# advait/c4a0

Hardware: AMD Instinct MI355X
Metric: self-play games/sec (and MCTS sims/sec) at n_mcts=100 (higher is better)
Workload: dtype bf16

## Files before the change

c4a0_amd/_lib.py:

```python
from __future__ import annotations

import ctypes as C
import os

_HERE = os.path.dirname(os.path.abspath(__file__))
LIB_PATH = os.path.join(_HERE, os.environ.get("C4A0_HIP_LIB", "libc4a0_hip.so"))

OK, ERR_BAD_ARG, ERR_HIP, ERR_NAN_IN_TREE, ERR_DEGENERATE_POLICY, ERR_ARENA_OVERFLOW, ERR_NOT_BOUND, ERR_NO_DEVICE, ERR_ILLEGAL_MOVE, ERR_CANCELLED = range(10)
STATUS_NAMES = {
    0: "C4_OK", 1: "C4_ERR_BAD_ARG", 2: "C4_ERR_HIP", 3: "C4_ERR_NAN_IN_TREE", 4: "C4_ERR_DEGENERATE_POLICY",
    5: "C4_ERR_ARENA_OVERFLOW", 6: "C4_ERR_NOT_BOUND", 7: "C4_ERR_NO_DEVICE", 8: "C4_ERR_ILLEGAL_MOVE", 9: "C4_ERR_CANCELLED",
}
FLAG_NO_MOVES = 1
FLAG_ONE_SIM_PER_STEP = 2
FLAG_RECLAIM = 4
FLAG_NO_RECLAIM = 8
FLAG_SEARCH = 16
FLAG_HOLD = 32
HOLD_PARKED = 64
HOLD_MOVE_NONE, HOLD_MOVE_SAMPLE = -1, -2
HOLD_OK, HOLD_REFUSED_TERMINAL, HOLD_REFUSED_COLUMN, HOLD_REFUSED_UNSEARCHED, HOLD_REFUSED_SAMPLE, HOLD_NO_GAME = range(6)
HOLD_POLL_UNKNOWN = 0xFFFFFFFF
MAX_SAMPLES_PER_GAME = 43
ABI_VERSION = 13
STRUCT_LAYOUT_SINCE = 7


class C4Error(RuntimeError):
    def __init__(self, status: int, detail: str = ""):
        self.status = status
        super().__init__(f"{STATUS_NAMES.get(status, status)}: {detail}" if detail else STATUS_NAMES.get(status, str(status)))


class GameMetadataC(C.Structure):
    _fields_ = [("game_id", C.c_uint64), ("player0_id", C.c_uint64), ("player1_id", C.c_uint64)]


class SampleRec(C.Structure):
    _fields_ = [("game_id", C.c_uint64), ("mask", C.c_uint64), ("value", C.c_uint64), ("policy", C.c_float * 7),
                ("q_penalty", C.c_float), ("q_no_penalty", C.c_float), ("meta", C.c_uint32)]


class Config(C.Structure):
    _fields_ = [("n_slots", C.c_uint32), ("blocks_per_slot", C.c_uint32), ("n_mcts_iterations", C.c_uint32),
                ("c_exploration", C.c_float), ("c_ply_penalty", C.c_float), ("planes_dtype", C.c_uint32),
                ("flags", C.c_uint32), ("device", C.c_int32), ("reclaim_period", C.c_uint32)]


class Counters(C.Structure):
    _fields_ = [(n, C.c_uint64) for n in ("sims", "select_levels", "backup_nodes", "expansions", "moves", "games_done",
                                          "ref_skipped_sims", "samples", "games_started", "step_kernel_ns", "step_launches",
                                          "eval_cache_probes", "eval_cache_hits", "reclaim_passes", "reclaim_blocks")] + \
               [("error", C.c_uint32), ("error_slot", C.c_uint32)]

    def as_dict(self):
        return {n: int(getattr(self, n)) for n, _ in self._fields_}


class NetworkBf16(C.Structure):
    _fields_ = [("channels", C.c_uint32), ("n_blocks", C.c_uint32), ("tower_w0", C.c_void_p), ("tower_w", C.c_void_p), ("tower_bias", C.c_void_p),
                ("w1", C.c_void_p), ("b1", C.c_void_p), ("n_policy_hidden", C.c_uint32), ("n_value_hidden", C.c_uint32),
                ("policy_w", C.c_void_p * 8), ("policy_b", C.c_void_p * 8), ("value_w", C.c_void_p * 8), ("value_b", C.c_void_p * 8),
                ("policy_out_w", C.c_void_p), ("value_out_w", C.c_void_p), ("policy_out_b", C.c_void_p), ("value_out_b", C.c_void_p)]


class PlayOptions(C.Structure):
    _fields_ = [("device", C.c_int32), ("resident_games", C.c_uint32), ("concurrent_sessions", C.c_uint32), ("steps_per_graph", C.c_uint32),
                ("tail_steps_per_graph", C.c_uint32), ("blocks_per_slot", C.c_uint32), ("flags", C.c_uint32), ("reclaim_period", C.c_uint32),
                ("dirichlet_alpha", C.c_float), ("dirichlet_epsilon", C.c_float), ("eval_cache_entries", C.c_uint64)]


class PlayPhases(C.Structure):
    _fields_ = [("setup_s", C.c_double), ("capture_s", C.c_double), ("steady_s", C.c_double), ("tail_s", C.c_double), ("drain_s", C.c_double),
                ("rounds", C.c_uint64), ("rounds_until_all_started", C.c_uint64), ("graph_captures", C.c_uint32), ("resident_games", C.c_uint32),
                ("sessions", C.c_uint32), ("rows_at_end", C.c_uint32)]

    def as_dict(self):
        return {n: getattr(self, n) for n, _ in self._fields_}


_P = C.POINTER
_vp = C.c_void_p
SIGNATURES = {
    "c4_last_error_string": (C.c_char_p, []),
    "c4_abi_version": (C.c_int, []),
    "c4_source_hash": (C.c_char_p, []),
    "c4_device_count": (C.c_int, [_P(C.c_int)]),
    "c4_session_create": (C.c_int, [_P(Config), _P(_vp)]),
    "c4_session_destroy": (C.c_int, [_vp]),
    "c4_session_set_games": (C.c_int, [_vp, _P(GameMetadataC), C.c_uint64, _P(C.c_uint64), _P(C.c_uint64)]),
    "c4_session_bind_io": (C.c_int, [_vp, _vp, _vp, _vp, _vp]),
    "c4_session_set_dirichlet": (C.c_int, [_vp, C.c_float, C.c_float]),
    "c4_session_bind_leaf_models": (C.c_int, [_vp, _vp]),
    "c4_session_set_eval_cache": (C.c_int, [_vp, C.c_uint64, C.c_uint32]),
    "c4_session_progress": (C.c_int, [_vp, _P(C.c_uint64), _P(C.c_uint64), _P(C.c_uint32)]),
    "c4_session_compact": (C.c_int, [_vp, C.c_uint32, _P(C.c_uint32), _P(C.c_uint32)]),
    "c4_session_start": (C.c_int, [_vp]),
    "c4_session_step": (C.c_int, [_vp]),
    "c4_session_set_step_shape": (C.c_int, [_vp, C.c_uint32]),
    "c4_session_step_head_out": (C.c_int, [_vp, _vp, _vp, _vp, _vp, _vp, _vp, C.c_uint32, C.c_uint32, C.c_uint32]),
    "c4_session_set_timing": (C.c_int, [_vp, C.c_int]),
    "c4_session_counters": (C.c_int, [_vp, _P(Counters)]),
    "c4_session_poll": (C.c_int, [_vp, _P(C.c_uint64), _P(C.c_uint32)]),
    "c4_session_arena": (C.c_int, [_vp, _P(C.c_uint64), _P(C.c_uint32), _P(C.c_uint32)]),
    "c4_session_sample_counts": (C.c_int, [_vp, _P(C.c_uint32), C.c_uint64]),
    "c4_session_drain_samples": (C.c_int, [_vp, _P(SampleRec), C.c_uint64, _P(C.c_uint64)]),
    "c4_session_pack_samples": (C.c_int, [_vp, _vp, C.c_uint64, _P(C.c_uint64)]),
    "c4_session_debug_phase_stamps": (C.c_int, [_vp, _P(C.c_uint64), C.c_uint64, _P(C.c_uint64)]),
    "c4_session_sample_store": (C.c_int, [_vp, _P(_vp), _P(_vp), _P(C.c_uint64)]),
    "c4_session_root_stats": (C.c_int, [_vp, C.c_uint32, _P(C.c_float), _P(C.c_float), _P(C.c_float),
                                        _P(C.c_uint64), _P(C.c_uint64), _P(C.c_uint64)]),
    "c4_trim_cached_memory": (C.c_int, []),
    "c4_records_to_cbor": (C.c_int, [_vp, _vp, C.c_uint64, _vp, C.c_uint64, _vp, C.c_uint64, _P(C.c_uint64)]),
    "c4_shuffle_games": (C.c_int, [C.c_uint64, C.c_uint64, _vp]),
    "c4_play_games_cancel": (None, []),
    "c4_play_games_bf16": (C.c_int, [_vp, C.c_uint64, C.c_uint32, C.c_float, C.c_float, _P(NetworkBf16), _P(PlayOptions), _vp, _vp, C.c_uint64,
                                     _P(C.c_uint64), _P(Counters), _P(PlayPhases)]),
    "c4_search_positions_bf16": (C.c_int, [_vp, _vp, C.c_uint64, C.c_uint32, C.c_float, C.c_float, _P(NetworkBf16), _P(PlayOptions), _vp, C.c_uint64,
                                           _P(Counters), _P(PlayPhases)]),
    "c4_cbor_to_records": (C.c_int, [_vp, C.c_uint64, _vp, _vp, C.c_uint64, _vp, C.c_uint64, _P(C.c_uint64), _P(C.c_uint64)]),
    "c4_session_leaf_keys": (C.c_int, [_vp, _vp]),
    "c4_session_unique_leaves": (C.c_int, [_vp, _vp, _vp, _vp, _vp]),
    "c4_session_scatter_outputs": (C.c_int, [_vp, _vp, _vp, C.c_uint32]),
    "c4_session_step_gather": (C.c_int, [_vp, _vp, _vp, C.c_uint32]),
    "c4_session_set_iterations": (C.c_int, [_vp, C.c_uint32]),
    "c4_session_hold_resume": (C.c_int, [_vp, _vp, _vp, _vp]),
    "c4_session_snapshot": (C.c_int, [_vp, _vp, _vp, _vp, C.c_uint64]),
    "c4_session_hold_poll": (C.c_int, [_vp, _P(C.c_uint32), _P(C.c_uint32), _P(C.c_uint32)]),
    "c4_session_leaves": (C.c_int, [_vp, _P(C.c_uint64), _P(C.c_uint64), _P(C.c_uint32), _P(C.c_uint32)]),
    "c4_pos_ops": (C.c_int, [_vp, _vp, _vp, C.c_uint64, C.c_float, _vp, _vp, _vp, _vp, _vp, _vp]),
    "c4_encode_planes": (C.c_int, [_vp, _vp, C.c_uint64, C.c_uint32, _vp, _vp]),
    "c4_expf_logf": (C.c_int, [_vp, C.c_uint64, C.c_int, _vp, _vp]),
    "c4_softmax7": (C.c_int, [_vp, _vp, C.c_uint64, _vp, _vp, _vp]),
    "c4_apply_temperature": (C.c_int, [_vp, _vp, C.c_uint64, _vp, _vp]),
    "c4_conv_tower_bf16": (C.c_int, [_vp, _vp, _vp, _vp, C.c_uint32, C.c_uint32, C.c_uint32, _vp, C.c_uint32, _vp]),
    "c4_linear_bf16": (C.c_int, [_vp, _vp, _vp, _vp, C.c_uint32, C.c_uint32, C.c_uint32, C.c_uint32, C.c_uint32, C.c_uint32, C.c_uint32, _vp]),
    "c4_linear_bf16_tile_map": (C.c_int, [C.c_uint32, C.c_uint32, C.c_uint32, C.c_uint32, _P(C.c_uint32), C.c_uint32, _P(C.c_uint32)]),
    "c4_planes_from_f32": (C.c_int, [_vp, _vp, C.c_uint32, _vp, C.c_uint32, _vp]),
    "c4_head_out_bf16": (C.c_int, [_vp, _vp, _vp, _vp, _vp, _vp, C.c_uint32, C.c_uint32, C.c_uint32, C.c_uint32, _vp, _vp, _vp]),
    "c4_dirichlet": (C.c_int, [_vp, _vp, _vp, C.c_float, C.c_uint64, _vp, _vp]),
    "c4_sample_move": (C.c_int, [_vp, _vp, _vp, _vp, C.c_uint64, _vp, _vp, _vp]),
    "c4_conv_tower_f32": (C.c_int, [_vp, _vp, _vp, _vp, C.c_uint32, C.c_uint32, C.c_uint32, _vp, _vp, _vp]),
    "c4_linear_f32": (C.c_int, [_vp, _vp, _vp, _vp, C.c_uint32, C.c_uint32, C.c_uint32, C.c_uint32, C.c_uint32, C.c_uint32, _vp]),
    "c4_head_out_f32": (C.c_int, [_vp, _vp, _vp, _vp, _vp, _vp, C.c_uint32, C.c_uint32, C.c_uint32, C.c_uint32, C.c_uint32, _vp, _vp, _vp, _vp]),
}

_lib = None


def lib() -> C.CDLL:
    global _lib
    if _lib is None:
        if not os.path.exists(LIB_PATH):
            raise ImportError(
                f"{LIB_PATH} is missing: the HIP extension is the product and there is no fallback. "
                "Build it with `python c4a0_amd/csrc/build.py` (hipcc --offload-arch=gfx950).")
        import torch

        L = C.CDLL(LIB_PATH)
        diagnostic = "C4A0_HIP_LIB" in os.environ
        for name, (res, args) in SIGNATURES.items():
            fn = getattr(L, name, None)
            if fn is None:
                if diagnostic:
                    continue
                raise ImportError(f"{LIB_PATH} does not export {name}")
            fn.restype = res
            fn.argtypes = args
        if L.c4_abi_version() != ABI_VERSION and not diagnostic:
            raise ImportError(f"{LIB_PATH} implements C ABI version {L.c4_abi_version()}, this binding is written for {ABI_VERSION}")
        if diagnostic and L.c4_abi_version() < STRUCT_LAYOUT_SINCE:
            raise ImportError(f"{LIB_PATH} implements C ABI version {L.c4_abi_version()}: c4_config / c4_counters changed layout in version "
                              f"{STRUCT_LAYOUT_SINCE}; build the A/B library from a revision at or after it")
        if "C4A0_HIP_LIB" not in os.environ:
            from .csrc import build as _build

            have, want = L.c4_source_hash().decode(), _build.source_hash()
            if have != want:
                raise ImportError(f"{LIB_PATH} was built from different sources (hash {have}, tree {want}): "
                                  "rebuild it with `python c4a0_amd/csrc/build.py`")
        _lib = L
    return _lib

# ... 6 lines not shown
```

c4a0_amd/csrc/build.py:

```python
import hashlib
import os
import subprocess
import sys

HERE = os.path.dirname(os.path.abspath(__file__))
PKG = os.path.dirname(HERE)
OUT = os.path.join(PKG, "libc4a0_hip.so")
SRCS = [os.path.join(HERE, "c4_session.hip"), os.path.join(HERE, "c4_conv_tower.hip"), os.path.join(HERE, "c4_head_gemm.hip"), os.path.join(HERE, "c4_results_host.hip"), os.path.join(HERE, "c4_selfplay_host.hip"), os.path.join(HERE, "c4_f32_net.hip")]
DEPS = SRCS + [os.path.join(HERE, "c4_device.hpp"), os.path.join(HERE, "c4_host.hpp"), os.path.join(HERE, "c4_head_out.hpp"), os.path.join(HERE, "c4_timeline.hpp"),
               os.path.join(os.path.dirname(PKG), "include", "c4a0_hip.h")]
FLAGS = ["--offload-arch=gfx950", "-O3", "-std=c++17", "-fPIC", "-shared", "-ffp-contract=off",
         "-fno-fast-math", "-Wall", "-Wno-unused-function",
         "-mllvm", "-amdgpu-kernarg-preload-count=16"]
MARKER = b"c4a0-src-hash:"


def source_hash(extra_flags=()) -> str:
    h = hashlib.sha256(" ".join(FLAGS + list(extra_flags)).encode())
    for d in DEPS:
        h.update(os.path.basename(d).encode() + b"\0")
        with open(d, "rb") as f:
            h.update(f.read())
    return h.hexdigest()[:32]


def embedded_hash(path: str):
    try:
        with open(path, "rb") as f:
            blob = f.read()
    except OSError:
        return None
    i = blob.find(MARKER)
    if i < 0:
        return None
    return blob[i + len(MARKER): i + len(MARKER) + 32].decode("ascii", "replace")


def is_stale(path: str = OUT, extra_flags=()) -> bool:
    return embedded_hash(path) != source_hash(extra_flags)


def build(force: bool = False, verbose: bool = False, diag: bool = False) -> str:
    hipcc = os.environ.get("HIPCC", "/opt/rocm/bin/hipcc")
    out = OUT.replace(".so", "_diag.so") if diag else OUT
    extra = ["-DC4_PHASE_STAMPS", "-DC4_DIAG_VARIANTS"] if diag else []
    if force or is_stale(out, extra):
        tmp = out + ".tmp%d" % os.getpid()
        cmd = [hipcc] + FLAGS + extra + ['-DC4_SOURCE_HASH="%s"' % source_hash(extra)] + SRCS + ["-o", tmp]
        if verbose:
            print(" ".join(cmd))
        r = subprocess.run(cmd, capture_output=True, text=True)
        if r.returncode != 0:
            if os.path.exists(tmp):
                os.remove(tmp)
            raise RuntimeError("hipcc failed:\n" + r.stdout + r.stderr)
        os.replace(tmp, out)
        if verbose and r.stderr:
            print(r.stderr)
    return out


if __name__ == "__main__":
    print(build(force="--force" in sys.argv, verbose=True, diag="--diag" in sys.argv))
```

c4a0_amd/csrc/c4_conv_tower.hip:

```cpp
#include <hip/hip_runtime.h>
#include <stdint.h>
#include <stdio.h>
#include <stdlib.h>

#include <string>
#include <type_traits>

#include "../../include/c4a0_hip.h"
#include "c4_head_out.hpp"
#include "c4_host.hpp"
#include "c4_timeline.hpp"

#ifndef C4_TOWER_PAIR_SAME_SIMD
#define C4_TOWER_PAIR_SAME_SIMD 0
#endif
#ifndef C4_TOWER_ALT_PRIO
#define C4_TOWER_ALT_PRIO 0
#endif

namespace {

typedef __bf16 bf16x8 __attribute__((ext_vector_type(8)));
typedef __bf16 bf16x4 __attribute__((ext_vector_type(4)));
typedef float f32x4 __attribute__((ext_vector_type(4)));

constexpr int kBS = 56;
constexpr int kTilesPerBoard = 3;

__device__ __forceinline__ int cell_slot(int r, int c) { return (r + 1) * 8 + (c + 1) + 1; }

template <int C, int NB>
struct Geo {
  static constexpr int KG = C / 8;
  static constexpr int MT = C / 16;
  static constexpr int KC = C / 32;
  static constexpr int kPlane = (NB * kBS + 10 + 15) / 16 * 16;
  static constexpr int kBufSlots = KG * kPlane;
  static constexpr bool kStageW = (C == 32);
  static constexpr int kWFrags = 9 * MT * KC;
  static constexpr int kLdsBytes = 2 * kBufSlots * 16 + (kStageW ? 2 * kWFrags * 1024 : 0);
  static constexpr int kTiles = NB * kTilesPerBoard;
  static_assert((kPlane * 16) % 256 == 0, "channel-group planes must keep the bank phase");
  static_assert(kLdsBytes <= 160 * 1024, "LDS budget");
};

#ifdef C4_PHASE_STAMPS
__device__ unsigned long long c4_tower_clk[80];
#define C4_TSTAMP(i) do { if (threadIdx.x == 0) tw_ts[i] = __builtin_amdgcn_s_memrealtime(); } while (0)
#else
#define C4_TSTAMP(i) do { } while (0)
#endif

struct TowerParams {
  const uint16_t* planes;
  const bf16x8* w0;
  const bf16x8* w;
  const float* bias;
  uint16_t* out;
  uint32_t n_boards;
  uint32_t n_blocks;
};

template <int C, int NB, bool kConv0, bool kSecond, bool kLast, int G_TILES, int MTW, bool kPrefetch, typename WF, typename Hook>
__device__ __forceinline__ void tower_layer(const uint4* __restrict__ src, uint4* __restrict__ dst, WF& wf,
                                            const float* __restrict__ bias, int tile_lo, int m0, int lane, Hook&& after_last_tile,
                                            uint16_t* __restrict__ out = nullptr, uint32_t board0 = 0, uint32_t n_boards = 0) {
  using G = Geo<C, NB>;
  constexpr int kSteps = kConv0 ? 3 : 9 * G::KC;
  constexpr int NF = kPrefetch ? 2 : 1;
  const int li = lane & 15, lg = lane >> 4;

  f32x4 bias4[MTW];
#pragma unroll
  for (int m = 0; m < MTW; m++) {
    const float* bp = bias + 16 * (m0 + m) + 4 * lg;
    bias4[m] = f32x4{bp[0], bp[1], bp[2], bp[3]};
  }

  uint4 fr[NF][kSteps];
  f32x4 acc[2][MTW];
  uint2 old[2][MTW];
  int e_slot[2], e_cell[2];
  int e_board[2];

  auto tile_cell = [&](int g, int& cell) __attribute__((always_inline)) {
    const int tl = tile_lo + g;
    const int bidx = tl / kTilesPerBoard;
    const int slot = 9 + 16 * (tl - bidx * kTilesPerBoard) + li;
    cell = slot;
    return bidx * kBS + slot;
  };
  auto load_frags = [&](int g, int f) __attribute__((always_inline)) {
    int cell;
    const int base = tile_cell(g, cell);
#pragma unroll
    for (int k = 0; k < kSteps; k++) {
      int d, plane;
      if (kConv0) {
        int tap = 4 * k + lg;
        tap = tap < 9 ? tap : 4;
        d = 8 * (tap / 3 - 1) + (tap % 3 - 1);
        plane = 0;
      } else {
        const int t = k / G::KC, kc = k % G::KC;
        d = 8 * (t / 3 - 1) + (t % 3 - 1);
        plane = 4 * kc + lg;
      }
      fr[f][k] = src[plane * G::kPlane + base + d];
    }
  };
  auto out_ptr = [&](int slot_in_plane, int m) __attribute__((always_inline)) {
    return reinterpret_cast<uint2*>(&dst[(2 * (m0 + m) + (lg >> 1)) * G::kPlane + slot_in_plane]) + (lg & 1);
  };
  auto start_tile = [&](int g, int a) __attribute__((always_inline)) {
    e_slot[a] = tile_cell(g, e_cell[a]);
    e_board[a] = (tile_lo + g) / kTilesPerBoard;
#pragma unroll
    for (int m = 0; m < MTW; m++) {
      acc[a][m] = bias4[m];
      if (kSecond && kPrefetch) old[a][m] = *out_ptr(e_slot[a], m);
    }
  };
  auto mfmas = [&](int f, int a) __attribute__((always_inline)) {
#pragma unroll
    for (int k = 0; k < kSteps; k++) {
#pragma unroll
      for (int m = 0; m < MTW; m++)
        acc[a][m] = __builtin_amdgcn_mfma_f32_16x16x32_bf16(wf[k][m], __builtin_bit_cast(bf16x8, fr[f][k]), acc[a][m], 0, 0, 0);
    }
  };
  auto epilogue = [&](int a) __attribute__((always_inline)) {
    const bool valid = ((e_cell[a] - 1) & 7) != 0;
#pragma unroll
    for (int m = 0; m < MTW; m++) {
      f32x4 v = acc[a][m];
      if (kSecond) {
        const uint2 o = kPrefetch ? old[a][m] : *out_ptr(e_slot[a], m);
        const float o0 = __uint_as_float(o.x << 16), o1 = __uint_as_float(o.x & 0xffff0000u);
        const float o2 = __uint_as_float(o.y << 16), o3 = __uint_as_float(o.y & 0xffff0000u);
        v[0] = o0 + fmaxf(v[0], 0.f); v[1] = o1 + fmaxf(v[1], 0.f);
        v[2] = o2 + fmaxf(v[2], 0.f); v[3] = o3 + fmaxf(v[3], 0.f);
      }
      const bf16x4 o = __builtin_convertvector(v, bf16x4);
      if (kLast) {
        const int rc = e_cell[a] - 1, cell = 7 * ((rc >> 3) - 1) + (rc & 7) - 1;
        const uint32_t gb = board0 + (uint32_t)e_board[a];
        if (valid && gb < n_boards)
          *reinterpret_cast<uint2*>(out + ((size_t)gb * 42 + cell) * C + 16 * (m0 + m) + 4 * lg) = __builtin_bit_cast(uint2, o);
      } else if (valid) {
        *out_ptr(e_slot[a], m) = __builtin_bit_cast(uint2, o);
      }
    }
  };

  load_frags(0, 0);
  if (kPrefetch) {
#pragma unroll
    for (int g = 0; g < G_TILES; g++) {
      const int a = g & 1, f = g & 1;
      start_tile(g, a);
      if (g + 1 < G_TILES) load_frags(g + 1, f ^ 1);
      mfmas(f, a);
      if (g >= 1) epilogue(a ^ 1);
    }
    epilogue((G_TILES - 1) & 1);
  } else {
#pragma unroll
    for (int g = 0; g < G_TILES; g++) {
      start_tile(g, 0);
      mfmas(0, 0);
      epilogue(0);
      if (g + 1 < G_TILES) load_frags(g + 1, 0);
    }
  }
  after_last_tile();
}

struct NoStamp { __device__ __forceinline__ void operator()(int) const {} };
struct NoFeed { static constexpr bool kRing = false; };
template <int C>
struct RingFeed {
  static constexpr bool kRing = true;
  static constexpr int kStageSlots = (C / 16) * (C / 32) * 64;
  const uint4* ring;
  __amdgpu_buffer_rsrc_t rsrc;
  int t, n_stages, wave, lane;
  __device__ __forceinline__ void issue(int st) {
    __builtin_amdgcn_raw_ptr_buffer_load_lds(rsrc, (__attribute__((address_space(3))) void*)(ring + (st & 3) * kStageSlots + wave * 64), 16,
                                             (int)((uint32_t)(lane * 16) | (st >= n_stages ? 0x80000000u : 0u)), st * (kStageSlots * 16) + wave * 1024, 0, 0);
  }
  __device__ __forceinline__ void stage_top() {
    t += 1;
    asm volatile("s_waitcnt vmcnt(2) lgkmcnt(0)" ::: "memory");
    __builtin_amdgcn_s_barrier();
    issue(t + 4);
  }
  template <typename WQ, int MTW>
  __device__ __forceinline__ void read(WQ& wq, int s, int kc, int m0) const {
    const uint4* st = ring + ((t + 1) & 3) * kStageSlots + lane;
#pragma unroll
    for (int m = 0; m < MTW; m++) wq[s % 2][m] = __builtin_bit_cast(bf16x8, st[((m0 + m) * (C / 32) + kc) * 64]);
  }
};
__device__ __forceinline__ float tower_relu1(float v) {
  float r;
  asm("v_max_f32 %0, 0, %1" : "=v"(r) : "v"(v));
  return r;
}
template <int C, int NB, int G_TILES, int MTW, int kDepth, typename WQ, typename Stamp = NoStamp, int kMode = -1, typename Feed = NoFeed>
__device__ __forceinline__ void tower_layer_stream(const bool kSecond, const bool kLast, const uint4* __restrict__ src, uint4* __restrict__ dst, WQ& wq,
                                                   const bf16x8* __restrict__ w_layer, bool has_next, const float* __restrict__ bias,
                                                   int tile_lo, int m0, int lane, uint16_t* __restrict__ out = nullptr,
                                                   uint32_t board0 = 0, uint32_t n_boards = 0, Stamp&& stamp = NoStamp{}, Feed&& feed = NoFeed{}) {
  using G = Geo<C, NB>;
  using FeedT = typename std::remove_reference<Feed>::type;
  constexpr int kSteps = 9 * G::KC;
  static_assert(kSteps % kDepth == 0, "the weight ring keeps its phase from layer to layer");
  static_assert(!FeedT::kRing || (kDepth == 2 && G::KC == 2), "the LDS ring is read one stage (= one tap = two k-steps) ahead");
  const int li = lane & 15, lg = lane >> 4;

  auto request = [&](int s) __attribute__((always_inline)) {
    if constexpr (FeedT::kRing) { feed.template read<WQ, MTW>(wq, s, s % G::KC, m0); return; }
    const int sl = s % kSteps;
    const bf16x8* wl = w_layer + (s >= kSteps ? G::kWFrags * 64 : 0);
#pragma unroll
    for (int m = 0; m < MTW; m++) wq[s % kDepth][m] = wl[(((sl / G::KC) * G::MT + m0 + m) * G::KC + (sl % G::KC)) * 64 + lane];
  };

  int base[G_TILES], cell[G_TILES];
  f32x4 acc[G_TILES][MTW];
#pragma unroll
  for (int g = 0; g < G_TILES; g++) {
    const int tl = tile_lo + g;
    const int bidx = tl / kTilesPerBoard;
    cell[g] = 9 + 16 * (tl - bidx * kTilesPerBoard) + li;
    base[g] = bidx * kBS + cell[g];
#pragma unroll
    for (int m = 0; m < MTW; m++) {
      const float* bp = bias + 16 * (m0 + m) + 4 * lg;
      acc[g][m] = f32x4{bp[0], bp[1], bp[2], bp[3]};
    }
  }
  uint4 fr[2][G_TILES][G::KC];
  auto read_row = [&](int r, int f) __attribute__((always_inline)) {
    const int d = 8 * (r - 1);
#pragma unroll
    for (int g = 0; g < G_TILES; g++)
#pragma unroll
      for (int kc = 0; kc < G::KC; kc++) fr[f][g][kc] = src[(4 * kc + lg) * G::kPlane + base[g] + d];
  };
  auto shifted = [&](const uint4& v, int dc) __attribute__((always_inline)) {
    if (dc == 1) return v;
    uint4 o;
    if (dc == 2) {
      o.x = (uint32_t)__builtin_amdgcn_update_dpp(0, (int)v.x, 0x101, 0xF, 0xF, true); o.y = (uint32_t)__builtin_amdgcn_update_dpp(0, (int)v.y, 0x101, 0xF, 0xF, true);
      o.z = (uint32_t)__builtin_amdgcn_update_dpp(0, (int)v.z, 0x101, 0xF, 0xF, true); o.w = (uint32_t)__builtin_amdgcn_update_dpp(0, (int)v.w, 0x101, 0xF, 0xF, true);
    } else {
      o.x = (uint32_t)__builtin_amdgcn_update_dpp(0, (int)v.x, 0x111, 0xF, 0xF, true); o.y = (uint32_t)__builtin_amdgcn_update_dpp(0, (int)v.y, 0x111, 0xF, 0xF, true);
      o.z = (uint32_t)__builtin_amdgcn_update_dpp(0, (int)v.z, 0x111, 0xF, 0xF, true); o.w = (uint32_t)__builtin_amdgcn_update_dpp(0, (int)v.w, 0x111, 0xF, 0xF, true);
// ... 11 lines not shown
      if constexpr (FeedT::kRing) {
        if (3 * r + dc > 0) { feed.stage_top(); __builtin_amdgcn_sched_barrier(0); }
      }
#pragma unroll
      for (int kc = 0; kc < G::KC; kc++) {
        const int s = (3 * r + dc) * G::KC + kc;
#pragma unroll
        for (int g = 0; g < G_TILES; g++) {
          const uint4 bfrag = shifted(fr[r & 1][g][kc], dc);
#pragma unroll
          for (int m = 0; m < MTW; m++)
            acc[g][m] = __builtin_amdgcn_mfma_f32_16x16x32_bf16(wq[s % kDepth][m], __builtin_bit_cast(bf16x8, bfrag), acc[g][m], 0, 0, 0);
        }
        if (FeedT::kRing || s + kDepth < kSteps || has_next) request(s + kDepth);
        __builtin_amdgcn_sched_barrier(0);
      }
    }
  }
  stamp(1);
  if constexpr (kMode >= 0) {
    constexpr bool kSec = kMode >= 1, kLst = kMode == 2;
    auto optr = [&](int g, int m) __attribute__((always_inline)) {
      return reinterpret_cast<uint2*>(&dst[(2 * (m0 + m) + (lg >> 1)) * G::kPlane + base[g]]) + (lg & 1);
    };
    uint2 res[G_TILES][MTW];
    if (kSec) {
#pragma unroll
      for (int g = 0; g < G_TILES; g++)
#pragma unroll
        for (int m = 0; m < MTW; m++) res[g][m] = *optr(g, m);
    }
    const bool valid = (li & 7) != 0;
    const uint32_t vmask = valid ? 0xFFFFFFFFu : 0u;
#pragma unroll
    for (int g = 0; g < G_TILES; g++) {
#pragma unroll
      for (int m = 0; m < MTW; m++) {
        f32x4 v = acc[g][m];
        if (kSec) {
          const uint2 o = res[g][m];
          v[0] = __uint_as_float(o.x << 16) + tower_relu1(v[0]); v[1] = __uint_as_float(o.x & 0xffff0000u) + tower_relu1(v[1]);
          v[2] = __uint_as_float(o.y << 16) + tower_relu1(v[2]); v[3] = __uint_as_float(o.y & 0xffff0000u) + tower_relu1(v[3]);
        }
        uint2 ob = __builtin_bit_cast(uint2, __builtin_convertvector(v, bf16x4));
        if (kLst) {
          const int rc = cell[g] - 1, bcell = 7 * ((rc >> 3) - 1) + (rc & 7) - 1;
          const uint32_t gb = board0 + (uint32_t)((tile_lo + g) / kTilesPerBoard);
          if (valid && gb < n_boards) *reinterpret_cast<uint2*>(out + ((size_t)gb * 42 + bcell) * C + 16 * (m0 + m) + 4 * lg) = ob;
        } else {
          ob.x &= vmask; ob.y &= vmask;
          *optr(g, m) = ob;
        }
      }
    }
    stamp(2);
    return;
  }
#pragma unroll
  for (int g = 0; g < G_TILES; g++) {
    const bool valid = ((cell[g] - 1) & 7) != 0;
#pragma unroll
    for (int m = 0; m < MTW; m++) {
      uint2* op = reinterpret_cast<uint2*>(&dst[(2 * (m0 + m) + (lg >> 1)) * G::kPlane + base[g]]) + (lg & 1);
      f32x4 v = acc[g][m];
      if (kSecond) {
        const uint2 o = *op;
        v[0] = __uint_as_float(o.x << 16) + fmaxf(v[0], 0.f); v[1] = __uint_as_float(o.x & 0xffff0000u) + fmaxf(v[1], 0.f);
        v[2] = __uint_as_float(o.y << 16) + fmaxf(v[2], 0.f); v[3] = __uint_as_float(o.y & 0xffff0000u) + fmaxf(v[3], 0.f);
      }
      const bf16x4 o = __builtin_convertvector(v, bf16x4);
      if (kLast) {
        const int rc = cell[g] - 1, bcell = 7 * ((rc >> 3) - 1) + (rc & 7) - 1;
        const uint32_t gb = board0 + (uint32_t)((tile_lo + g) / kTilesPerBoard);
        if (valid && gb < n_boards)
          *reinterpret_cast<uint2*>(out + ((size_t)gb * 42 + bcell) * C + 16 * (m0 + m) + 4 * lg) = __builtin_bit_cast(uint2, o);
      } else if (valid) {
        *op = __builtin_bit_cast(uint2, o);
      }
    }
  }
  stamp(2);
}

template <int KW, int NWAVES>
__device__ __forceinline__ void dma_weights(const void* w, uint32_t bytes, uint4* lds_dst, int first_frag, int wave, int lane) {
  const auto rsrc = __builtin_amdgcn_make_buffer_rsrc(const_cast<void*>(w), 0, (int)bytes, 0x00020000);
  const int wave_u = __builtin_amdgcn_readfirstlane(wave);
  for (int c = wave_u; c < KW; c += NWAVES)
    __builtin_amdgcn_raw_ptr_buffer_load_lds(rsrc, (__attribute__((address_space(3))) void*)(lds_dst + c * 64), 16, lane * 16, (first_frag + c) * 1024, 0, 0);
}

template <int C, int NB, int NT, int MS, bool ST = false, int KD = 3, bool RG = false>
__global__ __launch_bounds__(NT) void c4_conv_tower_kernel(const uint16_t* __restrict__ a_planes, const bf16x8* __restrict__ a_w0, const bf16x8* __restrict__ a_w,
                                                             const float* __restrict__ a_bias, uint16_t* __restrict__ a_out, uint32_t a_n_boards, uint32_t a_n_blocks) {
  const TowerParams p{a_planes, a_w0, a_w, a_bias, a_out, a_n_boards, a_n_blocks};
  C4_TL_BEGIN();
#ifdef C4_PHASE_STAMPS
  unsigned long long tw_ts[64];
  const unsigned long long wave_c0 = __builtin_amdgcn_s_memtime();
  const unsigned long long wave_r0 = __builtin_amdgcn_s_memrealtime();
  auto tw_flush = [&](int last) {
    if (threadIdx.x == 0) {
      atomicAdd(&c4_tower_clk[70], __builtin_amdgcn_s_memtime() - wave_c0);
      atomicAdd(&c4_tower_clk[71], __builtin_amdgcn_s_memrealtime() - wave_r0);
      atomicAdd(&c4_tower_clk[0], 1ull);
      for (int i = 0; i < last; i++) atomicAdd(&c4_tower_clk[1 + i], tw_ts[i + 1] - tw_ts[i]);
      atomicMin(&c4_tower_clk[78], tw_ts[0]);
      atomicMax(&c4_tower_clk[79], tw_ts[last]);
    }
  };
#endif
  C4_TSTAMP(0);
#ifdef C4_PHASE_STAMPS
  const unsigned long long wave_t0 = __builtin_amdgcn_s_memrealtime();
#endif
  using G = Geo<C, NB>;
  constexpr int MTW = G::MT / MS;
  static_assert(G::MT % MS == 0 && (!G::kStageW || MS == 1), "co-tile split");

  extern __shared__ __attribute__((aligned(256))) uint8_t lds_raw[];
  uint4* X = reinterpret_cast<uint4*>(lds_raw);
  uint4* T = X + G::kBufSlots;

  const int tid = threadIdx.x;
  const int lane = tid & 63;
  const int wave = tid >> 6;
#if C4_TOWER_PAIR_SAME_SIMD
  constexpr int kGroups = NT / 64 / MS;
  const int grp_index = wave % kGroups, grp_member = wave / kGroups;
#else
  const int grp_index = wave / MS, grp_member = wave % MS;
#endif
  const int m0 = grp_member * MTW;
  const uint32_t board0 = blockIdx.x * NB;

  constexpr int kWSteps = 9 * G::KC;
  bf16x8 wf[kWSteps][MTW];
#pragma unroll
  for (int k = 0; k < 3; k++)
#pragma unroll
    for (int m = 0; m < MTW; m++) wf[k][m] = p.w0[(k * G::MT + m0 + m) * 64 + lane];
  const int n_layers = 2 * (int)p.n_blocks;
  if constexpr (ST && RG) {
    RingFeed<C> f0{reinterpret_cast<const uint4*>(lds_raw) + 2 * G::kBufSlots,
                   __builtin_amdgcn_make_buffer_rsrc(const_cast<bf16x8*>(p.w), 0, (int)(2u * p.n_blocks * G::kWFrags * 1024u), 0x00020000), -1, 9 * n_layers,
                   __builtin_amdgcn_readfirstlane(wave), lane};
#pragma unroll
    for (int st = 0; st < 4; st++) f0.issue(st);
  }
  auto load_layer_weights = [&](int layer) __attribute__((always_inline)) {
    const bf16x8* wl = p.w + (size_t)(layer - 1) * G::kWFrags * 64;
#pragma unroll
    for (int k = 0; k < kWSteps; k++)
#pragma unroll
      for (int m = 0; m < MTW; m++) wf[k][m] = wl[(((k / G::KC) * G::MT + m0 + m) * G::KC + (k % G::KC)) * 64 + lane];
  };
  uint4* Wst = T + G::kBufSlots;
  auto stage_layer_weights = [&](int layer) __attribute__((always_inline)) {
    if (layer <= n_layers)
      dma_weights<G::kWFrags, NT / 64>(p.w, 2u * p.n_blocks * G::kWFrags * 1024u, Wst + (layer & 1) * G::kWFrags * 64, (layer - 1) * G::kWFrags, wave, lane);
  };
  auto fetch_staged_weights = [&](int layer) __attribute__((always_inline)) {
    const uint4* ws = Wst + (layer & 1) * G::kWFrags * 64;
#pragma unroll
    for (int k = 0; k < kWSteps; k++)
#pragma unroll
      for (int m = 0; m < MTW; m++)
        wf[k][m] = __builtin_bit_cast(bf16x8, ws[(((k / G::KC) * G::MT + m0 + m) * G::KC + (k % G::KC)) * 64 + lane]);
  };
  if (G::kStageW && !ST) stage_layer_weights(1);

  constexpr int kIn = (NB * 42 + NT - 1) / NT;
  uint32_t in_v[kIn];
#pragma unroll
  for (int j = 0; j < kIn; j++) {
    const int i = tid + j * NT;
    const int b = i / 42, cell = i - b * 42;
    const uint32_t g = board0 + b;
    in_v[j] = 0;
    if (i < NB * 42 && g < p.n_boards) in_v[j] = (uint32_t)p.planes[(size_t)g * 84 + cell] | ((uint32_t)p.planes[(size_t)g * 84 + 42 + cell] << 16);
  }
  for (int i = tid; i < 2 * G::kBufSlots; i += NT) X[i] = make_uint4(0, 0, 0, 0);
  int* pair_ctr = reinterpret_cast<int*>(lds_raw + G::kLdsBytes);
  if (ST && !RG && tid < 16) pair_ctr[tid] = 0;
  __syncthreads();
#pragma unroll
  for (int j = 0; j < kIn; j++) {
    const int i = tid + j * NT;
    const int b = i / 42, cell = i - b * 42;
    if (i < NB * 42) T[b * kBS + cell_slot(cell / 7, cell % 7)] = make_uint4(in_v[j], 0, 0, 0);
  }
  __syncthreads();
  C4_TSTAMP(1);

  constexpr int kWaves = NT / 64 / MS;
  static_assert(G::kTiles % kWaves == 0, "every wavefront owns the same number of cell tiles");
  constexpr int kTilesPerWave = G::kTiles / kWaves;
  constexpr bool kPrefetch = (C == 32);
  constexpr bool kFuseOut = (C == 32);
  const int tile_lo = grp_index * kTilesPerWave;

  if constexpr (ST && RG) {
    static_assert(NT == 512 && MS == 2 && C == 64, "one 1 KB DMA piece per wavefront and stage");
    const uint4* ring = T + G::kBufSlots;
    float* bias_lds = reinterpret_cast<float*>(lds_raw + 2 * G::kBufSlots * 16 + 4 * RingFeed<C>::kStageSlots * 16);
    RingFeed<C> feed{ring, __builtin_amdgcn_make_buffer_rsrc(const_cast<bf16x8*>(p.w), 0, (int)(2u * p.n_blocks * G::kWFrags * 1024u), 0x00020000),
                     -1, 9 * n_layers, __builtin_amdgcn_readfirstlane(wave), lane};
    for (int i = tid; i < n_layers * C; i += NT) bias_lds[i] = p.bias[C + i];
    bf16x8 wq[2][MTW];
    tower_layer<C, NB, true, false, false, kTilesPerWave, MTW, false>(T, X, wf, p.bias, tile_lo, m0, lane, [&]() __attribute__((always_inline)) {});
    asm volatile("s_waitcnt vmcnt(0) lgkmcnt(0)" ::: "memory");
    __builtin_amdgcn_s_barrier();
    feed.template read<decltype(wq), MTW>(wq, 0, 0, m0);
    feed.template read<decltype(wq), MTW>(wq, 1, 1, m0);
    for (int layer = 1; layer <= n_layers; layer++) {
      const bool second = (layer & 1) == 0;
      const float* bl = bias_lds + (size_t)(layer - 1) * C;
      if (layer == n_layers)
        tower_layer_stream<C, NB, kTilesPerWave, MTW, 2, decltype(wq), NoStamp, 2, RingFeed<C>&>(true, true, T, X, wq, nullptr, false, bl, tile_lo, m0, lane, p.out, board0, p.n_boards, NoStamp{}, feed);
      else if (second)
        tower_layer_stream<C, NB, kTilesPerWave, MTW, 2, decltype(wq), NoStamp, 1, RingFeed<C>&>(true, false, T, X, wq, nullptr, true, bl, tile_lo, m0, lane, p.out, board0, p.n_boards, NoStamp{}, feed);
      else
        tower_layer_stream<C, NB, kTilesPerWave, MTW, 2, decltype(wq), NoStamp, 0, RingFeed<C>&>(false, false, X, T, wq, nullptr, true, bl, tile_lo, m0, lane, p.out, board0, p.n_boards, NoStamp{}, feed);
    }
    asm volatile("s_waitcnt vmcnt(0)" ::: "memory");
    if (n_layers > 0) return;
  } else if constexpr (ST) {
    constexpr int kDepth = KD;
    bf16x8 wq[kDepth][MTW];
    if (n_layers >= 1) {
#pragma unroll
      for (int sdx = 0; sdx < kDepth; sdx++)
#pragma unroll
        for (int m = 0; m < MTW; m++) wq[sdx][m] = p.w[(((sdx / G::KC) * G::MT + m0 + m) * G::KC + (sdx % G::KC)) * 64 + lane];
    }
    tower_layer<C, NB, true, false, false, kTilesPerWave, MTW, false>(T, X, wf, p.bias, tile_lo, m0, lane, [&]() __attribute__((always_inline)) {});
    constexpr bool kBarrier = !(MS == 1 && kTilesPerWave % kTilesPerBoard == 0);
    if (kBarrier) __syncthreads();
    C4_TSTAMP(2);
    for (int layer = 1; layer <= n_layers; layer++) {
      const bf16x8* wl = p.w + (size_t)(layer - 1) * G::kWFrags * 64;
      const bool has_next = layer < n_layers;
      const float* bl = p.bias + (size_t)layer * C;
      const bool second = (layer & 1) == 0;
#if C4_TOWER_ALT_PRIO
      if (((layer ^ (__builtin_amdgcn_readfirstlane(wave) >> 2)) & 1) != 0) __builtin_amdgcn_s_setprio(1); else __builtin_amdgcn_s_setprio(0);
#endif
#ifdef C4_PHASE_STAMPS
      auto st_stamp = [&](int q) __attribute__((always_inline)) {
        asm volatile("s_waitcnt vmcnt(0) lgkmcnt(0)" ::: "memory");
        if (layer <= 19) C4_TSTAMP(2 + 3 * (layer - 1) + q);
      };
#elif defined(C4_TOWER64_FENCE)
      auto st_stamp = [&](int q) __attribute__((always_inline)) {
        if (C4_TOWER64_FENCE == 1) asm volatile("" ::: "memory");
        if (C4_TOWER64_FENCE == 2) asm volatile("s_waitcnt lgkmcnt(0)" ::: "memory");
        if (C4_TOWER64_FENCE == 3) asm volatile("s_waitcnt vmcnt(0) lgkmcnt(0)" ::: "memory");
      };
#else
      NoStamp st_stamp;
#endif
      if constexpr (MS == 1) {
        if (layer == n_layers)
          tower_layer_stream<C, NB, kTilesPerWave, MTW, kDepth, decltype(wq), decltype(st_stamp)&, 2>(true, true, T, X, wq, wl, false, bl, tile_lo, m0, lane, p.out, board0, p.n_boards, st_stamp);
        else if (second)
          tower_layer_stream<C, NB, kTilesPerWave, MTW, kDepth, decltype(wq), decltype(st_stamp)&, 1>(true, false, T, X, wq, wl, true, bl, tile_lo, m0, lane, p.out, board0, p.n_boards, st_stamp);
        else
          tower_layer_stream<C, NB, kTilesPerWave, MTW, kDepth, decltype(wq), decltype(st_stamp)&, 0>(false, false, X, T, wq, wl, true, bl, tile_lo, m0, lane, p.out, board0, p.n_boards, st_stamp);
      } else
      tower_layer_stream<C, NB, kTilesPerWave, MTW, kDepth>(second, layer == n_layers, second ? T : X, second ? X : T, wq, wl, has_next, bl, tile_lo, m0, lane,
                                                            p.out, board0, p.n_boards, st_stamp);
#ifdef C4_PHASE_STAMPS
      if (layer == n_layers) {
        st_stamp(3);
        if (layer <= 19) tw_flush(2 + 3 * layer);
        if (lane == 0) atomicAdd(&c4_tower_clk[62 + wave], __builtin_amdgcn_s_memrealtime() - wave_t0);
      }
#endif
      if (layer == n_layers) return;
      if (kBarrier) {
        __builtin_amdgcn_fence(__ATOMIC_RELEASE, "workgroup");
        int* ctr = pair_ctr + grp_index;
        if (lane == 0) __hip_atomic_fetch_add(ctr, 1, __ATOMIC_RELAXED, __HIP_MEMORY_SCOPE_WORKGROUP);
        while (__hip_atomic_load(ctr, __ATOMIC_RELAXED, __HIP_MEMORY_SCOPE_WORKGROUP) < MS * layer) __builtin_amdgcn_s_sleep(1);
        __builtin_amdgcn_fence(__ATOMIC_ACQUIRE, "workgroup");
      }
#if defined(C4_PHASE_STAMPS) || defined(C4_TOWER64_FENCE)
      st_stamp(3);
#endif
    }
  } else {
  tower_layer<C, NB, true, false, false, kTilesPerWave, MTW, kPrefetch>(T, X, wf, p.bias, tile_lo, m0, lane, [&]() __attribute__((always_inline)) {
    if (!G::kStageW && n_layers >= 1) load_layer_weights(1);
  });
  if (G::kStageW) asm volatile("s_waitcnt vmcnt(0)" ::: "memory");
  __syncthreads();
  C4_TSTAMP(2);
  for (int layer = 1; layer <= n_layers; layer++) {
    const bool is_second = (layer & 1) == 0;
    if (G::kStageW) {
      stage_layer_weights(layer + 1);
      fetch_staged_weights(layer);
    }
    auto next_weights = [&]() __attribute__((always_inline)) {
      if (!G::kStageW && layer < n_layers) load_layer_weights(layer + 1);
    };
    if (kFuseOut && layer == n_layers) {
      tower_layer<C, NB, false, true, true, kTilesPerWave, MTW, kPrefetch>(T, X, wf, p.bias + (size_t)layer * C, tile_lo, m0, lane, next_weights,
                                                                          p.out, board0, p.n_boards);
#ifdef C4_PHASE_STAMPS
      asm volatile("s_waitcnt vmcnt(0)" ::: "memory");
      if (layer < 20) { C4_TSTAMP(2 + layer); tw_flush(2 + layer); }
#endif
      C4_TL_END(1, p.out);
      return;
    }
    if (is_second) tower_layer<C, NB, false, true, false, kTilesPerWave, MTW, kPrefetch>(T, X, wf, p.bias + (size_t)layer * C, tile_lo, m0, lane, next_weights);
    else tower_layer<C, NB, false, false, false, kTilesPerWave, MTW, kPrefetch>(X, T, wf, p.bias + (size_t)layer * C, tile_lo, m0, lane, next_weights);
    if (G::kStageW) asm volatile("s_waitcnt vmcnt(0)" ::: "memory");
    __syncthreads();
#ifdef C4_PHASE_STAMPS
    if (layer < 20) C4_TSTAMP(2 + layer);
#endif
  }
  }

  if (ST) __syncthreads();
  for (int i = tid; i < NB * 42 * G::KG; i += NT) {
    const int kg = i % G::KG;
    const int bc = i / G::KG;
    const int b = bc / 42, cell = bc - b * 42;
    const uint32_t g = board0 + b;
    if (g < p.n_boards) {
      const uint4 v = X[kg * G::kPlane + b * kBS + cell_slot(cell / 7, cell % 7)];
      reinterpret_cast<uint4*>(p.out)[((size_t)g * 42 + cell) * G::KG + kg] = v;
    }
  }
  C4_TL_END(1, p.out);
}

template <int C, int NB, int NT, int MS, bool ST = false, int KD = 3, bool RG = false>
int launch_tower(const TowerParams& p, uint32_t n_boards, hipStream_t stream, int device) {
  const int kLds = Geo<C, NB>::kLdsBytes + (ST ? 64 : 0) + (RG ? 4 * RingFeed<C>::kStageSlots * 16 + 2 * (int)p.n_blocks * C * 4 : 0);
  auto k = c4_conv_tower_kernel<C, NB, NT, MS, ST, KD, RG>;
  hipError_t e = c4host::opt_in_lds((const void*)k, RG ? 160 * 1024 : kLds, device);
  if (e != hipSuccess) return c4host::fail(C4_ERR_HIP, std::string("c4_conv_tower_bf16: LDS opt-in (") + std::to_string(kLds) + " bytes) on device " + std::to_string(device) + ": " + hipGetErrorString(e));
  k<<<dim3((n_boards + NB - 1) / NB), dim3(NT), kLds, stream>>>(p.planes, p.w0, p.w, p.bias, p.out, p.n_boards, p.n_blocks);
  e = hipGetLastError();
  if (e != hipSuccess) return c4host::fail(C4_ERR_HIP, std::string("c4_conv_tower_bf16 launch: ") + hipGetErrorString(e));
  return C4_OK;
}

}

#ifdef C4_PHASE_STAMPS
extern "C" int c4_debug_tower_phases(double* phase_us, int n, double* span_us, unsigned long long* n_workgroups, int reset) {
  unsigned long long h[80];
  if (hipDeviceSynchronize() != hipSuccess || hipMemcpyFromSymbol(h, HIP_SYMBOL(c4_tower_clk), sizeof h) != hipSuccess) return C4_ERR_HIP;
  for (int i = 0; i < n && i < 76; i++) phase_us[i] = h[0] ? (double)h[1 + i] / (double)h[0] * 0.01 : 0.0;
  if (span_us) *span_us = h[79] > h[78] ? (double)(h[79] - h[78]) * 0.01 : 0.0;
  if (n_workgroups) *n_workgroups = h[0];
  if (reset) { unsigned long long z[80] = {0}; z[78] = ~0ull; if (hipMemcpyToSymbol(HIP_SYMBOL(c4_tower_clk), z, sizeof z) != hipSuccess) return C4_ERR_HIP; }
  return C4_OK;
}
#endif

C4_TL_SETTER(c4_debug_timeline_tower)

extern "C" {

int c4_conv_tower_bf16(const void* planes_dev, const void* w0_dev, const void* w_dev, const float* bias_dev,
                       uint32_t n_boards, uint32_t channels, uint32_t n_blocks, void* out_dev, uint32_t config, void* stream) {
  if (!planes_dev || !w0_dev || !bias_dev || !out_dev || (n_blocks && !w_dev)) return c4host::fail(C4_ERR_BAD_ARG, "c4_conv_tower_bf16: null argument");
  if (channels != 32 && channels != 64) return c4host::fail(C4_ERR_BAD_ARG, "c4_conv_tower_bf16: channels must be 32 or 64");
  if (n_boards == 0) return C4_OK;
  const int device = c4host::stream_device((hipStream_t)stream);
  c4host::DeviceGuard guard(device);
  if (guard.error() != hipSuccess) return c4host::fail(C4_ERR_HIP, std::string("c4_conv_tower_bf16: hipSetDevice: ") + hipGetErrorString(guard.error()));
  TowerParams p{(const uint16_t*)planes_dev, (const bf16x8*)w0_dev, (const bf16x8*)w_dev, bias_dev, (uint16_t*)out_dev, n_boards, n_blocks};
  if (config > 6 || (channels == 32 && config > 5)) return c4host::fail(C4_ERR_BAD_ARG, "c4_conv_tower_bf16: config must be 0 (automatic) .. 5 (32 channels) / .. 6 (64 channels)");
  if (channels == 64 && config == 4 && Geo<64, 8>::kLdsBytes + 64 + 4 * RingFeed<64>::kStageSlots * 16 + 2 * (int)n_blocks * 64 * 4 > 160 * 1024)
    return c4host::fail(C4_ERR_BAD_ARG, "c4_conv_tower_bf16: config 4 (weights through an LDS ring) keeps the layers' biases in LDS behind the ring: at most 23 residual blocks");
  if (channels == 32 && config == 1) return launch_tower<32, 16, 512, 1>(p, n_boards, (hipStream_t)stream, device);
  if (channels == 32 && config == 2) return launch_tower<32, 8, 512, 1>(p, n_boards, (hipStream_t)stream, device);
  if (channels == 32 && config == 3) return launch_tower<32, 16, 768, 1>(p, n_boards, (hipStream_t)stream, device);
  if (channels == 32 && config == 4) return launch_tower<32, 4, 768, 1>(p, n_boards, (hipStream_t)stream, device);
  if (channels == 32 && config == 5) return launch_tower<32, 2, 384, 1>(p, n_boards, (hipStream_t)stream, device);
  if (channels == 32 && n_boards <= 512) return launch_tower<32, 2, 384, 1>(p, n_boards, (hipStream_t)stream, device);
  if (channels == 32 && n_boards <= 1024) return launch_tower<32, 4, 768, 1>(p, n_boards, (hipStream_t)stream, device);
  if (channels == 32 && n_boards <= 8 * 160)
    return launch_tower<32, 8, 512, 1>(p, n_boards, (hipStream_t)stream, device);
#ifdef C4_DIAG_VARIANTS
  static const int st32 = [] { const char* e = getenv("C4_TOWER32_STREAM"); return e ? atoi(e) : 0; }();
  if (channels == 32 && st32) return launch_tower<32, 16, 512, 1, true>(p, n_boards, (hipStream_t)stream, device);
  static const int held = [] { const char* e = getenv("C4_TOWER64_HELD"); return e ? atoi(e) : 0; }();
  if (channels == 64 && held) return launch_tower<64, 8, 512, 2>(p, n_boards, (hipStream_t)stream, device);
#endif
  if (channels == 32)
    return launch_tower<32, 16, 512, 1>(p, n_boards, (hipStream_t)stream, device);
  if (channels == 64 && (config == 5 || (config == 0 && n_boards > 512 && n_boards <= 1024))) return launch_tower<64, 4, 512, 2, true>(p, n_boards, (hipStream_t)stream, device);
  if (channels == 64 && (config == 6 || (config == 0 && n_boards <= 512))) return launch_tower<64, 2, 256, 2, true>(p, n_boards, (hipStream_t)stream, device);
  if (channels == 64 && config == 2) return launch_tower<64, 8, 256, 1, true, 6>(p, n_boards, (hipStream_t)stream, device);
  if (channels == 64 && config == 3) return launch_tower<64, 8, 256, 1, true, 3>(p, n_boards, (hipStream_t)stream, device);
  if (channels == 64 && config == 4 && Geo<64, 8>::kLdsBytes + 64 + 4 * RingFeed<64>::kStageSlots * 16 + 2 * (int)n_blocks * 64 * 4 <= 160 * 1024)
    return launch_tower<64, 8, 512, 2, true, 2, true>(p, n_boards, (hipStream_t)stream, device);
  return launch_tower<64, 8, 512, 2, true>(p, n_boards, (hipStream_t)stream, device);
// ... 152 lines not shown
```

c4a0_amd/csrc/c4_head_out.hpp:

```cpp
#pragma once
#include <hip/hip_runtime.h>
#include <stdint.h>

namespace c4ho {

typedef __bf16 bf16x8 __attribute__((ext_vector_type(8)));
typedef float f32x4 __attribute__((ext_vector_type(4)));

constexpr int kHeadWaves = 6, kHeadSteps = 7;

struct Shared {
  f32x4 part[kHeadWaves][2][64];
  float tile[2][16][17];
  float res[16][12];
};

template <int kRows>
__device__ __forceinline__ void head_out_block(Shared& sh, const uint4* __restrict__ hp, const uint4* __restrict__ hv, const uint4* __restrict__ wp,
                                               const uint4* __restrict__ wv, const float* __restrict__ bp, const float* __restrict__ bv, uint32_t n_boards,
                                               uint32_t f8, uint32_t sp8, uint32_t sv8, float* __restrict__ logprobs, float* __restrict__ q, uint32_t block) {
  const uint32_t lane = threadIdx.x & 63, wave = threadIdx.x >> 6;
  const uint32_t row = lane & 15, kq = lane >> 4;
  const uint32_t g0 = block * kRows;
  const uint32_t gr = g0 + (row & (kRows - 1));
  const uint32_t g = gr < n_boards ? gr : n_boards - 1;
  const uint4* xp = hp + (size_t)g * sp8 + kq;
  const uint4* xv = hv + (size_t)g * sv8 + kq;
  const uint4* wpl = wp + (size_t)(row < 7 ? row : 0) * f8 + kq;
  const uint4* wvl = wv + (size_t)(row < 2 ? row : 0) * f8 + kq;
  f32x4 accp = {0.f, 0.f, 0.f, 0.f}, accv = {0.f, 0.f, 0.f, 0.f};
  const uint32_t n_iter = f8 / (4 * kHeadSteps * kHeadWaves);
  for (uint32_t it = 0; it < n_iter; it++) {
    const uint32_t s0 = (it * kHeadWaves + wave) * kHeadSteps;
    uint4 a_p[kHeadSteps], a_v[kHeadSteps], b_p[kHeadSteps], b_v[kHeadSteps];
#pragma unroll
    for (int s = 0; s < kHeadSteps; s++) {
      a_p[s] = xp[4 * (s0 + s)];
      a_v[s] = xv[4 * (s0 + s)];
      b_p[s] = wpl[4 * (s0 + s)];
      b_v[s] = wvl[4 * (s0 + s)];
    }
    __builtin_amdgcn_sched_barrier(0);
    const uint32_t mp = row < 7 ? 0xFFFFFFFFu : 0u, mv = row < 2 ? 0xFFFFFFFFu : 0u;
#pragma unroll
    for (int s = 0; s < kHeadSteps; s++) {
      b_p[s].x &= mp; b_p[s].y &= mp; b_p[s].z &= mp; b_p[s].w &= mp;
      b_v[s].x &= mv; b_v[s].y &= mv; b_v[s].z &= mv; b_v[s].w &= mv;
    }
#pragma unroll
    for (int s = 0; s < kHeadSteps; s++) {
      accp = __builtin_amdgcn_mfma_f32_16x16x32_bf16(__builtin_bit_cast(bf16x8, a_p[s]), __builtin_bit_cast(bf16x8, b_p[s]), accp, 0, 0, 0);
      accv = __builtin_amdgcn_mfma_f32_16x16x32_bf16(__builtin_bit_cast(bf16x8, a_v[s]), __builtin_bit_cast(bf16x8, b_v[s]), accv, 0, 0, 0);
    }
  }
  sh.part[wave][0][lane] = accp;
  sh.part[wave][1][lane] = accv;
  __syncthreads();
  if (wave < 2) {
    f32x4 sum = sh.part[0][wave][lane];
#pragma unroll
    for (int w = 1; w < kHeadWaves; w++) sum += sh.part[w][wave][lane];
    const float bias = wave == 0 ? (row < 7 ? bp[row] : 0.f) : (row < 2 ? bv[row] : 0.f);
#pragma unroll
    for (int r = 0; r < 4; r++) sh.tile[wave][4 * kq + r][row] = sum[r] + bias;
  }
  __syncthreads();
  if (threadIdx.x < kRows) {
    const uint32_t b = threadIdx.x, gb = g0 + b;
    float v[9];
#pragma unroll
    for (int o = 0; o < 7; o++) v[o] = sh.tile[0][b][o];
    v[7] = sh.tile[1][b][0];
    v[8] = sh.tile[1][b][1];
    float mx = v[0];
#pragma unroll
    for (int o = 1; o < 7; o++) mx = fmaxf(mx, v[o]);
    float sm = 0.f;
#pragma unroll
    for (int o = 0; o < 7; o++) sm += expf(v[o] - mx);
    const float lse = mx + logf(sm);
    const float q0 = tanhf(v[7]), q1 = tanhf(v[8]);
#pragma unroll
    for (int o = 0; o < 7; o++) sh.res[b][o] = v[o] - lse;
    sh.res[b][7] = q0;
    sh.res[b][8] = q1;
    if (gb < n_boards) {
#pragma unroll
      for (int o = 0; o < 7; o++) logprobs[(size_t)gb * 7 + o] = v[o] - lse;
      q[(size_t)gb * 2 + 0] = q0;
      q[(size_t)gb * 2 + 1] = q1;
    }
  }
}

}
```

c4a0_amd/csrc/c4_session.hip:

```cpp
#include <hip/hip_runtime.h>
#include <hip/hip_bf16.h>
#include <stddef.h>
#include <stdint.h>
#include <stdio.h>
#include <stdlib.h>
#include <string.h>
#include <mutex>
#include <string>
#include <vector>

#include "../../include/c4a0_hip.h"
#include "c4_device.hpp"
#include "c4_head_out.hpp"
#include "c4_host.hpp"
#include "c4_timeline.hpp"

#pragma clang fp contract(off)

namespace {

struct __attribute__((aligned(16))) Entry {
  uint32_t n;
  float q_pen;
  float q_nopen;
  float prior;
};
struct __attribute__((aligned(16))) Tail {
  uint16_t child[7];
  uint16_t legal;
};
struct __attribute__((aligned(128))) Block {
  Entry e[7];
  Tail t;
};
constexpr uint32_t kMaxBlocksPerSlot = 65535;

constexpr uint32_t kMaxPath = 43;
constexpr uint32_t kHotPath = 16;
struct __attribute__((aligned(256))) Slot {
  uint64_t root_mask, root_value;
  uint64_t leaf_mask, leaf_value;
  uint64_t game_id;
  uint32_t ordinal;
  uint32_t root_n;
  uint32_t state;
  uint32_t arena;
  uint32_t root_ref;
  uint32_t rng_word;
  uint32_t path[kHotPath];
  uint32_t path_deep[kMaxPath - kHotPath];
  uint32_t pad_[32 - (kMaxPath - kHotPath)];
};
static_assert(sizeof(Slot) == 256 && offsetof(Slot, path) == 64 && offsetof(Slot, path_deep) == 128, "slot state: one hot line + the deep path");
C4_DEV constexpr uint32_t slot_state(uint32_t status, uint32_t depth, uint32_t n_moves, uint32_t term, uint32_t rng_for) {
  return status | (depth << 8) | (n_moves << 16) | (term << 24) | (rng_for << 26);
}
C4_DEV uint32_t slot_status(uint32_t state) { return state & 0xFFu; }
static_assert(sizeof(Block) == 128 && sizeof(Entry) == 16 && sizeof(Tail) == 16 && sizeof(c4_sample_rec) == 64, "layout");

enum : uint32_t { kIdle = 0, kActive = 1, kParked = C4_HOLD_PARKED };
constexpr uint32_t kWavesPerTimingHelper = 1024;

#ifdef C4_PHASE_STAMPS
#define C4_STAMP(i, force)                                                                          \
  do {                                                                                              \
    asm volatile("s_waitcnt vmcnt(0) lgkmcnt(0)" ::: "memory");                                       \
    if (lane == 0) p.phase[(size_t)wave_index * 16 + (i)] = __builtin_amdgcn_s_memrealtime() + ((force) & 0);  \
  } while (0)
#define C4_STAMP_ANY(i)                                                                             \
  do {                                                                                              \
    asm volatile("s_waitcnt vmcnt(0) lgkmcnt(0)" ::: "memory");                                       \
    if (lane == (uint32_t)(__ffsll((long long)__ballot(1)) - 1)) p.phase[(size_t)wave_index * 16 + (i)] = __builtin_amdgcn_s_memrealtime();  \
  } while (0)
#else
#define C4_STAMP(i, force) do { } while (0)
#define C4_STAMP_ANY(i) do { } while (0)
#endif
enum : int { CTR_SIMS = 0, CTR_S, CTR_K, CTR_E, CTR_MOVES, CTR_DONE, CTR_SKIPPED, CTR_SAMPLES, CTR_PROBES, CTR_HITS, CTR_N = 16 };

struct Globals {
  unsigned long long queue_head;
  unsigned long long games_done;
  uint32_t error;
  uint32_t error_slot;
  uint32_t hold_active;
  uint32_t hold_need;
};

struct Params {
  Slot* slots;
  Block* blocks;
  unsigned long long* wave_ctr;
  unsigned long long* stamps;
  unsigned long long* clock_acc;
  uint32_t n_waves;
  uint32_t seq;
  unsigned long long* phase;
  uint64_t* leaf_models;
// ... 692 lines not shown
  const Slot* st = p.slots + gs;
  const Block* blocks = p.blocks + (size_t)gs * p.blocks_per_slot;
  const uint32_t state = st->state, root_block = st->arena >> 16, root_ref = st->root_ref;
  const bool game = slot_status(state) != kIdle;
  const uint4 re = load_block_lane(blocks, game ? root_block : 0u, sub);
  const float cnt = (game && sub < 7 && root_block != 0) ? (float)re.x : 0.0f;
  float w[7];
  float csum = 0.0f;
  for (int i = 0; i < 7; i++) { w[i] = shfl_f32(cnt, gbase + i); csum = csum + w[i]; }
  if (g >= p.n_slots) return;
  c4_sample_rec* rec = dst + g;
  if (!game) {
    reinterpret_cast<uint2*>(rec)[sub] = make_uint2(0u, 0u);
    if (sub == 7) { visits[g] = 0; status[g] = kIdle; }
    return;
  }
  if (sub < 7) rec->policy[sub] = (csum == 0.0f) ? (1.0f / 7.0f) : (w[sub] / csum);
  if (sub == 7) {
    const Entry* re0 = &blocks[root_ref >> 3].e[root_ref & 7];
    const float nf = (float)re0->n + 1.0f;
    rec->game_id = st->game_id; rec->mask = st->root_mask; rec->value = st->root_value;
    rec->q_penalty = re0->q_pen / nf; rec->q_no_penalty = re0->q_nopen / nf;
    rec->meta = ((state >> 16) & 0xFFu) | (3u << 16);
    visits[g] = re0->n;
    status[g] = slot_status(state);
  }
}

template <typename PlaneT, bool NOISE, bool CACHE>
__global__ __launch_bounds__(64, (NOISE || CACHE) ? 1 : C4_STEP_WAVES) void c4_step_gather_kernel(
    Slot* __restrict__ a_slots, const float* __restrict__ a_answers, const uint32_t* __restrict__ a_inverse, uint32_t a_n_unique, uint32_t a_n_waves,
    uint32_t a_n_slots, Params p) {
  const uint32_t lane = threadIdx.x & 63;
  const uint32_t sub = lane & 7;
  const uint32_t wave_index = blockIdx.x;
  const uint32_t g = wave_index * 8 + (lane >> 3);
  const unsigned long long t_start = __builtin_amdgcn_s_memrealtime();
  C4_STAMP(0, 0);
  if (blockIdx.x >= a_n_waves) { timing_helper(p, lane); return; }
  const uint32_t gs = g < a_n_slots ? g : 0;
  Slot* st = a_slots + gs;
  const uint4 hot = reinterpret_cast<const uint4*>(st)[sub];
  const uint32_t row = a_inverse[gs];
  float nn_logit = 0.f, nn_q = 0.f;
  if (row < a_n_unique) {
    nn_logit = a_answers[(size_t)row * 9 + (sub < 7 ? sub : 6)];
    nn_q = a_answers[(size_t)row * 9 + 7 + (sub & 1)];
  }
  step_body<PlaneT, NOISE, CACHE>(p, wave_index, lane, a_n_slots, st, hot, nn_logit, nn_q, t_start, g);
}

#ifdef C4_OUT_STEP_WAVES_PER_EU
#define C4_OUT_STEP_ATTR __attribute__((amdgpu_waves_per_eu(C4_OUT_STEP_WAVES_PER_EU, C4_OUT_STEP_WAVES_PER_EU)))
#else
#define C4_OUT_STEP_ATTR
#endif
template <typename PlaneT, uint32_t kGpw, bool SEARCH = false, bool HOLD = false>
__global__ __launch_bounds__(64 * c4ho::kHeadWaves, 1) C4_OUT_STEP_ATTR void c4_out_step_kernel(
    const uint4* __restrict__ hp, const uint4* __restrict__ hv, const uint4* __restrict__ wp, const uint4* __restrict__ wv,
    const float* __restrict__ bp, const float* __restrict__ bv, Slot* __restrict__ a_slots, uint32_t a_n_slots, uint32_t f8, uint32_t sp8, uint32_t sv8,
    Params p) {
  __shared__ c4ho::Shared sh;
  C4_TL_BEGIN();
  constexpr uint32_t kStepWaves = 16 / kGpw;
  static_assert(kGpw == 8 || kGpw == 4, "16 games per workgroup on two or four stepping wavefronts");
  const uint32_t lane = threadIdx.x & 63, wave = threadIdx.x >> 6, sub = lane & 7, grp = lane >> 3;
  const uint32_t b = wave * kGpw + grp;
  const bool mine = wave < kStepWaves && grp < kGpw;
  const uint32_t g = mine ? blockIdx.x * 16 + b : a_n_slots;
  const uint32_t wave_index = blockIdx.x * 2 + wave / (kStepWaves / 2);
  const uint32_t gs = g < a_n_slots ? g : 0;
  Slot* st = a_slots + gs;
  uint4 hot = make_uint4(0, 0, 0, 0);
  if (wave < kStepWaves) hot = reinterpret_cast<const uint4*>(st)[sub];
  c4ho::head_out_block<16>(sh, hp, hv, wp, wv, bp, bv, a_n_slots, f8, sp8, sv8, const_cast<float*>(p.logprobs), const_cast<float*>(p.q), blockIdx.x);
  __syncthreads();
  if (wave >= kStepWaves || wave_index >= p.n_waves) return;
  const float nn_logit = sh.res[b & 15][sub < 7 ? sub : 6];
  const float nn_q = sh.res[b & 15][7 + (sub & 1)];
  step_body<PlaneT, false, false, SEARCH, HOLD>(p, wave_index, lane, a_n_slots, st, hot, nn_logit, nn_q, 0ull, g);
  C4_TL_END(3, a_slots);
}

__global__ void k_pos_ops(const uint64_t* mask, const uint64_t* value, const int32_t* col, uint64_t n, float c_ply,
                          uint64_t* om, uint64_t* ov, uint32_t* olegal, uint32_t* oterm, float* oq) {
  const uint64_t i = (uint64_t)blockIdx.x * blockDim.x + threadIdx.x;
  if (i >= n) return;
  uint64_t m = mask[i], v = value[i];
  const uint32_t legal = c4::legal_mask(m);
  const uint32_t t = c4::terminal_state(m, v);
  float a = 0.0f, b = 0.0f;
  if (t) c4::terminal_value(t, m, c_ply, a, b);
  olegal[i] = legal;
  oterm[i] = t;
  oq[2 * i] = a;
  oq[2 * i + 1] = b;
  const int32_t c = col[i];
  if (c >= 0 && c < 7 && ((legal >> c) & 1u)) {
    c4::make_move(m, v, (uint32_t)c);
    om[i] = m; ov[i] = v;
  } else {
    om[i] = 0; ov[i] = 0;
  }
}

template <typename PlaneT>
__global__ void k_encode(const uint64_t* mask, const uint64_t* value, uint64_t n, void* planes) {
  const uint64_t i = (uint64_t)blockIdx.x * blockDim.x + threadIdx.x;
  if (i >= n * C4_PLANES_LEN) return;
  const uint64_t g = i / C4_PLANES_LEN;
  const uint32_t e = (uint32_t)(i % C4_PLANES_LEN);
  store_plane<PlaneT>(planes, i, c4::plane_bit(mask[g], value[g], e));
}

__global__ void k_ln_table(float* tab, uint32_t n) {
  const uint32_t i = blockIdx.x * blockDim.x + threadIdx.x;
  if (i < n) tab[i] = c4::c4_logf((float)i);
}

__global__ void k_expf_logf(const float* x, uint64_t n, int which, float* y) {
  const uint64_t i = (uint64_t)blockIdx.x * blockDim.x + threadIdx.x;
  if (i >= n) return;
  y[i] = which ? c4::c4_logf(x[i]) : c4::c4_expf(x[i]);
}

__global__ void k_softmax7(const float* logits, const uint32_t* legal, uint64_t n, float* out, uint32_t* err) {
  const uint64_t i = (uint64_t)blockIdx.x * blockDim.x + threadIdx.x;
  if (i >= n) return;
  float l[7], o[7];
  for (int c = 0; c < 7; c++) {
    l[c] = logits[7 * i + c];
    if (legal && !((legal[i] >> c) & 1u)) l[c] = __uint_as_float(0xff800000u);
  }
  const bool ok = c4::softmax7(l, o);
  err[i] = ok ? 0u : (uint32_t)C4_ERR_DEGENERATE_POLICY;
  for (int c = 0; c < 7; c++) out[7 * i + c] = ok ? o[c] : 0.0f;
}

__global__ void k_temperature(const float* policy, const float* t, uint64_t n, float* out) {
  const uint64_t i = (uint64_t)blockIdx.x * blockDim.x + threadIdx.x;
  if (i >= n) return;
  float p[7], o[7];
  for (int c = 0; c < 7; c++) p[c] = policy[7 * i + c];
  c4::apply_temperature(p, t[i], o);
  for (int c = 0; c < 7; c++) out[7 * i + c] = o[c];
}

__global__ void k_sample_move(const uint64_t* game_id, const uint32_t* n_moves, const float* policy, const float* t,
                              uint64_t n, int32_t* out_col, uint32_t* out_u32) {
  const uint64_t i = (uint64_t)blockIdx.x * blockDim.x + threadIdx.x;
  if (i >= n) return;
  float p[7], o[7];
  for (int c = 0; c < 7; c++) p[c] = policy[7 * i + c];
  c4::apply_temperature(p, t[i], o);
  const uint32_t u = c4::rng_first_u32(game_id[i] * (uint64_t)(42 + n_moves[i]));
  out_col[i] = c4::weighted_index(o, u);
  if (out_u32) out_u32[i] = u;
}

__global__ void k_dirichlet(const uint64_t* game_id, const uint32_t* n_moves, const uint32_t* legal, float alpha, uint64_t n, float* eta) {
  const uint64_t i = (uint64_t)blockIdx.x * blockDim.x + threadIdx.x;
  if (i >= n) return;
  float e[7];
  c4::dirichlet_noise(game_id[i], n_moves[i], legal[i], alpha, e);
  for (int c = 0; c < 7; c++) eta[7 * i + c] = e[c];
}
// ... 416 lines not shown

static int maybe_reclaim(c4_session* s) {
  if (!s->p.half_blocks) return C4_OK;
  hipStreamCaptureStatus cs = hipStreamCaptureStatusNone;
  unsigned long long id = 0;
  if (hipStreamGetCaptureInfo(s->stream, &cs, &id) != hipSuccess) { (void)hipGetLastError(); cs = hipStreamCaptureStatusNone; id = 0; }
  if (cs != hipStreamCaptureStatusActive) id = 0;
  if (id != s->reclaim_capture_id) { s->reclaim_capture_id = id; s->reclaim_count = 0; }
  if (s->reclaim_count++ % s->reclaim_period != 0) return C4_OK;
  hipLaunchKernelGGL(k_arena_reclaim, dim3((s->p.n_slots + kReclaimSlotsPerGroup - 1) / kReclaimSlotsPerGroup), dim3(kReclaimThreads), 0, s->stream, s->p,
                     reclaim_min_free(s->reclaim_period, s->p.max_sims));
  HIP_TRY(hipGetLastError());
  return C4_OK;
}

static hipError_t reset_clock_acc(unsigned long long* acc_dev) {
  const unsigned long long init[5] = {0ull, 0ull, ~0ull, 0ull, 0ull};
  return hipMemcpy(acc_dev, init, sizeof init, hipMemcpyHostToDevice);
}

static int session_create_on_device(const c4_config* cfg, c4_session* s) {
  uint64_t bps = cfg->blocks_per_slot;
  const bool reclaim = reclaim_mode(cfg);
  if (reclaim) {
    s->reclaim_period = cfg->reclaim_period ? cfg->reclaim_period : kReclaimPeriod;
    if (bps == 0) {
      uint64_t half = reclaim_half_min(cfg->n_mcts_iterations, s->reclaim_period, 2) + 3ull * cfg->n_mcts_iterations / 2;
      bps = 2 * (half > kMaxBlocksPerSlot / 2 ? kMaxBlocksPerSlot / 2 : half);
    }
    s->p.half_blocks = (uint32_t)(bps / 2);
    bps = 2ull * s->p.half_blocks;
  } else {
    if (bps == 0 && (cfg->flags & C4_FLAG_SEARCH)) bps = (uint64_t)cfg->n_mcts_iterations + 8;
    if (bps == 0) bps = 43ull * (cfg->n_mcts_iterations ? cfg->n_mcts_iterations : 1) + 8;
    if (bps < 2) bps = 2;
  }
  s->cfg.blocks_per_slot = (uint32_t)bps;
  const size_t n = cfg->n_slots;
  const uint32_t games_per_wave = 64u / s->lanes_per_game;
  s->n_waves = (uint32_t)((n + games_per_wave - 1) / games_per_wave);
  s->n_waves_cap = (uint32_t)((n + 7) / 8);
  Params& p = s->p;
  p.n_slots = cfg->n_slots;
  p.blocks_per_slot = (uint32_t)bps;
  p.n_iter = cfg->n_mcts_iterations;
  p.c_exploration = cfg->c_exploration;
  p.c_ply_penalty = cfg->c_ply_penalty;
  p.flags = cfg->flags;
  p.max_sims = (cfg->flags & (C4_FLAG_NO_MOVES | C4_FLAG_ONE_SIM_PER_STEP)) ? 1u : 2u;
  uint32_t n_ln = cfg->n_mcts_iterations + 64u;
  n_ln = n_ln < 1024u ? 1024u : (n_ln > 65536u ? 65536u : n_ln);
  hipError_t e;
  const size_t phase_rows = (size_t)s->n_waves_cap + (s->n_waves_cap + kWavesPerTimingHelper - 1) / kWavesPerTimingHelper + 1;
  if ((e = hipMalloc(&p.slots, n * sizeof(Slot))) != hipSuccess ||
      (e = arena_acquire(cfg->device, s->arena_bytes = n * bps * sizeof(Block), (void**)&p.blocks)) != hipSuccess ||
      (e = hipMalloc(&p.wave_ctr, (size_t)s->n_waves_cap * CTR_N * sizeof(unsigned long long))) != hipSuccess ||
      (e = hipMalloc(&p.glob, sizeof(Globals))) != hipSuccess ||
      (e = hipMalloc(&p.stamps, (size_t)s->n_waves_cap * 4 * sizeof(unsigned long long))) != hipSuccess ||
      (e = hipMalloc(&p.clock_acc, 5 * sizeof(unsigned long long))) != hipSuccess ||
      (e = hipMalloc(&p.phase, phase_rows * 16 * sizeof(unsigned long long))) != hipSuccess ||
      (e = hipMalloc(&s->ln_tab_dev, (size_t)n_ln * sizeof(float))) != hipSuccess ||
      (e = hipMalloc(&p.reclaim_ctr, 2 * sizeof(unsigned long long))) != hipSuccess ||
      (e = hipHostMalloc(&s->probe_host, sizeof(Globals))) != hipSuccess ||
      (e = hipEventCreateWithFlags(&s->probe_event, hipEventDisableTiming)) != hipSuccess)
    return fail(C4_ERR_HIP, std::string("allocating session (") + std::to_string((n * bps * sizeof(Block)) >> 20) +
                                " MiB of tree arena): " + hipGetErrorString(e));
  p.n_waves = s->n_waves;
  p.ln_tab = s->ln_tab_dev;
  p.n_ln = n_ln;
  hipLaunchKernelGGL(k_ln_table, dim3((n_ln + 255) / 256), dim3(256), 0, nullptr, s->ln_tab_dev, n_ln);
  HIP_TRY(hipGetLastError());
  HIP_TRY(hipDeviceSynchronize());
  HIP_TRY(hipMemset(p.stamps, 0, (size_t)s->n_waves_cap * 4 * sizeof(unsigned long long)));
  HIP_TRY(reset_clock_acc(p.clock_acc));
  HIP_TRY(hipMemset(p.phase, 0, phase_rows * 16 * sizeof(unsigned long long)));
  HIP_TRY(hipMemset(p.slots, 0, n * sizeof(Slot)));
  HIP_TRY(hipMemset(p.glob, 0, sizeof(Globals)));
  HIP_TRY(hipMemset(p.reclaim_ctr, 0, 2 * sizeof(unsigned long long)));
  HIP_TRY(hipMemset(p.wave_ctr, 0, (size_t)s->n_waves_cap * CTR_N * sizeof(unsigned long long)));
  memset(s->probe_host, 0, sizeof(Globals));
  return C4_OK;
}

int c4_session_create(const c4_config* cfg, c4_session** out) {
  if (!cfg || !out) return fail(C4_ERR_BAD_ARG, "null argument");
  *out = nullptr;
  if (cfg->n_slots == 0) return fail(C4_ERR_BAD_ARG, "n_slots must be > 0");
  if (cfg->planes_dtype > 1) return fail(C4_ERR_BAD_ARG, "planes_dtype must be 0 (f32) or 1 (bf16)");
  if (cfg->blocks_per_slot > kMaxBlocksPerSlot) return fail(C4_ERR_BAD_ARG, "blocks_per_slot is limited to 65535 (16-bit child links)");
  if (cfg->flags & C4_FLAG_SEARCH) {
    if (cfg->flags & C4_FLAG_NO_MOVES) return fail(C4_ERR_BAD_ARG, "C4_FLAG_SEARCH and C4_FLAG_NO_MOVES exclude each other: a search ends at n_mcts_iterations visits and hands its slot on");
    if (cfg->flags & C4_FLAG_RECLAIM) return fail(C4_ERR_BAD_ARG, "C4_FLAG_SEARCH: a search never moves, so its arena (n_mcts_iterations + 8 blocks) has nothing to reclaim (C4_FLAG_RECLAIM)");
    if (cfg->n_mcts_iterations == 0) return fail(C4_ERR_BAD_ARG, "C4_FLAG_SEARCH needs n_mcts_iterations >= 1");
  }
  if (cfg->flags & C4_FLAG_HOLD) {
    if (cfg->flags & C4_FLAG_SEARCH) return fail(C4_ERR_BAD_ARG, "C4_FLAG_HOLD and C4_FLAG_SEARCH exclude each other: a search hands its slot on after one record, a held game keeps it");
    if (cfg->flags & C4_FLAG_NO_MOVES) return fail(C4_ERR_BAD_ARG, "C4_FLAG_HOLD and C4_FLAG_NO_MOVES exclude each other: a held game parks at its target and moves when c4_session_hold_resume says so");
    if (cfg->flags & C4_FLAG_RECLAIM) return fail(C4_ERR_BAD_ARG, "C4_FLAG_HOLD: a held game's arena is never reclaimed (C4_FLAG_RECLAIM): the subtree under a move is kept in place");
    if (cfg->n_mcts_iterations == 0) return fail(C4_ERR_BAD_ARG, "C4_FLAG_HOLD needs n_mcts_iterations >= 1 (the largest target c4_session_set_iterations may ask for)");
  }
  if (reclaim_mode(cfg)) {
    const uint32_t period = cfg->reclaim_period ? cfg->reclaim_period : kReclaimPeriod;
    const uint64_t need = reclaim_half_min(cfg->n_mcts_iterations, period, 2);
    const uint64_t half = cfg->blocks_per_slot ? cfg->blocks_per_slot / 2 : kMaxBlocksPerSlot / 2;
    if (cfg->flags & C4_FLAG_NO_MOVES) return fail(C4_ERR_BAD_ARG, "C4_FLAG_RECLAIM: a search that never moves never frees anything (C4_FLAG_NO_MOVES)");
    if (cfg->flags & C4_FLAG_NO_RECLAIM) return fail(C4_ERR_BAD_ARG, "C4_FLAG_RECLAIM and C4_FLAG_NO_RECLAIM exclude each other");
    if (period > 4096) return fail(C4_ERR_BAD_ARG, "reclaim_period is limited to 4096 step launches");
    if (half < need)
      return fail(C4_ERR_BAD_ARG, "reclaimed arena too small: each half must hold the live subtree (n_mcts_iterations + simulations per launch + 8 blocks) and the blocks of 4 x "
                                  "reclaim_period step launches (" + std::to_string(need) + " blocks per half, i.e. blocks_per_slot >= " + std::to_string(2 * need) +
                                  "; a half is at most 32 767 blocks: n_mcts_iterations <= " + std::to_string(kMaxBlocksPerSlot / 2 - (need - cfg->n_mcts_iterations)) + ")");
  } else if ((cfg->flags & C4_FLAG_SEARCH) && cfg->blocks_per_slot == 0 && (uint64_t)cfg->n_mcts_iterations + 8 > kMaxBlocksPerSlot)
    return fail(C4_ERR_BAD_ARG, "C4_FLAG_SEARCH: n_mcts_iterations + 8 blocks per slot exceed 65535 (16-bit child links)");
  else if (!(cfg->flags & C4_FLAG_SEARCH) && cfg->blocks_per_slot == 0 && 43ull * cfg->n_mcts_iterations + 8 > kMaxBlocksPerSlot)
    return fail(C4_ERR_BAD_ARG, "n_mcts_iterations > 1523 is not supported with a never-reclaimed arena (C4_FLAG_NO_MOVES / C4_FLAG_NO_RECLAIM): a game's tree arena is limited to "
                                "65535 blocks (16-bit child links; up to 43 n + 8 blocks per game). "
                                "Pass blocks_per_slot explicitly to accept C4_ERR_ARENA_OVERFLOW on long searches");
  int ndev = 0;
  if (hipGetDeviceCount(&ndev) != hipSuccess || ndev == 0) return fail(C4_ERR_NO_DEVICE, "no HIP device visible");
  if (cfg->device < 0 || cfg->device >= ndev) return fail(C4_ERR_BAD_ARG, "device ordinal out of range");
  C4_ON_DEVICE(cfg->device);
  c4_session* s = new c4_session();
  s->cfg = *cfg;
  const int rc = session_create_on_device(cfg, s);
  if (rc != C4_OK) {
    const std::string msg = g_last_error;
    c4_session_destroy(s);
    return fail(rc, msg);
  }
  *out = s;
  return C4_OK;
}

int c4_session_destroy(c4_session* s) {
  if (!s) return C4_OK;
  c4host::DeviceGuard guard(s->cfg.device);
  if (s->stream) (void)hipStreamSynchronize(s->stream); else (void)hipDeviceSynchronize();
  (void)hipFree(s->p.slots); arena_release(s->cfg.device, s->p.blocks, s->arena_bytes); (void)hipFree(s->p.wave_ctr); (void)hipFree(s->p.glob); (void)hipFree(s->p.stamps); (void)hipFree(s->p.clock_acc); (void)hipFree(s->p.phase); (void)hipFree(s->p.reclaim_ctr);
  (void)hipFree(s->p.samples); (void)hipFree(s->p.sample_counts); (void)hipFree(s->p.cache);
  (void)hipFree(s->plan_dev); (void)hipFree(s->pairs_dev); (void)hipFree(s->offsets_dev); (void)hipFree(s->ln_tab_dev);
  if (s->total_host) (void)hipHostFree(s->total_host);
  (void)hipFree(s->uniq_tab); (void)hipFree(s->uniq_cell); (void)hipFree(s->uniq_row); (void)hipFree(s->uniq_count);
  (void)hipFree(s->reqs_dev); (void)hipFree(s->start_mask_dev); (void)hipFree(s->start_value_dev);
  (void)hipFree(s->hold_cols_dev); (void)hipFree(s->hold_temps_dev); (void)hipFree(s->hold_results_dev); (void)hipFree(s->snap_dev);
  if (s->snap_host) (void)hipHostFree(s->snap_host);
  if (s->probe_host) (void)hipHostFree(s->probe_host);
  if (s->probe_event) (void)hipEventDestroy(s->probe_event);
  delete s;
  return C4_OK;
}

int c4_trim_cached_memory(void) {
  ArenaCache c;
  {
    std::lock_guard<std::mutex> lock(g_arena_mutex);
    c = g_arena_cache;
    g_arena_cache = ArenaCache{};
  }
  if (c.ptr) {
    c4host::DeviceGuard guard(c.device);
    HIP_TRY(hipFree(c.ptr));
  }
  return C4_OK;
}

int c4_session_set_games(c4_session* s, const c4_game_metadata* reqs, uint64_t n_games,
                         const uint64_t* start_masks, const uint64_t* start_values) {
  if (!s || (!reqs && n_games)) return fail(C4_ERR_BAD_ARG, "null argument");
  if ((start_masks == nullptr) != (start_values == nullptr)) return fail(C4_ERR_BAD_ARG, "start_masks and start_values go together");
  if (n_games >= (1ull << 32) - 1) return fail(C4_ERR_BAD_ARG, "too many games for one session");
  if (hold_mode(s) && n_games > s->cfg.n_slots)
    return fail(C4_ERR_BAD_ARG, "c4_session_set_games: a hold session (C4_FLAG_HOLD) keeps request i on slot i for good: " + std::to_string(n_games) +
                                    " games do not fit " + std::to_string(s->cfg.n_slots) + " slots");
  C4_ON_DEVICE(s->cfg.device);
  HIP_TRY(hipStreamSynchronize(s->stream));
  (void)hipFree(s->reqs_dev); (void)hipFree(s->start_mask_dev); (void)hipFree(s->start_value_dev);
  (void)hipFree(s->p.samples); (void)hipFree(s->p.sample_counts); (void)hipFree(s->offsets_dev);
  s->reqs_dev = nullptr; s->start_mask_dev = s->start_value_dev = nullptr;
  s->p.samples = nullptr; s->p.sample_counts = nullptr; s->offsets_dev = nullptr;
  const size_t ng = n_games ? n_games : 1;
  HIP_TRY(hipMalloc(&s->offsets_dev, (ng + 1) * sizeof(unsigned long long)));
  if (!s->total_host) HIP_TRY(hipHostMalloc(&s->total_host, sizeof(unsigned long long)));
  HIP_TRY(hipMalloc(&s->reqs_dev, ng * sizeof(c4_game_metadata)));
  HIP_TRY(hipMalloc(&s->p.samples, ng * C4_MAX_SAMPLES_PER_GAME * sizeof(c4_sample_rec)));
  HIP_TRY(hipMalloc(&s->p.sample_counts, ng * sizeof(uint32_t)));
  HIP_TRY(hipMemset(s->p.sample_counts, 0, ng * sizeof(uint32_t)));
  if (n_games) HIP_TRY(hipMemcpy(s->reqs_dev, reqs, n_games * sizeof(c4_game_metadata), hipMemcpyHostToDevice));
  if (start_masks && n_games) {
    HIP_TRY(hipMalloc(&s->start_mask_dev, n_games * 8));
    HIP_TRY(hipMalloc(&s->start_value_dev, n_games * 8));
    HIP_TRY(hipMemcpy(s->start_mask_dev, start_masks, n_games * 8, hipMemcpyHostToDevice));
    HIP_TRY(hipMemcpy(s->start_value_dev, start_values, n_games * 8, hipMemcpyHostToDevice));
  }
  s->p.n_slots = s->cfg.n_slots;
  s->n_waves = s->p.n_waves = (s->cfg.n_slots + 64u / s->lanes_per_game - 1) / (64u / s->lanes_per_game);
  Globals g0{};
  g0.queue_head = n_games < s->cfg.n_slots ? n_games : s->cfg.n_slots;
  HIP_TRY(hipMemcpy(s->p.glob, &g0, sizeof g0, hipMemcpyHostToDevice));
  HIP_TRY(hipMemset(s->p.wave_ctr, 0, (size_t)s->n_waves_cap * CTR_N * sizeof(unsigned long long)));
  s->p.reqs = s->reqs_dev;
  s->p.start_mask = s->start_mask_dev;
  s->p.start_value = s->start_value_dev;
  s->p.n_games = n_games;
  s->n_games = n_games;
  s->have_games = true;
  HIP_TRY(hipMemset(s->p.stamps, 0, (size_t)s->n_waves_cap * 4 * sizeof(unsigned long long)));
  HIP_TRY(reset_clock_acc(s->p.clock_acc));
  if (s->p.cache) HIP_TRY(hipMemset(s->p.cache, 0, ((size_t)s->p.cache_mask + 1) * 64));
  s->seq = 0;
  s->reclaim_count = 0; s->reclaim_capture_id = 0;
  HIP_TRY(hipMemset(s->p.reclaim_ctr, 0, 2 * sizeof(unsigned long long)));
// ... 121 lines not shown
  constexpr unsigned lds_pad = 0;
#endif
  const uint32_t helpers = s->p.seq ? (s->n_waves + kWavesPerTimingHelper - 1) / kWavesPerTimingHelper : 0u;
  auto launch = [&](auto kernel) {
    hipLaunchKernelGGL(kernel, dim3(s->n_waves + helpers), dim3(64), lds_pad, s->stream, s->p.slots, s->p.logprobs, s->p.q, s->p.n_waves, s->p.n_slots, s->p);
  };
  auto launch_gather = [&](auto kernel) {
    hipLaunchKernelGGL(kernel, dim3(s->n_waves + helpers), dim3(64), lds_pad, s->stream, s->p.slots, answers, inverse, n_unique, s->p.n_waves, s->p.n_slots, s->p);
  };
  const bool f32 = s->cfg.planes_dtype == 0;
#define C4_LAUNCH_STEP(KERNEL, LAUNCH)                                                                               \
  do {                                                                                                               \
    if (f32) {                                                                                                       \
      if (noise) { if (cache) LAUNCH(KERNEL<float, true, true>); else LAUNCH(KERNEL<float, true, false>); }          \
      else       { if (cache) LAUNCH(KERNEL<float, false, true>); else LAUNCH(KERNEL<float, false, false>); }        \
    } else {                                                                                                         \
      if (noise) { if (cache) LAUNCH(KERNEL<uint16_t, true, true>); else LAUNCH(KERNEL<uint16_t, true, false>); }    \
      else       { if (cache) LAUNCH(KERNEL<uint16_t, false, true>); else LAUNCH(KERNEL<uint16_t, false, false>); }  \
    }                                                                                                                \
  } while (0)
  if (search_mode(s)) {
    if (f32) launch(c4_step_kernel<float, false, false, true>); else launch(c4_step_kernel<uint16_t, false, false, true>);
  } else if (hold_mode(s)) {
    if (f32) launch(c4_step_kernel<float, false, false, false, true>); else launch(c4_step_kernel<uint16_t, false, false, false, true>);
  } else if (inverse) C4_LAUNCH_STEP(c4_step_gather_kernel, launch_gather); else C4_LAUNCH_STEP(c4_step_kernel, launch);
#undef C4_LAUNCH_STEP
  HIP_TRY(hipGetLastError());
  return maybe_reclaim(s);
}

int c4_session_step(c4_session* s) { return launch_step(s, nullptr, nullptr, 0); }

int c4_session_step_gather(c4_session* s, const uint32_t* inverse_dev, const float* answers, uint32_t n_unique) {
  if (!s || !inverse_dev || (!answers && n_unique)) return fail(C4_ERR_BAD_ARG, "null argument");
  if (search_mode(s)) return fail(C4_ERR_BAD_ARG, "c4_session_step_gather: a search session (C4_FLAG_SEARCH) takes a device evaluator, not the callback mode's batches");
  if (hold_mode(s)) return fail(C4_ERR_BAD_ARG, "c4_session_step_gather: a hold session (C4_FLAG_HOLD) takes a device evaluator, not the callback mode's batches");
  if (!s->bound) return fail(C4_ERR_NOT_BOUND, "c4_session_step_gather: bind_io first");
  void *inv = nullptr, *ans = nullptr;
  {
    C4_ON_DEVICE(s->cfg.device);
    if (int rc = device_view(inverse_dev, s->cfg.device, "c4_session_step_gather: inverse_dev", &inv)) return rc;
    if (answers) if (int rc = device_view(answers, s->cfg.device, "c4_session_step_gather: answers", &ans)) return rc;
  }
  return launch_step(s, (const uint32_t*)inv, (const float*)ans, n_unique);
}

int c4_session_step_head_out(c4_session* s, const void* hidden_policy_dev, const void* hidden_value_dev, const void* w_policy_dev,
                             const void* w_value_dev, const float* b_policy_dev, const float* b_value_dev, uint32_t features,
                             uint32_t policy_row_stride, uint32_t value_row_stride) {
  if (!s) return fail(C4_ERR_BAD_ARG, "null session");
  if (!s->bound || !s->have_games) return fail(C4_ERR_NOT_BOUND, "bind_io and set_games must precede step");
  if (!hidden_policy_dev || !hidden_value_dev || !w_policy_dev || !w_value_dev || !b_policy_dev || !b_value_dev)
    return fail(C4_ERR_BAD_ARG, "c4_session_step_head_out: null argument");
  if (features % 8 != 0 || policy_row_stride % 8 != 0 || value_row_stride % 8 != 0 || (features / 8) % (4 * c4ho::kHeadSteps * c4ho::kHeadWaves) != 0)
    return fail(C4_ERR_BAD_ARG, "c4_session_step_head_out: features must be a multiple of 1 344 (42 x 32 channels) and the row strides of 8 elements");
  if (s->p.dir_eps > 0.0f || s->p.cache != nullptr || s->timing)
    return fail(C4_ERR_BAD_ARG, "c4_session_step_head_out: the fused launch exists for the default configuration only (no Dirichlet noise, no evaluation "
                                "cache, per-launch timing off): call c4_head_out_bf16 and c4_session_step");
  C4_ON_DEVICE(s->cfg.device);
  s->p.seq = 0;
  const uint32_t groups = (s->p.n_slots + 15) / 16;
  auto launch = [&](auto kernel) {
    hipLaunchKernelGGL(kernel, dim3(groups), dim3(64 * c4ho::kHeadWaves), 0, s->stream, (const uint4*)hidden_policy_dev, (const uint4*)hidden_value_dev,
                       (const uint4*)w_policy_dev, (const uint4*)w_value_dev, b_policy_dev, b_value_dev, s->p.slots, s->p.n_slots, features / 8,
                       policy_row_stride / 8, value_row_stride / 8, s->p);
  };
  if (search_mode(s)) {
    if (s->cfg.planes_dtype == 0)
      return fail(C4_ERR_BAD_ARG, "c4_session_step_head_out: a search session's fused launch is built for bf16 planes (planes_dtype 1): call c4_head_out_bf16 and c4_session_step");
    if (s->out_step_gpw == 4) launch(c4_out_step_kernel<uint16_t, 4, true>); else launch(c4_out_step_kernel<uint16_t, 8, true>);
  } else if (hold_mode(s)) {
    if (s->cfg.planes_dtype == 0)
      return fail(C4_ERR_BAD_ARG, "c4_session_step_head_out: a hold session's fused launch is built for bf16 planes (planes_dtype 1): call c4_head_out_bf16 and c4_session_step");
    if (s->out_step_gpw == 4) launch(c4_out_step_kernel<uint16_t, 4, false, true>); else launch(c4_out_step_kernel<uint16_t, 8, false, true>);
  } else if (s->out_step_gpw == 4) {
    if (s->cfg.planes_dtype == 0) launch(c4_out_step_kernel<float, 4>); else launch(c4_out_step_kernel<uint16_t, 4>);
  } else {
    if (s->cfg.planes_dtype == 0) launch(c4_out_step_kernel<float, 8>); else launch(c4_out_step_kernel<uint16_t, 8>);
  }
  HIP_TRY(hipGetLastError());
  return maybe_reclaim(s);
}

int c4_session_set_step_shape(c4_session* s, uint32_t games_per_wavefront) {
  if (!s) return fail(C4_ERR_BAD_ARG, "null session");
  if (games_per_wavefront != 4 && games_per_wavefront != 8) return fail(C4_ERR_BAD_ARG, "c4_session_set_step_shape: games_per_wavefront must be 4 or 8");
  s->out_step_gpw = games_per_wavefront;
  return C4_OK;
}

int c4_session_set_timing(c4_session* s, int enable) {
  if (!s) return fail(C4_ERR_BAD_ARG, "null session");
  C4_ON_DEVICE(s->cfg.device);
  HIP_TRY(hipStreamSynchronize(s->stream));
  HIP_TRY(hipMemset(s->p.stamps, 0, (size_t)s->n_waves_cap * 4 * sizeof(unsigned long long)));
  if (enable && !s->timing) s->seq = 0;
  s->timing = enable != 0;
  return C4_OK;
}

int c4_session_counters(c4_session* s, c4_counters* out) {
  if (!s || !out) return fail(C4_ERR_BAD_ARG, "null argument");
  C4_ON_DEVICE(s->cfg.device);
  HIP_TRY(hipStreamSynchronize(s->stream));
  std::vector<unsigned long long> h((size_t)s->n_waves_cap * CTR_N);
  HIP_TRY(hipMemcpy(h.data(), s->p.wave_ctr, h.size() * sizeof(unsigned long long), hipMemcpyDeviceToHost));
  Globals g{};
  HIP_TRY(hipMemcpy(&g, s->p.glob, sizeof g, hipMemcpyDeviceToHost));
  unsigned long long sum[CTR_N] = {0};
  for (size_t w = 0; w < s->n_waves_cap; w++)
    for (int k = 0; k < CTR_N; k++) sum[k] += h[w * CTR_N + k];
  memset(out, 0, sizeof *out);
  out->sims = sum[CTR_SIMS]; out->select_levels = sum[CTR_S]; out->backup_nodes = sum[CTR_K];
  out->expansions = sum[CTR_E]; out->moves = sum[CTR_MOVES]; out->games_done = sum[CTR_DONE];
  out->ref_skipped_sims = sum[CTR_SKIPPED]; out->samples = sum[CTR_SAMPLES];
  out->eval_cache_probes = sum[CTR_PROBES]; out->eval_cache_hits = sum[CTR_HITS];
  out->games_started = g.queue_head < s->n_games ? g.queue_head : s->n_games;
  out->error = g.error; out->error_slot = g.error_slot;
  unsigned long long rc2[2] = {0, 0};
  HIP_TRY(hipMemcpy(rc2, s->p.reclaim_ctr, sizeof rc2, hipMemcpyDeviceToHost));
  out->reclaim_passes = rc2[0]; out->reclaim_blocks = rc2[1];
  unsigned long long acc[2] = {0, 0};
  HIP_TRY(hipMemcpy(acc, s->p.clock_acc, sizeof acc, hipMemcpyDeviceToHost));
  if (s->seq > 0) {
    std::vector<unsigned long long> st((size_t)s->n_waves * 2);
    HIP_TRY(hipMemcpy(st.data(), s->p.stamps + (size_t)(s->seq & 1) * s->n_waves * 2, st.size() * sizeof(unsigned long long), hipMemcpyDeviceToHost));
    unsigned long long lo = ~0ull, hi = 0ull;
    for (size_t w = 0; w < s->n_waves; w++) { if (st[2 * w] < lo) lo = st[2 * w]; if (st[2 * w + 1] > hi) hi = st[2 * w + 1]; }
    if (hi > lo) { acc[0] += hi - lo; acc[1] += 1; }
  }
  out->step_kernel_ns = acc[0] * 10ull;
  out->step_launches = acc[1];
  return C4_OK;
}

int c4_session_poll(c4_session* s, uint64_t* games_done, uint32_t* error) {
  if (!s) return fail(C4_ERR_BAD_ARG, "null session");
  C4_ON_DEVICE(s->cfg.device);
  if (s->probe_pending && hipEventQuery(s->probe_event) == hipSuccess) {
    s->probe_done = s->probe_host->games_done;
    s->probe_started = s->probe_host->queue_head < s->n_games ? s->probe_host->queue_head : s->n_games;
    s->probe_error = s->probe_host->error;
    if (s->probe_epoch == s->hold_epoch) {
      s->hold_probe_valid = true;
      s->hold_probe_active = s->probe_host->hold_active;
      s->hold_probe_need = s->probe_host->hold_need;
    }
    s->probe_pending = false;
  }
  if (!s->probe_pending) {
    HIP_TRY(hipMemcpyAsync(s->probe_host, s->p.glob, sizeof(Globals), hipMemcpyDeviceToHost, s->stream));
    HIP_TRY(hipEventRecord(s->probe_event, s->stream));
    s->probe_pending = true;
    s->probe_epoch = s->hold_epoch;
  }
  if (games_done) *games_done = s->probe_done;
  if (error) *error = s->probe_error;
  return C4_OK;
}

int c4_session_progress(c4_session* s, uint64_t* games_done, uint64_t* games_started, uint32_t* error) {
  const int rc = c4_session_poll(s, games_done, error);
  if (rc == C4_OK && games_started) *games_started = s->probe_started;
  return rc;
}

// ... 387 lines not shown
```

c4a0_amd/nn.py:

```python
from __future__ import annotations

import ctypes
import threading
import warnings
from dataclasses import dataclass
from typing import Optional, Tuple

import numpy as np
import torch
import torch.nn as nn
import torch.nn.functional as F

from ._lib import check, lib

N_COLS, N_ROWS = 7, 6


@dataclass
class ModelConfig:
    n_residual_blocks: int = 1
    conv_filter_size: int = 32
    n_policy_layers: int = 4
    n_value_layers: int = 2

# ... 222 lines not shown

    def np_planes(self, st: dict, bucket: int):
        return st["in"][:bucket]

    def tower(self, planes, config=0):
        x = planes.float().contiguous()
        g = x.shape[0]
        out = torch.empty((g, 42 * self.cp), dtype=torch.float32, device=self.device)
        work = torch.empty_like(out) if self.n_blocks else None
        check(self.L.c4_conv_tower_f32(x.data_ptr(), self.tw0.data_ptr(), self.tw.data_ptr(), self.tbias.data_ptr(), g, self.cp, self.n_blocks,
                                       out.data_ptr(), work.data_ptr() if work is not None else None, _stream(self.device)))
        return out

    def linear_relu(self, x, w, b, out=None, config=0):
        assert x.stride(1) == 1 and w.is_contiguous()
        m, (n, k) = x.shape[0], w.shape
        y = out if out is not None else torch.empty((m, n), dtype=torch.float32, device=self.device)
        check(self.L.c4_linear_f32(x.data_ptr(), w.data_ptr(), b.data_ptr(), y.data_ptr(), m, n, k, x.stride(0), y.stride(0), 1, _stream(self.device)))
        return y

    def head_out(self, p, v, out_logprobs=None, out_q=None, out_preact=None):
        g = p.shape[0]
        lp = out_logprobs if out_logprobs is not None else torch.empty((g, 7), dtype=torch.float32, device=self.device)
        q = out_q if out_q is not None else torch.empty((g, 2), dtype=torch.float32, device=self.device)
        assert p.stride(1) == 1 and v.stride(1) == 1
        check(self.L.c4_head_out_f32(p.data_ptr(), v.data_ptr(), self.pol_w[-1].data_ptr(), self.val_w[-1].data_ptr(),
                                     self.pol_b32.data_ptr(), self.val_b32.data_ptr(), g, self.pol_w[-1].shape[1], self.val_w[-1].shape[1], p.stride(0),
                                     v.stride(0), lp.data_ptr(), q.data_ptr(), out_preact.data_ptr() if out_preact is not None else None, _stream(self.device)))
        return lp, q


class EvaluatorFallbackWarning(UserWarning):
    """An InferenceNet on a HIP device that runs neither hand-written chain: not bf16 with 32 or 64 channels (the bf16 chain),
    and not f32 with hip_tower=True (the f32 chain, 1 to 64 channels), so PyTorch's kernels evaluate it."""


class InferenceNet:

    latency_mode = False
    graph_safe = True
    stage_hook = None
    _CHAIN_OPERANDS = frozenset(("tw0", "tw", "tbias", "conv_w", "conv_b", "pol_w", "pol_b", "val_w", "val_b", "pol_b32", "val_b32",
                                 "_bias32", "cp", "hp"))

    def __init__(self, model: ConnectFourNet, device: torch.device, dtype: torch.dtype = torch.bfloat16,
                 hip_tower: Optional[bool] = None, gemm: Optional[str] = None, gemm_config=None, tower_config: int = 0,
                 strict: bool = False):
        self.device, self.dtype = torch.device(device), dtype
        model = model.eval()
        self.channels = model.config.conv_filter_size
        self.n_blocks = len(model.conv) - 1
        f32 = dtype == torch.float32 and bool(hip_tower)
        if f32:
            if self.device.type != "cuda" or not 1 <= self.channels <= 64:
                raise ValueError("the f32 HIP evaluator needs a HIP device and 1 to 64 channels")
            if gemm not in (None, "hip") or gemm_config is not None or tower_config:
                raise ValueError("gemm / gemm_config / tower_config are bf16 switches: the f32 HIP evaluator has none")
        can_tower = self.device.type == "cuda" and ((dtype == torch.bfloat16 and self.channels in (32, 64)) or f32)
        if hip_tower and not can_tower:
            raise ValueError("hip_tower needs a HIP device, bf16 and 32 or 64 channels")
        self.hip_tower = can_tower if hip_tower is None else bool(hip_tower)
        if not self.hip_tower and hip_tower is None and self.device.type == "cuda":
            why = (f"{self.channels} channels (the HIP tower and GEMM are written for 32 and 64)" if dtype == torch.bfloat16
                   else f"dtype {dtype} (the default HIP kernels compute in bf16; f32 networks: hip_tower=True)")
            msg = (f"InferenceNet: {why}: this evaluator runs on PyTorch's convolutions and the library GEMM, not on the "
                   "hand-written HIP kernels -- slower, and a position's low bits depend on the batch it is evaluated in")
            if strict:
                raise ValueError(msg + " (strict=True)")
            warnings.warn(msg, EvaluatorFallbackWarning, stacklevel=2)
        folded = fold_network(model)
        gemm = gemm or ("hip" if self.hip_tower else "hipblaslt")
        if gemm not in ("hip", "hipblaslt"):
            raise ValueError("gemm must be 'hip' or 'hipblaslt'")
        if gemm == "hip" and not (self.hip_tower and (f32 or (42 * self.channels) % 192 == 0)):
            raise ValueError("gemm='hip' needs the HIP tower (bf16, 32 or 64 channels on a HIP device)")
        self.gemm = gemm
        if strict and gemm != "hip":
            raise ValueError("InferenceNet(strict=True): gemm='hipblaslt' leaves the hand-written GEMM (its low bits depend on the batch)")
        self.batch_invariant = self.hip_tower and gemm == "hip"
        cfg = str(gemm_config if gemm_config is not None else "0").split(",")
        self.gemm_config = (int(cfg[0]), int(cfg[-1]))
        self.tower_config = int(tower_config)
        self._np_lock = threading.Lock()
        ch = self.chain = (_F32Chain(folded, self.device) if f32 else _Bf16Chain(folded, self.device, hip_gemm=gemm == "hip") if self.hip_tower
                           else _TorchChain(folded, self.device, dtype))
        self.merged_w1 = self.merged_b1 = None
        if len(ch.pol_w) > 1 and len(ch.val_w) > 1:
            self.merged_w1 = torch.cat([ch.pol_w[0], ch.val_w[0]], dim=0).contiguous()
            self.merged_b1 = torch.cat([ch.pol_b[0], ch.val_b[0]], dim=0).contiguous()
            ch.hidden_bias_added(self.merged_b1)

    def __getattr__(self, name):
        if name in InferenceNet._CHAIN_OPERANDS and "chain" in self.__dict__:
            return getattr(self.chain, name)
        raise AttributeError(f"{type(self).__name__!r} object has no attribute {name!r}")

    @property
    def path(self) -> str:
        return "hip" if (self.hip_tower and self.gemm == "hip") else "torch"

    @torch.no_grad()
    def tower(self, planes: torch.Tensor, latency: Optional[bool] = None) -> torch.Tensor:
        latency = self.latency_mode if latency is None else latency
        config = self.tower_config or (2 if (latency and self.channels == 32 and 1024 < planes.shape[0] <= 2048) else 0)
        return self.chain.tower(planes, config)

    @torch.no_grad()
    def forward_hidden(self, planes: torch.Tensor, latency: Optional[bool] = None) -> Tuple[torch.Tensor, torch.Tensor]:
        hook, ch = self.stage_hook, self.chain
        if hook is not None:
            hook(0)
        x = self.tower(planes, latency)
        if hook is not None:
            hook(2)
        if self.merged_w1 is not None:
            h = self._linear_relu(x, self.merged_w1, self.merged_b1, latency=latency)
            f = self.merged_w1.shape[0] // 2
            p, v, rest = h[:, :f], h[:, f:], slice(1, -1)
        else:
            p, v, rest = x, x, slice(0, -1)
        if hook is not None:
            hook(1)
        for i, (w, b) in enumerate(zip(ch.pol_w[rest], ch.pol_b[rest])):
            p = self._linear_relu(p, w, b, latency=latency)
            if hook is not None:
                hook(3 + i)
        for w, b in zip(ch.val_w[rest], ch.val_b[rest]):
            v = self._linear_relu(v, w, b, latency=latency)
        return p, v

    @property
    def fused_step_ok(self) -> bool:
        own = type(self).forward is InferenceNet.forward and type(self).__call__ is InferenceNet.__call__
        return own and bool(self.hip_tower) and self.dtype == torch.bfloat16 and (42 * self.channels) % 1344 == 0

    def head_out_operands(self):
        ch = self.chain
        return ch.pol_w[-1], ch.val_w[-1], ch.pol_b32, ch.val_b32

    @torch.no_grad()
    def forward(self, planes: torch.Tensor, out_logprobs: Optional[torch.Tensor] = None,
                out_q: Optional[torch.Tensor] = None, latency: Optional[bool] = None) -> Tuple[torch.Tensor, torch.Tensor]:
        p, v = self.forward_hidden(planes, latency)
        return self.chain.head_out(p, v, out_logprobs, out_q)

    def _head_out_f32(self, p, v, out_logprobs=None, out_q=None, out_preact=None):
        return self.chain.head_out(p, v, out_logprobs, out_q, out_preact)

    _NP_BUCKET = 128

    @torch.no_grad()
    def forward_numpy(self, x):
        x = np.ascontiguousarray(x, dtype=np.float32)
        b = int(x.shape[0])
        if b == 0:
            return np.zeros((0, 7), np.float32), np.zeros((0,), np.float32), np.zeros((0,), np.float32)
        if self.chain.np_planes is None:
            lp, q = self.forward(torch.from_numpy(x).to(self.device))
            lp, q = lp.float().cpu().numpy(), q.float().cpu().numpy()
            return np.ascontiguousarray(lp), np.ascontiguousarray(q[:, 0]), np.ascontiguousarray(q[:, 1])
        if x.shape[1:] != (2, 6, 7):
            raise ValueError(f"forward_numpy: positions must be [B, 2, 6, 7], got {x.shape}")
        bucket = -(-b // self._NP_BUCKET) * self._NP_BUCKET
        with self._np_lock:
            return self._forward_numpy_locked(x, b, bucket)

    def _forward_numpy_locked(self, x, b: int, bucket: int):
        ch = self.chain
        st = getattr(self, "_np", None)
        if st is None or st["cap"] < bucket:
            cap = max(2048, 1 << (bucket - 1).bit_length())
            st = self._np = {"cap": cap, "graphs": {}, "stream": torch.cuda.Stream(device=self.device),
                             "in": torch.zeros((cap, 2, 6, 7), dtype=torch.float32, device=self.device),
                             "slot": torch.zeros(2, dtype=torch.int64).pin_memory(),
                             "h_lp": torch.zeros((cap, 7), dtype=torch.float32).pin_memory(),
                             "h_q": torch.zeros((cap, 2), dtype=torch.float32).pin_memory(),
                             "planes": torch.zeros((cap, 2, 6, 7), dtype=torch.bfloat16, device=self.device) if ch.np_converts else None}
            st["slot_np"] = st["slot"].numpy()
        stream = st["stream"]
        with torch.cuda.stream(stream):
            g = st["graphs"].get(bucket)
            if g is None:
                from .session import CAPTURE_ERROR_MODE

                def body():
                    self.forward(ch.np_planes(st, bucket), out_logprobs=st["h_lp"][:bucket], out_q=st["h_q"][:bucket], latency=True)

                st["slot_np"][0], st["slot_np"][1] = st["in"].data_ptr(), 0
                for _ in range(2):
                    body()
                stream.synchronize()
                g = torch.cuda.CUDAGraph()
                with torch.cuda.graph(g, stream=stream, capture_error_mode=CAPTURE_ERROR_MODE):
                    body()
                st["graphs"][bucket] = g
            if ch.np_converts and x.flags.writeable and x.ctypes.data % 16 == 0 and torch.from_numpy(x).is_pinned():
                st["slot_np"][0] = x.ctypes.data
            else:
                st["in"][:b].copy_(torch.from_numpy(x if x.flags.writeable else x.copy()), non_blocking=True)
                st["slot_np"][0] = st["in"].data_ptr()
            st["slot_np"][1] = b
            g.replay()
        stream.synchronize()
        lp, q = st["h_lp"].numpy()[:b], st["h_q"].numpy()[:b]
        return lp.copy(), np.ascontiguousarray(q[:, 0]), np.ascontiguousarray(q[:, 1])

    def _alone_config(self, m: int, n: int, k: int, latency: Optional[bool] = None) -> int:
        if not (self.latency_mode if latency is None else latency):
            return 0
        wide = n > k
        if k >= 2048:
            return 0 if (m <= 1024 or wide) else 11
        if m <= 1024:
            if not self.use_loader_waves:
                return 0
            if wide:
                return 41 if m <= 384 else (42 if m <= 576 else (44 if m <= 864 else 43))
# ... 49 lines not shown
```

c4a0_amd/session.py:

```python
from __future__ import annotations

import ctypes as C
import time
from typing import Callable, List, Optional, Sequence, Tuple

import numpy as np
import torch

from . import _lib
from ._lib import C4Error, Config, Counters, GameMetadataC, SampleRec, check

DeviceEvaluator = Callable[[torch.Tensor], Tuple[torch.Tensor, torch.Tensor]]
"""evaluator(planes[G,2,6,7]) -> (policy_logprobs[G,7] float32, q[G,2] float32) on the same device."""

CAPTURE_ERROR_MODE = "thread_local"


class _capture:

    def __init__(self, graph: "torch.cuda.CUDAGraph", stream: Optional[torch.cuda.Stream] = None):
        self.graph = graph
        self.stream = stream if stream is not None else torch.cuda.Stream()
        self.ctx = torch.cuda.stream(self.stream)

    def __enter__(self):
        self.ctx.__enter__()
        self.graph.capture_begin(capture_error_mode=CAPTURE_ERROR_MODE)

    def __exit__(self, *args):
        self.graph.capture_end()
        self.ctx.__exit__(*args)


def capture(graph: "torch.cuda.CUDAGraph", stream: Optional[torch.cuda.Stream] = None):
    return _capture(graph, stream) if LEAN_CAPTURE else torch.cuda.graph(graph, stream=stream, capture_error_mode=CAPTURE_ERROR_MODE)


LEAN_CAPTURE = True


class DeviceSession:
    def __init__(self, n_slots: int, n_mcts_iterations: int, c_exploration: float, c_ply_penalty: float,
                 device: Optional[torch.device] = None, planes_dtype: torch.dtype = torch.float32,
                 blocks_per_slot: int = 0, no_moves: bool = False, one_sim_per_step: bool = False,
                 reclaim: Optional[bool] = None, reclaim_period: int = 0, search: bool = False, hold: bool = False):
        if not torch.cuda.is_available():
            raise RuntimeError("c4a0_amd needs a HIP device: the tree kernels have no CPU fallback")
        self.L = _lib.lib()
        self.device = torch.device(device if device is not None else f"cuda:{torch.cuda.current_device()}")
        if self.device.type != "cuda":
            raise ValueError("device must be a cuda (HIP) device")
        dev_index = self.device.index if self.device.index is not None else torch.cuda.current_device()
        if planes_dtype not in (torch.float32, torch.bfloat16):
            raise ValueError("planes_dtype must be float32 or bfloat16")
        self.n_slots = int(n_slots)
        self.n_mcts_iterations = int(n_mcts_iterations)
        cfg = Config(self.n_slots, int(blocks_per_slot), self.n_mcts_iterations, float(c_exploration),
                     float(c_ply_penalty), 0 if planes_dtype == torch.float32 else 1,
                     (_lib.FLAG_NO_MOVES if no_moves else 0) | (_lib.FLAG_ONE_SIM_PER_STEP if one_sim_per_step else 0) |
                     (_lib.FLAG_RECLAIM if reclaim else (_lib.FLAG_NO_RECLAIM if reclaim is False else 0)) |
                     (_lib.FLAG_SEARCH if search else 0) | (_lib.FLAG_HOLD if hold else 0), dev_index, int(reclaim_period))
        self.search = bool(search)
        self.hold = bool(hold)
        h = C.c_void_p()
        check(self.L.c4_session_create(C.byref(cfg), C.byref(h)))
        self._h = h
        with torch.cuda.device(self.device):
            self.planes = torch.zeros((self.n_slots, 2, 6, 7), dtype=planes_dtype, device=self.device)
            self.logprobs = torch.zeros((self.n_slots, 7), dtype=torch.float32, device=self.device)
            self.q = torch.zeros((self.n_slots, 2), dtype=torch.float32, device=self.device)
        self.n_games = 0
        self.rows = self.n_slots
        self._bound_stream = None
        self._timing, self._extensions = True, False

    def close(self):
        if getattr(self, "_h", None):
            self.L.c4_session_destroy(self._h)
            self._h = None

    def __del__(self):
        try:
            self.close()
        except Exception:
            pass

    def set_games(self, reqs, start_positions: Optional[Sequence[Tuple[int, int]]] = None):
        if isinstance(reqs, np.ndarray):
            tab = np.ascontiguousarray(reqs, dtype=np.uint64).reshape(-1, 3)
        else:
            tab = np.array([(int(g), int(a), int(b)) for g, a, b in reqs], dtype=np.uint64).reshape(-1, 3)
        n = len(tab)
        arr = C.cast(tab.ctypes.data, C.POINTER(GameMetadataC)) if n else (GameMetadataC * 1)()
        sm = sv = None
        if start_positions is not None:
            if len(start_positions) != n:
                raise ValueError("start_positions must match reqs")
            if isinstance(start_positions, np.ndarray):
                cols = np.ascontiguousarray(start_positions, dtype=np.uint64).reshape(-1, 2)
                keep = (np.ascontiguousarray(cols[:, 0]), np.ascontiguousarray(cols[:, 1]))
                sm, sv = (C.cast(a.ctypes.data, C.POINTER(C.c_uint64)) if n else None for a in keep)
            else:
                sm = (C.c_uint64 * max(1, n))(*[int(m) for m, _ in start_positions])
                sv = (C.c_uint64 * max(1, n))(*[int(v) for _, v in start_positions])
        check(self.L.c4_session_set_games(self._h, arr, n, sm, sv))
        self.n_games = n
        self.rows = self.n_slots

    def bind(self, stream: Optional[torch.cuda.Stream] = None):
        st = stream if stream is not None else torch.cuda.current_stream(self.device)
        check(self.L.c4_session_bind_io(self._h, self.planes.data_ptr(), self.logprobs.data_ptr(), self.q.data_ptr(),
                                        C.c_void_p(st.cuda_stream)))
        self._bound_stream = st

    def set_dirichlet(self, alpha: float, epsilon: float):
        check(self.L.c4_session_set_dirichlet(self._h, float(alpha), float(epsilon)))
        self._extensions = self._extensions or float(epsilon) > 0.0

    def set_eval_cache(self, n_entries: int, max_sims_per_step: int = 0):
        check(self.L.c4_session_set_eval_cache(self._h, int(n_entries), int(max_sims_per_step)))
        self._extensions = self._extensions or int(n_entries) > 0

    def bind_leaf_models(self) -> torch.Tensor:
        models = torch.zeros(self.n_slots, dtype=torch.int64, device=self.device)
        check(self.L.c4_session_bind_leaf_models(self._h, C.c_void_p(models.data_ptr())))
        self.leaf_models = models
        return self.leaf_models

    def arena(self) -> dict:
        b, bps, half = C.c_uint64(), C.c_uint32(), C.c_uint32()
        check(self.L.c4_session_arena(self._h, C.byref(b), C.byref(bps), C.byref(half)))
        return {"bytes": b.value, "blocks_per_slot": bps.value, "reclaim_half_blocks": half.value}

    def start(self):
        check(self.L.c4_session_start(self._h))

    def step(self):
        check(self.L.c4_session_step(self._h))

    def set_timing(self, enable: bool):
        check(self.L.c4_session_set_timing(self._h, 1 if enable else 0))
        self._timing = bool(enable)

    def set_step_shape(self, games_per_wavefront: int):
        if not hasattr(self.L, "c4_session_set_step_shape"):
            return
        check(self.L.c4_session_set_step_shape(self._h, int(games_per_wavefront)))

    def round(self, evaluator: DeviceEvaluator):
        if (self.fuse_output_step and not self._timing and not self._extensions and getattr(self, "leaf_models", None) is None
                and getattr(evaluator, "fused_step_ok", False) and not ((self.search or self.hold) and self.planes.dtype != torch.bfloat16)):
            r = self.rows
            p, v = evaluator.forward_hidden(self.planes if r == self.n_slots else self.planes[:r])
            wp, wv, bp, bv = evaluator.head_out_operands()
            assert p.stride(1) == 1 and v.stride(1) == 1 and p.shape[0] == r
            check(self.L.c4_session_step_head_out(self._h, C.c_void_p(p.data_ptr()), C.c_void_p(v.data_ptr()), C.c_void_p(wp.data_ptr()),
                                                  C.c_void_p(wv.data_ptr()), C.c_void_p(bp.data_ptr()), C.c_void_p(bv.data_ptr()),
                                                  p.shape[1], p.stride(0), v.stride(0)))
            return
        if hasattr(evaluator, "round") and getattr(evaluator, "s", None) is self:
            evaluator.round()
            return
        self.evaluate(evaluator)
        self.step()

    def capture_steps(self, evaluator: DeviceEvaluator, steps_per_graph: int = 8,
                      stream: Optional[torch.cuda.Stream] = None) -> "torch.cuda.CUDAGraph":
        self.set_timing(False)
        main = stream if stream is not None else torch.cuda.current_stream(self.device)
        side = torch.cuda.Stream(device=self.device)
        side.wait_stream(main)
        with torch.cuda.stream(side):
            self.bind(side)
            for _ in range(2):
                self.evaluate(evaluator)
        main.wait_stream(side)
        torch.cuda.synchronize(self.device)
        graph = torch.cuda.CUDAGraph()
        with capture(graph, stream if stream is not None else torch.cuda.Stream(device=self.device)):
            self.bind(torch.cuda.current_stream(self.device))
            for _ in range(steps_per_graph):
                self.round(evaluator)
        self.bind(main)
        return graph

    def counters(self) -> dict:
        c = Counters()
        check(self.L.c4_session_counters(self._h, C.byref(c)))
        return c.as_dict()

    def poll(self) -> Tuple[int, int]:
        done, err = C.c_uint64(), C.c_uint32()
        check(self.L.c4_session_poll(self._h, C.byref(done), C.byref(err)))
        return done.value, err.value

    def progress(self) -> Tuple[int, int, int]:
        done, started, err = C.c_uint64(), C.c_uint64(), C.c_uint32()
        check(self.L.c4_session_progress(self._h, C.byref(done), C.byref(started), C.byref(err)))
        return done.value, started.value, err.value

    def compact(self, multiple: int = 256) -> Tuple[int, int]:
        act, rows = C.c_uint32(), C.c_uint32()
        check(self.L.c4_session_compact(self._h, int(multiple), C.byref(act), C.byref(rows)))
        self.rows = rows.value
        return act.value, rows.value

    def raise_if_device_error(self):
        c = self.counters()
        if c["error"]:
            raise C4Error(c["error"], f"raised on device by slot {c['error_slot']}")

    def sample_counts(self) -> np.ndarray:
        out = np.zeros(max(1, self.n_games), dtype=np.uint32)
        check(self.L.c4_session_sample_counts(self._h, out.ctypes.data_as(C.POINTER(C.c_uint32)), self.n_games))
        return out[: self.n_games]

    def drain_samples(self) -> np.ndarray:
        n = C.c_uint64()
        check(self.L.c4_session_drain_samples(self._h, None, 0, C.byref(n)))
        buf = np.zeros(max(1, n.value), dtype=SAMPLE_DTYPE)
        check(self.L.c4_session_drain_samples(self._h, buf.ctypes.data_as(C.POINTER(SampleRec)), n.value, C.byref(n)))
        return buf[: n.value]

    def pack_samples_device(self) -> torch.Tensor:
        n = C.c_uint64()
        check(self.L.c4_session_pack_samples(self._h, None, 0, C.byref(n)))
        out = torch.empty((max(1, n.value), 64), dtype=torch.uint8, device=self.device)
        if n.value:
            check(self.L.c4_session_pack_samples(self._h, C.c_void_p(out.data_ptr()), n.value, C.byref(n)))
        return out[: n.value]

    def set_iterations(self, n: int):
        check(self.L.c4_session_set_iterations(self._h, int(n)))

    def hold_resume(self, cols: Optional[torch.Tensor] = None, temperatures: Optional[torch.Tensor] = None,
                    results: Optional[torch.Tensor] = None):
        ptr = lambda t: C.c_void_p(t.data_ptr()) if t is not None else None
        check(self.L.c4_session_hold_resume(self._h, ptr(cols), ptr(temperatures), ptr(results)))

    def snapshot(self) -> Tuple[np.ndarray, np.ndarray, np.ndarray]:
        recs = np.zeros(self.n_slots, dtype=SAMPLE_DTYPE)
        visits, status = np.zeros(self.n_slots, dtype=np.uint32), np.zeros(self.n_slots, dtype=np.uint32)
        check(self.L.c4_session_snapshot(self._h, recs.ctypes.data, visits.ctypes.data, status.ctypes.data, self.n_slots))
        return recs, visits, status

    def hold_poll(self) -> Tuple[Optional[int], Optional[int], int]:
        act, need, err = C.c_uint32(), C.c_uint32(), C.c_uint32()
        check(self.L.c4_session_hold_poll(self._h, C.byref(act), C.byref(need), C.byref(err)))
        known = act.value != _lib.HOLD_POLL_UNKNOWN
        return (act.value if known else None), (need.value if known else None), err.value

    def root_stats(self, slot: int = 0):
        pol = (C.c_float * 7)()
        qp, qn = C.c_float(), C.c_float()
        n, m, v = C.c_uint64(), C.c_uint64(), C.c_uint64()
        check(self.L.c4_session_root_stats(self._h, slot, pol, C.byref(qp), C.byref(qn), C.byref(n), C.byref(m), C.byref(v)))
        return np.array(pol[:], dtype=np.float32), qp.value, qn.value, n.value, (m.value, v.value)

    def leaves(self, with_ordinals: bool = False):
        m = np.zeros(self.n_slots, dtype=np.uint64)
        v = np.zeros(self.n_slots, dtype=np.uint64)
        s = np.zeros(self.n_slots, dtype=np.uint32)
        o = np.zeros(self.n_slots, dtype=np.uint32)
        check(self.L.c4_session_leaves(self._h, m.ctypes.data_as(C.POINTER(C.c_uint64)), v.ctypes.data_as(C.POINTER(C.c_uint64)),
                                       s.ctypes.data_as(C.POINTER(C.c_uint32)), o.ctypes.data_as(C.POINTER(C.c_uint32))))
        return (m, v, s, o) if with_ordinals else (m, v, s)

    def evaluate(self, evaluator: DeviceEvaluator):
        r = self.rows
        planes, logprobs, q = (self.planes, self.logprobs, self.q) if r == self.n_slots else (self.planes[:r], self.logprobs[:r], self.q[:r])
        if getattr(evaluator, "graph_safe", False):
            evaluator(planes, out_logprobs=logprobs, out_q=q)
            return
        lp, q_out = evaluator(planes)
        if lp.data_ptr() != logprobs.data_ptr():
            logprobs.copy_(lp.reshape(r, 7))
        if q_out.data_ptr() != q.data_ptr():
            q.copy_(q_out.reshape(r, 2))

    fuse_output_step = True
    NARROW_CHECK_ROUNDS = 64

    def wants_narrowing(self, multiple: int = 256, asynchronous: bool = False) -> bool:
        if getattr(self, "leaf_models", None) is not None or self.rows <= multiple:
            return False
        if asynchronous:
            done, started, _err = self.progress()
        else:
            c = self.counters()
            done, started = c["games_done"], c["games_started"]
        return started >= self.n_games and (self.n_games - done) <= self.rows // 2

    def narrow_if_worthwhile(self, multiple: int = 256, asynchronous: bool = False) -> bool:
        if not self.wants_narrowing(multiple, asynchronous):
            return False
        before = self.rows
        self.compact(multiple)
        return self.rows != before

    def run(self, evaluator: DeviceEvaluator, max_steps: Optional[int] = None, poll_every: int = 16,
            on_step: Optional[Callable[[int], None]] = None, steps_per_graph: int = 0, phases: Optional[dict] = None,
            tail_steps_per_graph: int = 0) -> int:
        self.bind()
        self.start()
        steps = 0
        t_c = time.perf_counter()
        graph = self.capture_steps(evaluator, steps_per_graph) if steps_per_graph > 0 else None
        if phases is not None:
            phases.update(first_capture_s=time.perf_counter() - t_c, recapture_s=0.0, captures=1 if graph is not None else 0, t_loop0=time.perf_counter())
        max_chunks_in_flight = 2
        inflight = []
        chunks = 0
        while True:
            if graph is not None:
                graph.replay()
                steps += steps_per_graph
                chunk_end = True
            else:
                if on_step is not None:
                    self.evaluate(evaluator)
                    on_step(steps)
                    self.step()
                else:
                    self.round(evaluator)
                steps += 1
                chunk_end = steps % poll_every == 0
            if chunk_end:
                ev = torch.cuda.Event()
                ev.record(torch.cuda.current_stream(self.device))
                inflight.append(ev)
                if len(inflight) > max_chunks_in_flight:
                    inflight.pop(0).synchronize()
                done, started, err = self.progress()
                if err:
                    self.raise_if_device_error()
                if phases is not None and started >= self.n_games and "t_all_started" not in phases:
                    phases["t_all_started"], phases["steps_all_started"] = time.perf_counter(), steps
                if done >= self.n_games:
                    break
                chunks += 1
                if graph is not None and chunks % max(1, self.NARROW_CHECK_ROUNDS // steps_per_graph) == 0 and \
                        self.narrow_if_worthwhile(asynchronous=bool(getattr(evaluator, "batch_invariant", False))):
                    inflight.clear()
                    t_c = time.perf_counter()
                    steps_per_graph = int(tail_steps_per_graph or steps_per_graph)
                    graph = self.capture_steps(evaluator, steps_per_graph)
                    if phases is not None:
                        phases["recapture_s"] += time.perf_counter() - t_c
                        phases["captures"] += 1
                        phases.setdefault("narrowings", []).append((steps, [self.rows]))
            if max_steps is not None and steps >= max_steps:
                break
        if graph is not None:
            torch.cuda.synchronize(self.device)
            self.set_timing(True)
        c = self.counters()
        if c["error"]:
            raise C4Error(c["error"], f"raised on device by slot {c['error_slot']}")
        return steps


PAIRED_STEP_GAMES_PER_WAVEFRONT = 4


def capture_pair(sessions: Sequence["DeviceSession"], streams: Sequence[torch.cuda.Stream], evaluator, steps_per_graph: int = 32,
                 strict: bool = False, offset_stage: int = 1) -> "torch.cuda.CUDAGraph":
    a, b = sessions
    s0, s1 = streams
    dev = a.device
    for s in sessions:
        s.set_timing(False)
        s.set_step_shape(PAIRED_STEP_GAMES_PER_WAVEFRONT)
    for s, st in zip(sessions, streams):
        side = torch.cuda.Stream(device=dev)
        side.wait_stream(st)
        with torch.cuda.stream(side):
            s.bind(side)
            for _ in range(2):
                s.evaluate(evaluator)
        st.wait_stream(side)
    torch.cuda.synchronize(dev)
    graph = torch.cuda.CUDAGraph()
    prev_hook = getattr(evaluator, "stage_hook", None)
    try:
        with capture(graph, s0):
            a.bind(s0)
            b.bind(s1)
            s1.wait_stream(s0)
            ev_b_prev = None
            for r in range(steps_per_graph):
                ev_a, ev_b = torch.cuda.Event(), torch.cuda.Event()
                free = not strict

                def hook_a(stage, ev_a=ev_a, wait_for=ev_b_prev, free=free, r=r):
                    if free:
                        if r == 0 and stage == offset_stage:
                            ev_a.record(s0)
                        return
                    if stage == 0 and wait_for is not None:
                        s0.wait_event(wait_for)
                    elif stage == 1:
                        ev_a.record(s0)

                def hook_b(stage, ev_a=ev_a, ev_b=ev_b, free=free, r=r):
                    if free:
                        if r == 0 and stage == 0:
                            s1.wait_event(ev_a)
                        return
                    if stage == 0:
                        s1.wait_event(ev_a)
                    elif stage == 1:
                        ev_b.record(s1)

                evaluator.stage_hook = hook_a
                with torch.cuda.stream(s0):
                    a.round(evaluator)
                evaluator.stage_hook = hook_b
                with torch.cuda.stream(s1):
                    b.round(evaluator)
                ev_b_prev = ev_b
            s0.wait_stream(s1)
    finally:
        evaluator.stage_hook = prev_hook
    return graph


def run_sessions(sessions: Sequence["DeviceSession"], evaluator: DeviceEvaluator, steps_per_graph: int = 8,
                 max_chunks_in_flight: int = 2, paired: Optional[bool] = None, phases: Optional[dict] = None,
                 tail_steps_per_graph: Optional[int] = None) -> List[int]:
    dev = sessions[0].device
    streams = [torch.cuda.Stream(device=dev) for _ in sessions]
    cur = torch.cuda.current_stream(dev)
    invariant = bool(getattr(evaluator, "batch_invariant", False))
    paired = len(sessions) == 2 and hasattr(evaluator, "stage_hook") and paired is not False
    graphs = []
    for s, st in zip(sessions, streams):
        st.wait_stream(cur)
        with torch.cuda.stream(st):
            s.bind(st)
            s.start()
        st.synchronize()
        if not paired:
            graphs.append(s.capture_steps(evaluator, steps_per_graph, stream=st))
    if paired:
        return _run_pair(sessions, streams, evaluator, steps_per_graph, max_chunks_in_flight, invariant, phases, tail_steps_per_graph)
    steps = [0] * len(sessions)
    chunks = [0] * len(sessions)
    live = [s.n_games > 0 for s in sessions]
    inflight: List[List[torch.cuda.Event]] = [[] for _ in sessions]
    while any(live):
        for i, (s, st, g) in enumerate(zip(sessions, streams, graphs)):
            if not live[i]:
                continue
            with torch.cuda.stream(st):
                g.replay()
                ev = torch.cuda.Event()
                ev.record(st)
                steps[i] += steps_per_graph
                inflight[i].append(ev)
                if len(inflight[i]) > max_chunks_in_flight:
                    inflight[i].pop(0).synchronize()
                done, err = s.poll()
            if err:
                torch.cuda.synchronize(dev)
                s.raise_if_device_error()
            chunks[i] += 1
            if done >= s.n_games:
                live[i] = False
            elif chunks[i] % max(1, s.NARROW_CHECK_ROUNDS // steps_per_graph) == 0 and s.narrow_if_worthwhile(asynchronous=invariant):
                inflight[i].clear()
                graphs[i] = s.capture_steps(evaluator, steps_per_graph, stream=st)
    torch.cuda.synchronize(dev)
    for s in sessions:
        s.set_timing(True)
        s.raise_if_device_error()
    return steps


def _run_pair(sessions, streams, evaluator, steps_per_graph, max_chunks_in_flight, invariant, phases=None, tail_steps_per_graph=None) -> List[int]:
    dev = sessions[0].device
    t_c = time.perf_counter()
    graph = capture_pair(sessions, streams, evaluator, steps_per_graph)
    if phases is not None:
        phases.update(first_capture_s=time.perf_counter() - t_c, recapture_s=0.0, captures=1, t_loop0=time.perf_counter())
    per_graph = steps_per_graph
    tail_steps = int(tail_steps_per_graph or steps_per_graph)
    steps = 0
    since_check = 0
    inflight: List[torch.cuda.Event] = []
    while True:
        with torch.cuda.stream(streams[0]):
            graph.replay()
            ev = torch.cuda.Event()
            ev.record(streams[0])
        steps += per_graph
        since_check += per_graph
        inflight.append(ev)
        if len(inflight) > max_chunks_in_flight:
            inflight.pop(0).synchronize()
        done_all, started_all = True, True
        for s, st in zip(sessions, streams):
            with torch.cuda.stream(st):
# ... 41 lines not shown
```

include/c4a0_hip.h:

```cpp
#ifndef C4A0_HIP_H
#define C4A0_HIP_H

#include <stddef.h>
#include <stdint.h>

#ifdef __cplusplus
extern "C" {
#endif

#define C4_ABI_VERSION 13

#define C4_N_COLS 7
#define C4_N_ROWS 6
#define C4_BUF_N_CHANNELS 2
#define C4_PLANES_LEN 84
#define C4_MAX_SAMPLES_PER_GAME 43

typedef enum {
  C4_OK = 0,
  C4_ERR_BAD_ARG = 1,
  C4_ERR_HIP = 2,
  C4_ERR_NAN_IN_TREE = 3,
  C4_ERR_DEGENERATE_POLICY = 4,
  C4_ERR_ARENA_OVERFLOW = 5,
  C4_ERR_NOT_BOUND = 6,
  C4_ERR_NO_DEVICE = 7,
  C4_ERR_ILLEGAL_MOVE = 8,
  C4_ERR_CANCELLED = 9
} c4_status;

typedef struct {
  uint64_t game_id;
  uint64_t player0_id;
  uint64_t player1_id;
} c4_game_metadata;

typedef struct {
  uint64_t game_id;
  uint64_t mask;
  uint64_t value;
  float policy[7];
  float q_penalty;
  float q_no_penalty;
  uint32_t meta;
} c4_sample_rec;

typedef struct {
  uint32_t n_slots;
  uint32_t blocks_per_slot;
  uint32_t n_mcts_iterations;
  float c_exploration;
  float c_ply_penalty;
  uint32_t planes_dtype;
  uint32_t flags;
  int32_t device;
  uint32_t reclaim_period;
} c4_config;

#define C4_FLAG_NO_MOVES 1u
#define C4_FLAG_ONE_SIM_PER_STEP 2u

#define C4_FLAG_RECLAIM 4u

#define C4_FLAG_NO_RECLAIM 8u

#define C4_FLAG_SEARCH 16u

#define C4_FLAG_HOLD 32u
#define C4_HOLD_PARKED 64u
#define C4_HOLD_MOVE_NONE (-1)
#define C4_HOLD_MOVE_SAMPLE (-2)
#define C4_HOLD_OK 0
#define C4_HOLD_REFUSED_TERMINAL 1
#define C4_HOLD_REFUSED_COLUMN 2
#define C4_HOLD_REFUSED_UNSEARCHED 3
#define C4_HOLD_REFUSED_SAMPLE 4
#define C4_HOLD_NO_GAME 5
#define C4_HOLD_POLL_UNKNOWN 0xFFFFFFFFu

typedef struct {
  uint64_t sims;
  uint64_t select_levels;
  uint64_t backup_nodes;
  uint64_t expansions;
  uint64_t moves;
  uint64_t games_done;
  uint64_t ref_skipped_sims;
  uint64_t samples;
  uint64_t games_started;
  uint64_t step_kernel_ns;
  uint64_t step_launches;
  uint64_t eval_cache_probes;
  uint64_t eval_cache_hits;
  uint64_t reclaim_passes;
  uint64_t reclaim_blocks;
  uint32_t error;
  uint32_t error_slot;
} c4_counters;

typedef struct c4_session c4_session;

const char* c4_last_error_string(void);
int c4_abi_version(void);
const char* c4_source_hash(void);
int c4_device_count(int* out);

int c4_session_create(const c4_config* cfg, c4_session** out);
int c4_session_destroy(c4_session* s);
int c4_trim_cached_memory(void);

int c4_session_set_games(c4_session* s, const c4_game_metadata* reqs, uint64_t n_games,
                         const uint64_t* start_masks, const uint64_t* start_values);

int c4_session_bind_io(c4_session* s, void* planes_dev, const float* logprobs_dev, const float* q_dev,
                       void* stream);

int c4_session_set_dirichlet(c4_session* s, float alpha, float epsilon);

int c4_session_bind_leaf_models(c4_session* s, uint64_t* leaf_models_dev);

int c4_session_set_eval_cache(c4_session* s, uint64_t n_entries, uint32_t max_sims_per_step);

int c4_session_start(c4_session* s);

int c4_session_step(c4_session* s);


int c4_session_step_head_out(c4_session* s, const void* hidden_policy_dev, const void* hidden_value_dev, const void* w_policy_dev,
                             const void* w_value_dev, const float* b_policy_dev, const float* b_value_dev, uint32_t features,
                             uint32_t policy_row_stride, uint32_t value_row_stride);
int c4_session_set_step_shape(c4_session* s, uint32_t games_per_wavefront);

int c4_session_set_timing(c4_session* s, int enable);

int c4_session_counters(c4_session* s, c4_counters* out);
int c4_session_poll(c4_session* s, uint64_t* games_done, uint32_t* error);
int c4_session_progress(c4_session* s, uint64_t* games_done, uint64_t* games_started, uint32_t* error);

int c4_session_compact(c4_session* s, uint32_t multiple, uint32_t* n_active, uint32_t* n_slots_now);

int c4_session_arena(c4_session* s, uint64_t* bytes, uint32_t* blocks_per_slot, uint32_t* reclaim_half_blocks);
int c4_session_sample_counts(c4_session* s, uint32_t* counts_host, uint64_t n_games);
int c4_session_drain_samples(c4_session* s, c4_sample_rec* dst_host, uint64_t cap, uint64_t* n_written);
int c4_session_pack_samples(c4_session* s, c4_sample_rec* dst_dev, uint64_t cap, uint64_t* n_written);
int c4_session_debug_phase_stamps(c4_session* s, uint64_t* out_host, uint64_t cap_words, uint64_t* n_words);
int c4_session_sample_store(c4_session* s, const c4_sample_rec** recs_dev, const uint32_t** counts_dev, uint64_t* n_games);

typedef struct {
  uint32_t channels;
  uint32_t n_blocks;
  const void* tower_w0;
  const void* tower_w;
  const float* tower_bias;
  const void* w1;
  const float* b1;
  uint32_t n_policy_hidden;
  uint32_t n_value_hidden;
  const void* policy_w[8];
  const float* policy_b[8];
  const void* value_w[8];
  const float* value_b[8];
  const void* policy_out_w;
  const void* value_out_w;
  const float* policy_out_b;
  const float* value_out_b;
} c4_network_bf16;

typedef struct {
  int32_t device;
  uint32_t resident_games;
  uint32_t concurrent_sessions;
  uint32_t steps_per_graph;
  uint32_t tail_steps_per_graph;
  uint32_t blocks_per_slot;
  uint32_t flags;
  uint32_t reclaim_period;
  float dirichlet_alpha;
  float dirichlet_epsilon;
  uint64_t eval_cache_entries;
} c4_play_options;

typedef struct {
  double setup_s;
  double capture_s;
  double steady_s;
  double tail_s;
  double drain_s;
  uint64_t rounds;
  uint64_t rounds_until_all_started;
  uint32_t graph_captures;
  uint32_t resident_games;
  uint32_t sessions;
  uint32_t rows_at_end;
} c4_play_phases;

int c4_play_games_bf16(const c4_game_metadata* reqs, uint64_t n_games, uint32_t n_mcts_iterations, float c_exploration,
                       float c_ply_penalty, const c4_network_bf16* net, const c4_play_options* options, uint32_t* counts_host,
                       c4_sample_rec* records_host, uint64_t records_cap, uint64_t* n_records, c4_counters* totals,
                       c4_play_phases* phases);
int c4_search_positions_bf16(const uint64_t* masks, const uint64_t* values, uint64_t n_positions, uint32_t n_mcts_iterations,
                             float c_exploration, float c_ply_penalty, const c4_network_bf16* net, const c4_play_options* options,
                             c4_sample_rec* records, uint64_t records_cap, c4_counters* totals, c4_play_phases* phases);
void c4_play_games_cancel(void);

int c4_records_to_cbor(const c4_game_metadata* metas, const uint32_t* counts, uint64_t n_games, const c4_sample_rec* recs,
                       uint64_t n_records, uint8_t* dst, uint64_t cap, uint64_t* n_written);
int c4_cbor_to_records(const uint8_t* src, uint64_t len, c4_game_metadata* metas, uint32_t* counts, uint64_t cap_games,
                       c4_sample_rec* recs, uint64_t cap_records, uint64_t* n_games, uint64_t* n_records);

int c4_shuffle_games(uint64_t seed, uint64_t n_games, uint32_t* order);

int c4_session_root_stats(c4_session* s, uint32_t slot, float policy[7], float* q_penalty,
                          float* q_no_penalty, uint64_t* visit_count, uint64_t* root_mask, uint64_t* root_value);
// ... 65 lines not shown
```

Before: 28830.

## Fuse next round's conv tower into the head-out/MCTS step kernel

Adds a kernel that runs the output heads and MCTS step and then, in the same launch, runs the conv tower on the freshly written leaf planes for the next round. The tower output is handed to the evaluator so the next forward skips its own tower launch. The staged-weight tower path moves into a shared header and the output layers' LDS reuses the idle weight stage. This removes a kernel launch and a round-trip of the planes per round, but it adds cache-invalidation bookkeeping keyed on buffer pointers, and the fused kernel needs enough LDS for both stages.

```diff
diff --git a/c4a0_amd/_lib.py b/c4a0_amd/_lib.py
--- a/c4a0_amd/_lib.py
+++ b/c4a0_amd/_lib.py
@@ -22,7 +22,7 @@
 HOLD_OK, HOLD_REFUSED_TERMINAL, HOLD_REFUSED_COLUMN, HOLD_REFUSED_UNSEARCHED, HOLD_REFUSED_SAMPLE, HOLD_NO_GAME = range(6)
 HOLD_POLL_UNKNOWN = 0xFFFFFFFF
 MAX_SAMPLES_PER_GAME = 43
-ABI_VERSION = 13
+ABI_VERSION = 14
 STRUCT_LAYOUT_SINCE = 7
 
 
@@ -99,6 +99,7 @@
     "c4_session_step": (C.c_int, [_vp]),
     "c4_session_set_step_shape": (C.c_int, [_vp, C.c_uint32]),
     "c4_session_step_head_out": (C.c_int, [_vp, _vp, _vp, _vp, _vp, _vp, _vp, C.c_uint32, C.c_uint32, C.c_uint32]),
+    "c4_session_step_head_out_tower": (C.c_int, [_vp, _vp, _vp, _vp, _vp, _vp, _vp, C.c_uint32, C.c_uint32, C.c_uint32, _vp, _vp, _vp, C.c_uint32, C.c_uint32, _vp]),
     "c4_session_set_timing": (C.c_int, [_vp, C.c_int]),
     "c4_session_counters": (C.c_int, [_vp, _P(Counters)]),
     "c4_session_poll": (C.c_int, [_vp, _P(C.c_uint64), _P(C.c_uint32)]),
diff --git a/c4a0_amd/csrc/build.py b/c4a0_amd/csrc/build.py
--- a/c4a0_amd/csrc/build.py
+++ b/c4a0_amd/csrc/build.py
@@ -7,7 +7,7 @@
 PKG = os.path.dirname(HERE)
 OUT = os.path.join(PKG, "libc4a0_hip.so")
 SRCS = [os.path.join(HERE, "c4_session.hip"), os.path.join(HERE, "c4_conv_tower.hip"), os.path.join(HERE, "c4_head_gemm.hip"), os.path.join(HERE, "c4_results_host.hip"), os.path.join(HERE, "c4_selfplay_host.hip"), os.path.join(HERE, "c4_f32_net.hip")]
-DEPS = SRCS + [os.path.join(HERE, "c4_device.hpp"), os.path.join(HERE, "c4_host.hpp"), os.path.join(HERE, "c4_head_out.hpp"), os.path.join(HERE, "c4_timeline.hpp"),
+DEPS = SRCS + [os.path.join(HERE, "c4_device.hpp"), os.path.join(HERE, "c4_host.hpp"), os.path.join(HERE, "c4_head_out.hpp"), os.path.join(HERE, "c4_timeline.hpp"), os.path.join(HERE, "c4_tower.hpp"),
                os.path.join(os.path.dirname(PKG), "include", "c4a0_hip.h")]
 FLAGS = ["--offload-arch=gfx950", "-O3", "-std=c++17", "-fPIC", "-shared", "-ffp-contract=off",
          "-fno-fast-math", "-Wall", "-Wno-unused-function",
diff --git a/c4a0_amd/csrc/c4_conv_tower.hip b/c4a0_amd/csrc/c4_conv_tower.hip
--- a/c4a0_amd/csrc/c4_conv_tower.hip
+++ b/c4a0_amd/csrc/c4_conv_tower.hip
@@ -10,6 +10,7 @@
 #include "c4_head_out.hpp"
 #include "c4_host.hpp"
 #include "c4_timeline.hpp"
+#include "c4_tower.hpp"
 
 #ifndef C4_TOWER_PAIR_SAME_SIMD
 #define C4_TOWER_PAIR_SAME_SIMD 0
@@ -20,29 +21,7 @@
 
 namespace {
 
-typedef __bf16 bf16x8 __attribute__((ext_vector_type(8)));
-typedef __bf16 bf16x4 __attribute__((ext_vector_type(4)));
-typedef float f32x4 __attribute__((ext_vector_type(4)));
-
-constexpr int kBS = 56;
-constexpr int kTilesPerBoard = 3;
-
-__device__ __forceinline__ int cell_slot(int r, int c) { return (r + 1) * 8 + (c + 1) + 1; }
-
-template <int C, int NB>
-struct Geo {
-  static constexpr int KG = C / 8;
-  static constexpr int MT = C / 16;
-  static constexpr int KC = C / 32;
-  static constexpr int kPlane = (NB * kBS + 10 + 15) / 16 * 16;
-  static constexpr int kBufSlots = KG * kPlane;
-  static constexpr bool kStageW = (C == 32);
-  static constexpr int kWFrags = 9 * MT * KC;
-  static constexpr int kLdsBytes = 2 * kBufSlots * 16 + (kStageW ? 2 * kWFrags * 1024 : 0);
-  static constexpr int kTiles = NB * kTilesPerBoard;
-  static_assert((kPlane * 16) % 256 == 0, "channel-group planes must keep the bank phase");
-  static_assert(kLdsBytes <= 160 * 1024, "LDS budget");
-};
+using namespace c4tw;
 
 #ifdef C4_PHASE_STAMPS
 __device__ unsigned long long c4_tower_clk[80];
@@ -50,131 +29,6 @@
 #else
 #define C4_TSTAMP(i) do { } while (0)
 #endif
-
-struct TowerParams {
-  const uint16_t* planes;
-  const bf16x8* w0;
-  const bf16x8* w;
-  const float* bias;
-  uint16_t* out;
-  uint32_t n_boards;
-  uint32_t n_blocks;
-};
-
-template <int C, int NB, bool kConv0, bool kSecond, bool kLast, int G_TILES, int MTW, bool kPrefetch, typename WF, typename Hook>
-__device__ __forceinline__ void tower_layer(const uint4* __restrict__ src, uint4* __restrict__ dst, WF& wf,
-                                            const float* __restrict__ bias, int tile_lo, int m0, int lane, Hook&& after_last_tile,
-                                            uint16_t* __restrict__ out = nullptr, uint32_t board0 = 0, uint32_t n_boards = 0) {
-  using G = Geo<C, NB>;
-  constexpr int kSteps = kConv0 ? 3 : 9 * G::KC;
-  constexpr int NF = kPrefetch ? 2 : 1;
-  const int li = lane & 15, lg = lane >> 4;
-
-  f32x4 bias4[MTW];
-#pragma unroll
-  for (int m = 0; m < MTW; m++) {
-    const float* bp = bias + 16 * (m0 + m) + 4 * lg;
-    bias4[m] = f32x4{bp[0], bp[1], bp[2], bp[3]};
-  }
-
-  uint4 fr[NF][kSteps];
-  f32x4 acc[2][MTW];
-  uint2 old[2][MTW];
-  int e_slot[2], e_cell[2];
-  int e_board[2];
-
-  auto tile_cell = [&](int g, int& cell) __attribute__((always_inline)) {
-    const int tl = tile_lo + g;
-    const int bidx = tl / kTilesPerBoard;
-    const int slot = 9 + 16 * (tl - bidx * kTilesPerBoard) + li;
-    cell = slot;
-    return bidx * kBS + slot;
-  };
-  auto load_frags = [&](int g, int f) __attribute__((always_inline)) {
-    int cell;
-    const int base = tile_cell(g, cell);
-#pragma unroll
-    for (int k = 0; k < kSteps; k++) {
-      int d, plane;
-      if (kConv0) {
-        int tap = 4 * k + lg;
-        tap = tap < 9 ? tap : 4;
-        d = 8 * (tap / 3 - 1) + (tap % 3 - 1);
-        plane = 0;
-      } else {
-        const int t = k / G::KC, kc = k % G::KC;
-        d = 8 * (t / 3 - 1) + (t % 3 - 1);
-        plane = 4 * kc + lg;
-      }
-      fr[f][k] = src[plane * G::kPlane + base + d];
-    }
-  };
-  auto out_ptr = [&](int slot_in_plane, int m) __attribute__((always_inline)) {
-    return reinterpret_cast<uint2*>(&dst[(2 * (m0 + m) + (lg >> 1)) * G::kPlane + slot_in_plane]) + (lg & 1);
-  };
-  auto start_tile = [&](int g, int a) __attribute__((always_inline)) {
-    e_slot[a] = tile_cell(g, e_cell[a]);
-    e_board[a] = (tile_lo + g) / kTilesPerBoard;
-#pragma unroll
-    for (int m = 0; m < MTW; m++) {
-      acc[a][m] = bias4[m];
-      if (kSecond && kPrefetch) old[a][m] = *out_ptr(e_slot[a], m);
-    }
-  };
-  auto mfmas = [&](int f, int a) __attribute__((always_inline)) {
-#pragma unroll
-    for (int k = 0; k < kSteps; k++) {
-#pragma unroll
-      for (int m = 0; m < MTW; m++)
-        acc[a][m] = __builtin_amdgcn_mfma_f32_16x16x32_bf16(wf[k][m], __builtin_bit_cast(bf16x8, fr[f][k]), acc[a][m], 0, 0, 0);
-    }
-  };
-  auto epilogue = [&](int a) __attribute__((always_inline)) {
-    const bool valid = ((e_cell[a] - 1) & 7) != 0;
-#pragma unroll
-    for (int m = 0; m < MTW; m++) {
-      f32x4 v = acc[a][m];
-      if (kSecond) {
-        const uint2 o = kPrefetch ? old[a][m] : *out_ptr(e_slot[a], m);
-        const float o0 = __uint_as_float(o.x << 16), o1 = __uint_as_float(o.x & 0xffff0000u);
-        const float o2 = __uint_as_float(o.y << 16), o3 = __uint_as_float(o.y & 0xffff0000u);
-        v[0] = o0 + fmaxf(v[0], 0.f); v[1] = o1 + fmaxf(v[1], 0.f);
-        v[2] = o2 + fmaxf(v[2], 0.f); v[3] = o3 + fmaxf(v[3], 0.f);
-      }
-      const bf16x4 o = __builtin_convertvector(v, bf16x4);
-      if (kLast) {
-        const int rc = e_cell[a] - 1, cell = 7 * ((rc >> 3) - 1) + (rc & 7) - 1;
-        const uint32_t gb = board0 + (uint32_t)e_board[a];
-        if (valid && gb < n_boards)
-          *reinterpret_cast<uint2*>(out + ((size_t)gb * 42 + cell) * C + 16 * (m0 + m) + 4 * lg) = __builtin_bit_cast(uint2, o);
-      } else if (valid) {
-        *out_ptr(e_slot[a], m) = __builtin_bit_cast(uint2, o);
-      }
-    }
-  };
-
-  load_frags(0, 0);
-  if (kPrefetch) {
-#pragma unroll
-    for (int g = 0; g < G_TILES; g++) {
-      const int a = g & 1, f = g & 1;
-      start_tile(g, a);
-      if (g + 1 < G_TILES) load_frags(g + 1, f ^ 1);
-      mfmas(f, a);
-      if (g >= 1) epilogue(a ^ 1);
-    }
-    epilogue((G_TILES - 1) & 1);
-  } else {
-#pragma unroll
-    for (int g = 0; g < G_TILES; g++) {
-      start_tile(g, 0);
-      mfmas(0, 0);
-      epilogue(0);
-      if (g + 1 < G_TILES) load_frags(g + 1, 0);
-    }
-  }
-  after_last_tile();
-}
 
 struct NoStamp { __device__ __forceinline__ void operator()(int) const {} };
 struct NoFeed { static constexpr bool kRing = false; };
@@ -352,14 +206,6 @@
   stamp(2);
 }
 
-template <int KW, int NWAVES>
-__device__ __forceinline__ void dma_weights(const void* w, uint32_t bytes, uint4* lds_dst, int first_frag, int wave, int lane) {
-  const auto rsrc = __builtin_amdgcn_make_buffer_rsrc(const_cast<void*>(w), 0, (int)bytes, 0x00020000);
-  const int wave_u = __builtin_amdgcn_readfirstlane(wave);
-  for (int c = wave_u; c < KW; c += NWAVES)
-    __builtin_amdgcn_raw_ptr_buffer_load_lds(rsrc, (__attribute__((address_space(3))) void*)(lds_dst + c * 64), 16, lane * 16, (first_frag + c) * 1024, 0, 0);
-}
-
 template <int C, int NB, int NT, int MS, bool ST = false, int KD = 3, bool RG = false>
 __global__ __launch_bounds__(NT) void c4_conv_tower_kernel(const uint16_t* __restrict__ a_planes, const bf16x8* __restrict__ a_w0, const bf16x8* __restrict__ a_w,
                                                              const float* __restrict__ a_bias, uint16_t* __restrict__ a_out, uint32_t a_n_boards, uint32_t a_n_blocks) {
@@ -404,6 +250,33 @@
   const int m0 = grp_member * MTW;
   const uint32_t board0 = blockIdx.x * NB;
 
+  if constexpr (G::kStageW && !ST) {
+    using S = StagedTower<C, NB, NT>;
+    typename S::WF wf;
+    uint32_t in_v[S::kIn];
+    S::load_conv0_weights(wf, p, lane);
+    S::template stage_layer_weights<NT / 64>(p, lds_raw, 1, wave, lane);
+    S::load_input(p, board0, tid, in_v);
+    S::template zero_images<NT>(lds_raw, tid);
+    __syncthreads();
+    S::store_input(lds_raw, tid, in_v);
+    __syncthreads();
+    C4_TSTAMP(1);
+    auto stamp = [&](int i) __attribute__((always_inline)) {
+#ifdef C4_PHASE_STAMPS
+      if (i < 22) C4_TSTAMP(i);
+#endif
+    };
+    if (S::layers(p, lds_raw, wf, board0, tid, stamp)) {
+#ifdef C4_PHASE_STAMPS
+      asm volatile("s_waitcnt vmcnt(0)" ::: "memory");
+      const int last = 2 + 2 * (int)p.n_blocks;
+      if (last < 22) { C4_TSTAMP(last); tw_flush(last); }
+#endif
+      C4_TL_END(1, p.out);
+      return;
+    }
+  } else {
   constexpr int kWSteps = 9 * G::KC;
   bf16x8 wf[kWSteps][MTW];
 #pragma unroll
@@ -425,20 +298,6 @@
 #pragma unroll
       for (int m = 0; m < MTW; m++) wf[k][m] = wl[(((k / G::KC) * G::MT + m0 + m) * G::KC + (k % G::KC)) * 64 + lane];
   };
-  uint4* Wst = T + G::kBufSlots;
-  auto stage_layer_weights = [&](int layer) __attribute__((always_inline)) {
-    if (layer <= n_layers)
-      dma_weights<G::kWFrags, NT / 64>(p.w, 2u * p.n_blocks * G::kWFrags * 1024u, Wst + (layer & 1) * G::kWFrags * 64, (layer - 1) * G::kWFrags, wave, lane);
-  };
-  auto fetch_staged_weights = [&](int layer) __attribute__((always_inline)) {
-    const uint4* ws = Wst + (layer & 1) * G::kWFrags * 64;
-#pragma unroll
-    for (int k = 0; k < kWSteps; k++)
-#pragma unroll
-      for (int m = 0; m < MTW; m++)
-        wf[k][m] = __builtin_bit_cast(bf16x8, ws[(((k / G::KC) * G::MT + m0 + m) * G::KC + (k % G::KC)) * 64 + lane]);
-  };
-  if (G::kStageW && !ST) stage_layer_weights(1);
 
   constexpr int kIn = (NB * 42 + NT - 1) / NT;
   uint32_t in_v[kIn];
@@ -466,8 +325,6 @@
   constexpr int kWaves = NT / 64 / MS;
   static_assert(G::kTiles % kWaves == 0, "every wavefront owns the same number of cell tiles");
   constexpr int kTilesPerWave = G::kTiles / kWaves;
-  constexpr bool kPrefetch = (C == 32);
-  constexpr bool kFuseOut = (C == 32);
   const int tile_lo = grp_index * kTilesPerWave;
 
   if constexpr (ST && RG) {
@@ -560,38 +417,23 @@
 #endif
     }
   } else {
-  tower_layer<C, NB, true, false, false, kTilesPerWave, MTW, kPrefetch>(T, X, wf, p.bias, tile_lo, m0, lane, [&]() __attribute__((always_inline)) {
-    if (!G::kStageW && n_layers >= 1) load_layer_weights(1);
+  tower_layer<C, NB, true, false, false, kTilesPerWave, MTW, false>(T, X, wf, p.bias, tile_lo, m0, lane, [&]() __attribute__((always_inline)) {
+    if (n_layers >= 1) load_layer_weights(1);
   });
-  if (G::kStageW) asm volatile("s_waitcnt vmcnt(0)" ::: "memory");
   __syncthreads();
   C4_TSTAMP(2);
   for (int layer = 1; layer <= n_layers; layer++) {
     const bool is_second = (layer & 1) == 0;
-    if (G::kStageW) {
-      stage_layer_weights(layer + 1);
-      fetch_staged_weights(layer);
-    }
     auto next_weights = [&]() __attribute__((always_inline)) {
-      if (!G::kStageW && layer < n_layers) load_layer_weights(layer + 1);
+      if (layer < n_layers) load_layer_weights(layer + 1);
     };
-    if (kFuseOut && layer == n_layers) {
-      tower_layer<C, NB, false, true, true, kTilesPerWave, MTW, kPrefetch>(T, X, wf, p.bias + (size_t)layer * C, tile_lo, m0, lane, next_weights,
-                                                                          p.out, board0, p.n_boards);
-#ifdef C4_PHASE_STAMPS
-      asm volatile("s_waitcnt vmcnt(0)" ::: "memory");
-      if (layer < 20) { C4_TSTAMP(2 + layer); tw_flush(2 + layer); }
-#endif
-      C4_TL_END(1, p.out);
-      return;
-    }
-    if (is_second) tower_layer<C, NB, false, true, false, kTilesPerWave, MTW, kPrefetch>(T, X, wf, p.bias + (size_t)layer * C, tile_lo, m0, lane, next_weights);
-    else tower_layer<C, NB, false, false, false, kTilesPerWave, MTW, kPrefetch>(X, T, wf, p.bias + (size_t)layer * C, tile_lo, m0, lane, next_weights);
-    if (G::kStageW) asm volatile("s_waitcnt vmcnt(0)" ::: "memory");
+    if (is_second) tower_layer<C, NB, false, true, false, kTilesPerWave, MTW, false>(T, X, wf, p.bias + (size_t)layer * C, tile_lo, m0, lane, next_weights);
+    else tower_layer<C, NB, false, false, false, kTilesPerWave, MTW, false>(X, T, wf, p.bias + (size_t)layer * C, tile_lo, m0, lane, next_weights);
     __syncthreads();
 #ifdef C4_PHASE_STAMPS
     if (layer < 20) C4_TSTAMP(2 + layer);
 #endif
+  }
   }
   }
 
diff --git a/c4a0_amd/csrc/c4_head_out.hpp b/c4a0_amd/csrc/c4_head_out.hpp
--- a/c4a0_amd/csrc/c4_head_out.hpp
+++ b/c4a0_amd/csrc/c4_head_out.hpp
@@ -29,7 +29,7 @@
   const uint4* wpl = wp + (size_t)(row < 7 ? row : 0) * f8 + kq;
   const uint4* wvl = wv + (size_t)(row < 2 ? row : 0) * f8 + kq;
   f32x4 accp = {0.f, 0.f, 0.f, 0.f}, accv = {0.f, 0.f, 0.f, 0.f};
-  const uint32_t n_iter = f8 / (4 * kHeadSteps * kHeadWaves);
+  const uint32_t n_iter = wave < kHeadWaves ? f8 / (4 * kHeadSteps * kHeadWaves) : 0;
   for (uint32_t it = 0; it < n_iter; it++) {
     const uint32_t s0 = (it * kHeadWaves + wave) * kHeadSteps;
     uint4 a_p[kHeadSteps], a_v[kHeadSteps], b_p[kHeadSteps], b_v[kHeadSteps];
@@ -53,8 +53,10 @@
       accv = __builtin_amdgcn_mfma_f32_16x16x32_bf16(__builtin_bit_cast(bf16x8, a_v[s]), __builtin_bit_cast(bf16x8, b_v[s]), accv, 0, 0, 0);
     }
   }
-  sh.part[wave][0][lane] = accp;
-  sh.part[wave][1][lane] = accv;
+  if (wave < kHeadWaves) {
+    sh.part[wave][0][lane] = accp;
+    sh.part[wave][1][lane] = accv;
+  }
   __syncthreads();
   if (wave < 2) {
     f32x4 sum = sh.part[0][wave][lane];
diff --git a/c4a0_amd/csrc/c4_session.hip b/c4a0_amd/csrc/c4_session.hip
--- a/c4a0_amd/csrc/c4_session.hip
+++ b/c4a0_amd/csrc/c4_session.hip
@@ -14,6 +14,7 @@
 #include "c4_head_out.hpp"
 #include "c4_host.hpp"
 #include "c4_timeline.hpp"
+#include "c4_tower.hpp"
 
 #pragma clang fp contract(off)
 
@@ -872,6 +873,57 @@
   C4_TL_END(3, a_slots);
 }
 
+using FusedTower = c4tw::StagedTower<32, 16, 512>;
+constexpr int kFusedTowerLds = c4tw::Geo<32, 16>::kLdsBytes;
+static_assert(sizeof(c4ho::Shared) <= (size_t)FusedTower::kFreeUntilLayer1Bytes, "the output layers' LDS fits in the idle weight stage");
+template <uint32_t kGpw>
+__global__ __launch_bounds__(512) void c4_out_step_tower_kernel(
+    const uint4* __restrict__ hp, const uint4* __restrict__ hv, const uint4* __restrict__ wp, const uint4* __restrict__ wv,
+    const float* __restrict__ bp, const float* __restrict__ bv, Slot* __restrict__ a_slots, uint32_t a_n_slots, uint32_t f8, uint32_t sp8, uint32_t sv8,
+    const c4tw::bf16x8* tw0, const c4tw::bf16x8* tw, const float* tbias, uint16_t* tout, uint32_t n_blocks, Params p) {
+  extern __shared__ __attribute__((aligned(256))) uint8_t c4_fused_lds[];
+  c4ho::Shared& sh = *reinterpret_cast<c4ho::Shared*>(c4_fused_lds + FusedTower::kFreeUntilLayer1);
+  C4_TL_BEGIN();
+  constexpr uint32_t kStepWaves = 16 / kGpw;
+  static_assert(kGpw == 8 || kGpw == 4, "16 games per workgroup on two or four stepping wavefronts");
+  const uint32_t lane = threadIdx.x & 63, wave = threadIdx.x >> 6, sub = lane & 7, grp = lane >> 3;
+  const uint32_t b = wave * kGpw + grp;
+  const bool mine = wave < kStepWaves && grp < kGpw;
+  const uint32_t g = mine ? blockIdx.x * 16 + b : a_n_slots;
+  const uint32_t wave_index = blockIdx.x * 2 + wave / (kStepWaves / 2);
+  const uint32_t gs = g < a_n_slots ? g : 0;
+  Slot* st = a_slots + gs;
+  uint4 hot = make_uint4(0, 0, 0, 0);
+  if (wave < kStepWaves) hot = reinterpret_cast<const uint4*>(st)[sub];
+  c4ho::head_out_block<16>(sh, hp, hv, wp, wv, bp, bv, a_n_slots, f8, sp8, sv8, const_cast<float*>(p.logprobs), const_cast<float*>(p.q), blockIdx.x);
+  __syncthreads();
+  const c4tw::TowerParams tp{reinterpret_cast<const uint16_t*>(p.planes), tw0, tw, tbias, tout, a_n_slots, n_blocks};
+  if (wave < kStepWaves) {
+    if (wave_index < p.n_waves) {
+      const float nn_logit = sh.res[b & 15][sub < 7 ? sub : 6];
+      const float nn_q = sh.res[b & 15][7 + (sub & 1)];
+      step_body<uint16_t, false, false>(p, wave_index, lane, a_n_slots, st, hot, nn_logit, nn_q, 0ull, g);
+    }
+    asm volatile("s_waitcnt vmcnt(0)" ::: "memory");
+    __builtin_amdgcn_fence(__ATOMIC_RELEASE, "workgroup");
+  } else {
+    constexpr int kIdle = 8 - (int)kStepWaves;
+    FusedTower::stage_layer_weights<kIdle>(tp, c4_fused_lds, 1, (int)(wave - kStepWaves), (int)lane);
+    FusedTower::zero_images<64 * kIdle>(c4_fused_lds, (int)(threadIdx.x - 64 * kStepWaves));
+  }
+  __syncthreads();
+  __builtin_amdgcn_fence(__ATOMIC_ACQUIRE, "workgroup");
+  const uint32_t board0 = blockIdx.x * 16;
+  FusedTower::WF wf;
+  uint32_t in_v[FusedTower::kIn];
+  FusedTower::load_conv0_weights(wf, tp, (int)lane);
+  FusedTower::load_input(tp, board0, (int)threadIdx.x, in_v);
+  FusedTower::store_input(c4_fused_lds, (int)threadIdx.x, in_v);
+  __syncthreads();
+  FusedTower::layers(tp, c4_fused_lds, wf, board0, (int)threadIdx.x, [](int) {});
+  C4_TL_END(3, a_slots);
+}
+
 __global__ void k_pos_ops(const uint64_t* mask, const uint64_t* value, const int32_t* col, uint64_t n, float c_ply,
                           uint64_t* om, uint64_t* ov, uint32_t* olegal, uint32_t* oterm, float* oq) {
   const uint64_t i = (uint64_t)blockIdx.x * blockDim.x + threadIdx.x;
@@ -1454,6 +1506,8 @@
   return C4_OK;
 }
 
+static hipError_t fused_tower_opt_in(int device);
+
 int c4_session_create(const c4_config* cfg, c4_session** out) {
   if (!cfg || !out) return fail(C4_ERR_BAD_ARG, "null argument");
   *out = nullptr;
@@ -1499,6 +1553,10 @@
     const std::string msg = g_last_error;
     c4_session_destroy(s);
     return fail(rc, msg);
+  }
+  if (cfg->planes_dtype == 1 && !search_mode(s) && !hold_mode(s)) {
+    c4host::DeviceGuard guard(s->cfg.device);
+    if (guard.error() == hipSuccess) (void)fused_tower_opt_in(s->cfg.device);
   }
   *out = s;
   return C4_OK;
@@ -1786,6 +1844,51 @@
   return maybe_reclaim(s);
 }
 
+static hipError_t fused_tower_opt_in(int device) {
+  hipError_t e = c4host::opt_in_lds((const void*)c4_out_step_tower_kernel<8>, kFusedTowerLds, device);
+  if (e == hipSuccess) e = c4host::opt_in_lds((const void*)c4_out_step_tower_kernel<4>, kFusedTowerLds, device);
+  return e;
+}
+
+int c4_session_step_head_out_tower(c4_session* s, const void* hidden_policy_dev, const void* hidden_value_dev, const void* w_policy_dev,
+                                   const void* w_value_dev, const float* b_policy_dev, const float* b_value_dev, uint32_t features,
+                                   uint32_t policy_row_stride, uint32_t value_row_stride, const void* tower_w0_dev, const void* tower_w_dev,
+                                   const float* tower_bias_dev, uint32_t channels, uint32_t n_blocks, void* tower_out_dev) {
+  if (!s) return fail(C4_ERR_BAD_ARG, "null session");
+  if (!s->bound || !s->have_games) return fail(C4_ERR_NOT_BOUND, "bind_io and set_games must precede step");
+  if (!hidden_policy_dev || !hidden_value_dev || !w_policy_dev || !w_value_dev || !b_policy_dev || !b_value_dev || !tower_w0_dev || !tower_w_dev ||
+      !tower_bias_dev || !tower_out_dev)
+    return fail(C4_ERR_BAD_ARG, "c4_session_step_head_out_tower: null argument");
+  if (features % 8 != 0 || policy_row_stride % 8 != 0 || value_row_stride % 8 != 0 || (features / 8) % (4 * c4ho::kHeadSteps * c4ho::kHeadWaves) != 0)
+    return fail(C4_ERR_BAD_ARG, "c4_session_step_head_out_tower: features must be a multiple of 1 344 (42 x 32 channels) and the row strides of 8 elements");
+  if (s->p.dir_eps > 0.0f || s->p.cache != nullptr || s->timing)
+    return fail(C4_ERR_BAD_ARG, "c4_session_step_head_out_tower: the fused launch exists for the default configuration only (no Dirichlet noise, no evaluation "
+                                "cache, per-launch timing off): call c4_head_out_bf16, c4_session_step and c4_conv_tower_bf16");
+  if (search_mode(s) || hold_mode(s) || s->p.leaf_models)
+    return fail(C4_ERR_BAD_ARG, "c4_session_step_head_out_tower: not built for search sessions, hold sessions or multi-model games: call c4_session_step_head_out "
+                                "and c4_conv_tower_bf16");
+  if (channels != 32 || n_blocks == 0)
+    return fail(C4_ERR_BAD_ARG, "c4_session_step_head_out_tower: the fused tower is the 32-channel one with at least one residual block: call "
+                                "c4_session_step_head_out and c4_conv_tower_bf16");
+  if (s->cfg.planes_dtype != 1)
+    return fail(C4_ERR_BAD_ARG, "c4_session_step_head_out_tower: the fused tower reads bf16 planes (planes_dtype 1): call c4_session_step_head_out and "
+                                "c4_conv_tower_bf16");
+  C4_ON_DEVICE(s->cfg.device);
+  if (const hipError_t e = fused_tower_opt_in(s->cfg.device); e != hipSuccess)
+    return fail(C4_ERR_HIP, std::string("c4_session_step_head_out_tower: LDS opt-in: ") + hipGetErrorString(e));
+  s->p.seq = 0;
+  const uint32_t groups = (s->p.n_slots + 15) / 16;
+  auto launch = [&](auto kernel) {
+    hipLaunchKernelGGL(kernel, dim3(groups), dim3(512), kFusedTowerLds, s->stream, (const uint4*)hidden_policy_dev, (const uint4*)hidden_value_dev,
+                       (const uint4*)w_policy_dev, (const uint4*)w_value_dev, b_policy_dev, b_value_dev, s->p.slots, s->p.n_slots, features / 8,
+                       policy_row_stride / 8, value_row_stride / 8, (const c4tw::bf16x8*)tower_w0_dev, (const c4tw::bf16x8*)tower_w_dev, tower_bias_dev,
+                       (uint16_t*)tower_out_dev, n_blocks, s->p);
+  };
+  if (s->out_step_gpw == 4) launch(c4_out_step_tower_kernel<4>); else launch(c4_out_step_tower_kernel<8>);
+  HIP_TRY(hipGetLastError());
+  return maybe_reclaim(s);
+}
+
 int c4_session_set_step_shape(c4_session* s, uint32_t games_per_wavefront) {
   if (!s) return fail(C4_ERR_BAD_ARG, "null session");
   if (games_per_wavefront != 4 && games_per_wavefront != 8) return fail(C4_ERR_BAD_ARG, "c4_session_set_step_shape: games_per_wavefront must be 4 or 8");
diff --git a/c4a0_amd/csrc/c4_tower.hpp b/c4a0_amd/csrc/c4_tower.hpp
--- /dev/null
+++ b/c4a0_amd/csrc/c4_tower.hpp
@@ -0,0 +1,252 @@
+#pragma once
+#include <hip/hip_runtime.h>
+#include <stdint.h>
+
+namespace c4tw {
+
+typedef __bf16 bf16x8 __attribute__((ext_vector_type(8)));
+typedef __bf16 bf16x4 __attribute__((ext_vector_type(4)));
+typedef float f32x4 __attribute__((ext_vector_type(4)));
+
+constexpr int kBS = 56;
+constexpr int kTilesPerBoard = 3;
+
+__device__ __forceinline__ int cell_slot(int r, int c) { return (r + 1) * 8 + (c + 1) + 1; }
+
+template <int C, int NB>
+struct Geo {
+  static constexpr int KG = C / 8;
+  static constexpr int MT = C / 16;
+  static constexpr int KC = C / 32;
+  static constexpr int kPlane = (NB * kBS + 10 + 15) / 16 * 16;
+  static constexpr int kBufSlots = KG * kPlane;
+  static constexpr bool kStageW = (C == 32);
+  static constexpr int kWFrags = 9 * MT * KC;
+  static constexpr int kLdsBytes = 2 * kBufSlots * 16 + (kStageW ? 2 * kWFrags * 1024 : 0);
+  static constexpr int kTiles = NB * kTilesPerBoard;
+  static_assert((kPlane * 16) % 256 == 0, "channel-group planes must keep the bank phase");
+  static_assert(kLdsBytes <= 160 * 1024, "LDS budget");
+};
+
+struct TowerParams {
+  const uint16_t* planes;
+  const bf16x8* w0;
+  const bf16x8* w;
+  const float* bias;
+  uint16_t* out;
+  uint32_t n_boards;
+  uint32_t n_blocks;
+};
+
+template <int C, int NB, bool kConv0, bool kSecond, bool kLast, int G_TILES, int MTW, bool kPrefetch, typename WF, typename Hook>
+__device__ __forceinline__ void tower_layer(const uint4* __restrict__ src, uint4* __restrict__ dst, WF& wf,
+                                            const float* __restrict__ bias, int tile_lo, int m0, int lane, Hook&& after_last_tile,
+                                            uint16_t* __restrict__ out = nullptr, uint32_t board0 = 0, uint32_t n_boards = 0) {
+  using G = Geo<C, NB>;
+  constexpr int kSteps = kConv0 ? 3 : 9 * G::KC;
+  constexpr int NF = kPrefetch ? 2 : 1;
+  const int li = lane & 15, lg = lane >> 4;
+
+  f32x4 bias4[MTW];
+#pragma unroll
+  for (int m = 0; m < MTW; m++) {
+    const float* bp = bias + 16 * (m0 + m) + 4 * lg;
+    bias4[m] = f32x4{bp[0], bp[1], bp[2], bp[3]};
+  }
+
+  uint4 fr[NF][kSteps];
+  f32x4 acc[2][MTW];
+  uint2 old[2][MTW];
+  int e_slot[2], e_cell[2];
+  int e_board[2];
+
+  auto tile_cell = [&](int g, int& cell) __attribute__((always_inline)) {
+    const int tl = tile_lo + g;
+    const int bidx = tl / kTilesPerBoard;
+    const int slot = 9 + 16 * (tl - bidx * kTilesPerBoard) + li;
+    cell = slot;
+    return bidx * kBS + slot;
+  };
+  auto load_frags = [&](int g, int f) __attribute__((always_inline)) {
+    int cell;
+    const int base = tile_cell(g, cell);
+#pragma unroll
+    for (int k = 0; k < kSteps; k++) {
+      int d, plane;
+      if (kConv0) {
+        int tap = 4 * k + lg;
+        tap = tap < 9 ? tap : 4;
+        d = 8 * (tap / 3 - 1) + (tap % 3 - 1);
+        plane = 0;
+      } else {
+        const int t = k / G::KC, kc = k % G::KC;
+        d = 8 * (t / 3 - 1) + (t % 3 - 1);
+        plane = 4 * kc + lg;
+      }
+      fr[f][k] = src[plane * G::kPlane + base + d];
+    }
+  };
+  auto out_ptr = [&](int slot_in_plane, int m) __attribute__((always_inline)) {
+    return reinterpret_cast<uint2*>(&dst[(2 * (m0 + m) + (lg >> 1)) * G::kPlane + slot_in_plane]) + (lg & 1);
+  };
+  auto start_tile = [&](int g, int a) __attribute__((always_inline)) {
+    e_slot[a] = tile_cell(g, e_cell[a]);
+    e_board[a] = (tile_lo + g) / kTilesPerBoard;
+#pragma unroll
+    for (int m = 0; m < MTW; m++) {
+      acc[a][m] = bias4[m];
+      if (kSecond && kPrefetch) old[a][m] = *out_ptr(e_slot[a], m);
+    }
+  };
+  auto mfmas = [&](int f, int a) __attribute__((always_inline)) {
+#pragma unroll
+    for (int k = 0; k < kSteps; k++) {
+#pragma unroll
+      for (int m = 0; m < MTW; m++)
+        acc[a][m] = __builtin_amdgcn_mfma_f32_16x16x32_bf16(wf[k][m], __builtin_bit_cast(bf16x8, fr[f][k]), acc[a][m], 0, 0, 0);
+    }
+  };
+  auto epilogue = [&](int a) __attribute__((always_inline)) {
+    const bool valid = ((e_cell[a] - 1) & 7) != 0;
+#pragma unroll
+    for (int m = 0; m < MTW; m++) {
+      f32x4 v = acc[a][m];
+      if (kSecond) {
+        const uint2 o = kPrefetch ? old[a][m] : *out_ptr(e_slot[a], m);
+        const float o0 = __uint_as_float(o.x << 16), o1 = __uint_as_float(o.x & 0xffff0000u);
+        const float o2 = __uint_as_float(o.y << 16), o3 = __uint_as_float(o.y & 0xffff0000u);
+        v[0] = o0 + fmaxf(v[0], 0.f); v[1] = o1 + fmaxf(v[1], 0.f);
+        v[2] = o2 + fmaxf(v[2], 0.f); v[3] = o3 + fmaxf(v[3], 0.f);
+      }
+      const bf16x4 o = __builtin_convertvector(v, bf16x4);
+      if (kLast) {
+        const int rc = e_cell[a] - 1, cell = 7 * ((rc >> 3) - 1) + (rc & 7) - 1;
+        const uint32_t gb = board0 + (uint32_t)e_board[a];
+        if (valid && gb < n_boards)
+          *reinterpret_cast<uint2*>(out + ((size_t)gb * 42 + cell) * C + 16 * (m0 + m) + 4 * lg) = __builtin_bit_cast(uint2, o);
+      } else if (valid) {
+        *out_ptr(e_slot[a], m) = __builtin_bit_cast(uint2, o);
+      }
+    }
+  };
+
+  load_frags(0, 0);
+  if (kPrefetch) {
+#pragma unroll
+    for (int g = 0; g < G_TILES; g++) {
+      const int a = g & 1, f = g & 1;
+      start_tile(g, a);
+      if (g + 1 < G_TILES) load_frags(g + 1, f ^ 1);
+      mfmas(f, a);
+      if (g >= 1) epilogue(a ^ 1);
+    }
+    epilogue((G_TILES - 1) & 1);
+  } else {
+#pragma unroll
+    for (int g = 0; g < G_TILES; g++) {
+      start_tile(g, 0);
+      mfmas(0, 0);
+      epilogue(0);
+      if (g + 1 < G_TILES) load_frags(g + 1, 0);
+    }
+  }
+  after_last_tile();
+}
+
+template <int KW, int NWAVES>
+__device__ __forceinline__ void dma_weights(const void* w, uint32_t bytes, uint4* lds_dst, int first_frag, int wave, int lane) {
+  const auto rsrc = __builtin_amdgcn_make_buffer_rsrc(const_cast<void*>(w), 0, (int)bytes, 0x00020000);
+  const int wave_u = __builtin_amdgcn_readfirstlane(wave);
+  for (int c = wave_u; c < KW; c += NWAVES)
+    __builtin_amdgcn_raw_ptr_buffer_load_lds(rsrc, (__attribute__((address_space(3))) void*)(lds_dst + c * 64), 16, lane * 16, (first_frag + c) * 1024, 0, 0);
+}
+
+template <int C, int NB, int NT>
+struct StagedTower {
+  using G = Geo<C, NB>;
+  static_assert(G::kStageW, "the layers' weights go through the LDS stages");
+  static constexpr int MTW = G::MT;
+  static constexpr int kWSteps = 9 * G::KC;
+  static constexpr int kIn = (NB * 42 + NT - 1) / NT;
+  static constexpr int kWaves = NT / 64;
+  static_assert(G::kTiles % kWaves == 0, "every wavefront owns the same number of cell tiles");
+  static constexpr int kTilesPerWave = G::kTiles / kWaves;
+  static constexpr int kFreeUntilLayer1 = 2 * G::kBufSlots * 16;
+  static constexpr int kFreeUntilLayer1Bytes = G::kWFrags * 1024;
+  typedef bf16x8 WF[kWSteps][MTW];
+
+  static __device__ __forceinline__ uint4* X(uint8_t* lds_raw) { return reinterpret_cast<uint4*>(lds_raw); }
+  static __device__ __forceinline__ uint4* T(uint8_t* lds_raw) { return X(lds_raw) + G::kBufSlots; }
+  static __device__ __forceinline__ uint4* Wst(uint8_t* lds_raw) { return T(lds_raw) + G::kBufSlots; }
+
+  static __device__ __forceinline__ void load_conv0_weights(WF& wf, const TowerParams& p, int lane) {
+#pragma unroll
+    for (int k = 0; k < 3; k++)
+#pragma unroll
+      for (int m = 0; m < MTW; m++) wf[k][m] = p.w0[(k * G::MT + m) * 64 + lane];
+  }
+  template <int NWAVES>
+  static __device__ __forceinline__ void stage_layer_weights(const TowerParams& p, uint8_t* lds_raw, int layer, int wave, int lane) {
+    if (layer <= 2 * (int)p.n_blocks)
+      dma_weights<G::kWFrags, NWAVES>(p.w, 2u * p.n_blocks * G::kWFrags * 1024u, Wst(lds_raw) + (layer & 1) * G::kWFrags * 64, (layer - 1) * G::kWFrags, wave, lane);
+  }
+  static __device__ __forceinline__ void load_input(const TowerParams& p, uint32_t board0, int tid, uint32_t (&in_v)[kIn]) {
+#pragma unroll
+    for (int j = 0; j < kIn; j++) {
+      const int i = tid + j * NT;
+      const int b = i / 42, cell = i - b * 42;
+      const uint32_t g = board0 + b;
+      in_v[j] = 0;
+      if (i < NB * 42 && g < p.n_boards) in_v[j] = (uint32_t)p.planes[(size_t)g * 84 + cell] | ((uint32_t)p.planes[(size_t)g * 84 + 42 + cell] << 16);
+    }
+  }
+  template <int NP>
+  static __device__ __forceinline__ void zero_images(uint8_t* lds_raw, int t) {
+    uint4* x = X(lds_raw);
+    for (int i = t; i < 2 * G::kBufSlots; i += NP) x[i] = make_uint4(0, 0, 0, 0);
+  }
+  static __device__ __forceinline__ void store_input(uint8_t* lds_raw, int tid, const uint32_t (&in_v)[kIn]) {
+    uint4* t = T(lds_raw);
+#pragma unroll
+    for (int j = 0; j < kIn; j++) {
+      const int i = tid + j * NT;
+      const int b = i / 42, cell = i - b * 42;
+      if (i < NB * 42) t[b * kBS + cell_slot(cell / 7, cell % 7)] = make_uint4(in_v[j], 0, 0, 0);
+    }
+  }
+  template <typename Stamp>
+  static __device__ __forceinline__ bool layers(const TowerParams& p, uint8_t* lds_raw, WF& wf, uint32_t board0, int tid, Stamp&& stamp) {
+    uint4 *x = X(lds_raw), *t = T(lds_raw);
+    const int lane = tid & 63, wave = tid >> 6;
+    const int n_layers = 2 * (int)p.n_blocks;
+    const int tile_lo = wave * kTilesPerWave;
+    auto nothing = []() __attribute__((always_inline)) {};
+    tower_layer<C, NB, true, false, false, kTilesPerWave, MTW, true>(t, x, wf, p.bias, tile_lo, 0, lane, nothing);
+    asm volatile("s_waitcnt vmcnt(0)" ::: "memory");
+    __syncthreads();
+    stamp(2);
+    for (int layer = 1; layer <= n_layers; layer++) {
+      const bool is_second = (layer & 1) == 0;
+      stage_layer_weights<kWaves>(p, lds_raw, layer + 1, wave, lane);
+      const uint4* ws = Wst(lds_raw) + (layer & 1) * G::kWFrags * 64;
+#pragma unroll
+      for (int k = 0; k < kWSteps; k++)
+#pragma unroll
+        for (int m = 0; m < MTW; m++)
+          wf[k][m] = __builtin_bit_cast(bf16x8, ws[(((k / G::KC) * G::MT + m) * G::KC + (k % G::KC)) * 64 + lane]);
+      if (layer == n_layers) {
+        tower_layer<C, NB, false, true, true, kTilesPerWave, MTW, true>(t, x, wf, p.bias + (size_t)layer * C, tile_lo, 0, lane, nothing,
+                                                                         p.out, board0, p.n_boards);
+        return true;
+      }
+      if (is_second) tower_layer<C, NB, false, true, false, kTilesPerWave, MTW, true>(t, x, wf, p.bias + (size_t)layer * C, tile_lo, 0, lane, nothing);
+      else tower_layer<C, NB, false, false, false, kTilesPerWave, MTW, true>(x, t, wf, p.bias + (size_t)layer * C, tile_lo, 0, lane, nothing);
+      asm volatile("s_waitcnt vmcnt(0)" ::: "memory");
+      __syncthreads();
+      stamp(2 + layer);
+    }
+    return false;
+  }
+};
+
+}
diff --git a/c4a0_amd/nn.py b/c4a0_amd/nn.py
--- a/c4a0_amd/nn.py
+++ b/c4a0_amd/nn.py
@@ -328,6 +328,7 @@
         self.gemm_config = (int(cfg[0]), int(cfg[-1]))
         self.tower_config = int(tower_config)
         self._np_lock = threading.Lock()
+        self._tower_ready = {}
         ch = self.chain = (_F32Chain(folded, self.device) if f32 else _Bf16Chain(folded, self.device, hip_gemm=gemm == "hip") if self.hip_tower
                            else _TorchChain(folded, self.device, dtype))
         self.merged_w1 = self.merged_b1 = None
@@ -356,7 +357,9 @@
         hook, ch = self.stage_hook, self.chain
         if hook is not None:
             hook(0)
-        x = self.tower(planes, latency)
+        x = self._tower_ready.pop((planes.data_ptr(), planes.shape[0]), None) if self._tower_ready else None
+        if x is None:
+            x = self.tower(planes, latency)
         if hook is not None:
             hook(2)
         if self.merged_w1 is not None:
@@ -379,6 +382,14 @@
     def fused_step_ok(self) -> bool:
         own = type(self).forward is InferenceNet.forward and type(self).__call__ is InferenceNet.__call__
         return own and bool(self.hip_tower) and self.dtype == torch.bfloat16 and (42 * self.channels) % 1344 == 0
+
+    @property
+    def fused_tower_ok(self) -> bool:
+        return self.fused_step_ok and self.channels == 32 and self.n_blocks >= 1 and self.tower_config == 0 and not self.latency_mode
+
+    def tower_operands(self):
+        ch = self.chain
+        return ch.tw0, ch.tw, ch.tbias
 
     def head_out_operands(self):
         ch = self.chain
diff --git a/c4a0_amd/session.py b/c4a0_amd/session.py
--- a/c4a0_amd/session.py
+++ b/c4a0_amd/session.py
@@ -73,8 +73,11 @@
         self.rows = self.n_slots
         self._bound_stream = None
         self._timing, self._extensions = True, False
+        self._tower_mark = None
 
     def close(self):
+        if getattr(self, "_tower_mark", None) is not None:
+            self._drop_tower_mark()
         if getattr(self, "_h", None):
             self.L.c4_session_destroy(self._h)
             self._h = None
@@ -104,6 +107,7 @@
                 sm = (C.c_uint64 * max(1, n))(*[int(m) for m, _ in start_positions])
                 sv = (C.c_uint64 * max(1, n))(*[int(v) for _, v in start_positions])
         check(self.L.c4_session_set_games(self._h, arr, n, sm, sv))
+        self._drop_tower_mark()
         self.n_games = n
         self.rows = self.n_slots
 
@@ -112,6 +116,7 @@
         check(self.L.c4_session_bind_io(self._h, self.planes.data_ptr(), self.logprobs.data_ptr(), self.q.data_ptr(),
                                         C.c_void_p(st.cuda_stream)))
         self._bound_stream = st
+        self._drop_tower_mark()
 
     def set_dirichlet(self, alpha: float, epsilon: float):
         check(self.L.c4_session_set_dirichlet(self._h, float(alpha), float(epsilon)))
@@ -133,7 +138,19 @@
         return {"bytes": b.value, "blocks_per_slot": bps.value, "reclaim_half_blocks": half.value}
 
     def start(self):
+        self._drop_tower_mark()
         check(self.L.c4_session_start(self._h))
+
+    def _drop_tower_mark(self):
+        mark, self._tower_mark = self._tower_mark, None
+        if mark is not None:
+            mark[0]._tower_ready.pop(mark[1], None)
+
+    def _tower_next_ok(self, evaluator, rows: int) -> bool:
+        knob = self.fuse_next_tower
+        return bool(knob and getattr(evaluator, "fused_tower_ok", False) and not self.search and not self.hold
+                    and self.planes.dtype == torch.bfloat16 and (knob == "force" or rows > 1024)
+                    and hasattr(self.L, "c4_session_step_head_out_tower"))
 
     def step(self):
         check(self.L.c4_session_step(self._h))
@@ -147,13 +164,25 @@
             return
         check(self.L.c4_session_set_step_shape(self._h, int(games_per_wavefront)))
 
-    def round(self, evaluator: DeviceEvaluator):
+    def round(self, evaluator: DeviceEvaluator, tower_next: bool = False):
         if (self.fuse_output_step and not self._timing and not self._extensions and getattr(self, "leaf_models", None) is None
                 and getattr(evaluator, "fused_step_ok", False) and not ((self.search or self.hold) and self.planes.dtype != torch.bfloat16)):
             r = self.rows
             p, v = evaluator.forward_hidden(self.planes if r == self.n_slots else self.planes[:r])
             wp, wv, bp, bv = evaluator.head_out_operands()
             assert p.stride(1) == 1 and v.stride(1) == 1 and p.shape[0] == r
+            self._tower_mark = None
+            if tower_next and self._tower_next_ok(evaluator, r):
+                x = torch.empty((r, 42 * evaluator.channels), dtype=torch.bfloat16, device=self.device)
+                tw0, tw, tb = evaluator.tower_operands()
+                check(self.L.c4_session_step_head_out_tower(self._h, C.c_void_p(p.data_ptr()), C.c_void_p(v.data_ptr()), C.c_void_p(wp.data_ptr()),
+                                                            C.c_void_p(wv.data_ptr()), C.c_void_p(bp.data_ptr()), C.c_void_p(bv.data_ptr()),
+                                                            p.shape[1], p.stride(0), v.stride(0), C.c_void_p(tw0.data_ptr()), C.c_void_p(tw.data_ptr()),
+                                                            C.c_void_p(tb.data_ptr()), evaluator.channels, evaluator.n_blocks, C.c_void_p(x.data_ptr())))
+                key = (self.planes.data_ptr(), r)
+                evaluator._tower_ready[key] = x
+                self._tower_mark = (evaluator, key)
+                return
             check(self.L.c4_session_step_head_out(self._h, C.c_void_p(p.data_ptr()), C.c_void_p(v.data_ptr()), C.c_void_p(wp.data_ptr()),
                                                   C.c_void_p(wv.data_ptr()), C.c_void_p(bp.data_ptr()), C.c_void_p(bv.data_ptr()),
                                                   p.shape[1], p.stride(0), v.stride(0)))
@@ -179,8 +208,8 @@
         graph = torch.cuda.CUDAGraph()
         with capture(graph, stream if stream is not None else torch.cuda.Stream(device=self.device)):
             self.bind(torch.cuda.current_stream(self.device))
-            for _ in range(steps_per_graph):
-                self.round(evaluator)
+            for i in range(steps_per_graph):
+                self.round(evaluator, tower_next=i + 1 < steps_per_graph)
         self.bind(main)
         return graph
 
@@ -202,6 +231,7 @@
     def compact(self, multiple: int = 256) -> Tuple[int, int]:
         act, rows = C.c_uint32(), C.c_uint32()
         check(self.L.c4_session_compact(self._h, int(multiple), C.byref(act), C.byref(rows)))
+        self._drop_tower_mark()
         self.rows = rows.value
         return act.value, rows.value
 
@@ -279,6 +309,7 @@
             q.copy_(q_out.reshape(r, 2))
 
     fuse_output_step = True
+    fuse_next_tower = True
     NARROW_CHECK_ROUNDS = 64
 
     def wants_narrowing(self, multiple: int = 256, asynchronous: bool = False) -> bool:
@@ -413,11 +444,12 @@
                         ev_b.record(s1)
 
                 evaluator.stage_hook = hook_a
+                tower_next = r + 1 < steps_per_graph
                 with torch.cuda.stream(s0):
-                    a.round(evaluator)
+                    a.round(evaluator, tower_next=tower_next)
                 evaluator.stage_hook = hook_b
                 with torch.cuda.stream(s1):
-                    b.round(evaluator)
+                    b.round(evaluator, tower_next=tower_next)
                 ev_b_prev = ev_b
             s0.wait_stream(s1)
     finally:
diff --git a/include/c4a0_hip.h b/include/c4a0_hip.h
--- a/include/c4a0_hip.h
+++ b/include/c4a0_hip.h
@@ -8,7 +8,7 @@
 extern "C" {
 #endif
 
-#define C4_ABI_VERSION 13
+#define C4_ABI_VERSION 14
 
 #define C4_N_COLS 7
 #define C4_N_ROWS 6
@@ -129,6 +129,10 @@
 int c4_session_step_head_out(c4_session* s, const void* hidden_policy_dev, const void* hidden_value_dev, const void* w_policy_dev,
                              const void* w_value_dev, const float* b_policy_dev, const float* b_value_dev, uint32_t features,
                              uint32_t policy_row_stride, uint32_t value_row_stride);
+int c4_session_step_head_out_tower(c4_session* s, const void* hidden_policy_dev, const void* hidden_value_dev, const void* w_policy_dev,
+                                   const void* w_value_dev, const float* b_policy_dev, const float* b_value_dev, uint32_t features,
+                                   uint32_t policy_row_stride, uint32_t value_row_stride, const void* tower_w0_dev, const void* tower_w_dev,
+                                   const float* tower_bias_dev, uint32_t channels, uint32_t n_blocks, void* tower_out_dev);
 int c4_session_set_step_shape(c4_session* s, uint32_t games_per_wavefront);
 
 int c4_session_set_timing(c4_session* s, int enable);
```

Result: slower. 26470 (-8.2%).
